# pculbertson/argus

Measured on NVIDIA B200. Metric: train image-pairs/sec, higher is better.
Workload: dtype bf16

## Files before the change

argus_b200/csrc/api.cu:

```cuda
#include "../../include/argus_b200.h"

#include "conv_ops.h"
#include "kernels.h"
#include "kernels_fp32.h"
#include "model.h"
#include "runtime.h"

#include <algorithm>
#include <cstring>
#include <vector>

using namespace argus;

static float* lib_scratch(int64_t elems) {
  static float* buf = nullptr;
  static int64_t cap = 0;
  if (elems > cap) {
    ARGUS_CUDA(cudaDeviceSynchronize());
    if (buf) ARGUS_CUDA(cudaFree(buf));
    ARGUS_CUDA(cudaMalloc(&buf, elems * sizeof(float)));
    cap = elems;
  }
  return buf;
}

static ConvShape make_shape(int N, int H, int W, int Cin, int Cout, int k, int stride, int kind) {
  ConvShape s;
  s.N = N; s.H = H; s.W = W; s.Cin = Cin; s.Cout = Cout; s.k = k; s.stride = stride; s.kind = kind;
  return s;
}

extern "C" {

const char* argus_last_error_string(void) { return get_last_error(); }
int argus_version(void) { return 100; }

int argus_profile_enable(int on) {
  ARGUS_API_BEGIN
  profile_enable(on != 0);
  ARGUS_API_END
}
int argus_profile_report(char* json, int cap) {
  ARGUS_API_BEGIN
  ARGUS_CHECK(json != nullptr && cap > 2, "bad report buffer");
  const std::string r = profile_report_json();
  ARGUS_CHECK(static_cast<int>(r.size()) < cap, "profile report buffer too small");
  std::memcpy(json, r.c_str(), r.size() + 1);
  ARGUS_API_END
}
int64_t argus_launch_count(void) { return launch_count(); }

int argus_require_device(void) {
  ARGUS_API_BEGIN
  require_sm100();
  ARGUS_API_END
}

int argus_conv2d_forward(const void* x, const void* w, void* y, int N, int H, int W, int Cin, int Cout, int k,
                         int stride, int kind, const float* scale, const float* shift, const void* residual, int relu,
                         float* stat_partial, int stat_slot_capacity, void* stream) {
  ARGUS_API_BEGIN
  require_sm100();
  ConvShape s = make_shape(N, H, W, Cin, Cout, k, stride, kind);
  ConvLaunch l = plan_conv_forward(s, static_cast<const __nv_bfloat16*>(x), static_cast<const __nv_bfloat16*>(w),
                                   static_cast<__nv_bfloat16*>(y));
  Epilogue e;
  e.scale = scale; e.shift = shift; e.residual = static_cast<const __nv_bfloat16*>(residual); e.relu = relu;
  e.stat_partial = stat_partial;
  ARGUS_CHECK(stat_partial == nullptr || stat_slot_capacity >= stat_slots(l), "statistics buffer has too few slots");
  launch_conv(l, e, static_cast<cudaStream_t>(stream));
  ARGUS_API_END
}

int argus_conv2d_stat_slots(int N, int H, int W, int Cin, int Cout, int k, int stride, int kind, int* slots) {
  ARGUS_API_BEGIN
  require_sm100();
  ARGUS_CHECK(slots != nullptr, "null argument");
  ConvShape s = make_shape(N, H, W, Cin, Cout, k, stride, kind);
  validate_shape(s);
  const int64_t m_tiles = (s.out_pixels() + kBlockM - 1) / kBlockM;
  const int64_t tiles = m_tiles * ((Cout + 63) / 64);
  *slots = 4 * static_cast<int>(std::min<int64_t>(tiles, num_sms()));
  ARGUS_API_END
}

int argus_conv2d_dgrad(const void* dy, const void* w, void* dx, int N, int H, int W, int Cin, int Cout, int k,
                       int stride, const void* residual, void* stream) {
  ARGUS_API_BEGIN
  require_sm100();
  ConvShape s = make_shape(N, H, W, Cin, Cout, k, stride, 0);
  ARGUS_CHECK(residual == nullptr || stride == 1, "residual add is only supported for stride-1 dgrad");
  auto ls = plan_conv_dgrad(s, static_cast<const __nv_bfloat16*>(dy), static_cast<const __nv_bfloat16*>(w),
                            static_cast<__nv_bfloat16*>(dx));
  Epilogue e;
  e.residual = static_cast<const __nv_bfloat16*>(residual);
  for (auto& l : ls) launch_conv(l, e, static_cast<cudaStream_t>(stream));
  ARGUS_API_END
}

int argus_conv2d_dgrad_bits(const void* dy, const void* w, void* dx, int N, int H, int W, int Cin, int Cout, int k,
                            const void* residual, const void* residual_bits, void* stream) {
  ARGUS_API_BEGIN
  require_sm100();
  ConvShape s = make_shape(N, H, W, Cin, Cout, k, 1, 0);
  ARGUS_CHECK(residual != nullptr && residual_bits != nullptr, "null argument");
  auto ls = plan_conv_dgrad(s, static_cast<const __nv_bfloat16*>(dy), static_cast<const __nv_bfloat16*>(w),
                            static_cast<__nv_bfloat16*>(dx));
  Epilogue e;
  e.residual = static_cast<const __nv_bfloat16*>(residual);
  e.residual_bits = static_cast<const uint8_t*>(residual_bits);
  for (auto& l : ls) launch_conv(l, e, static_cast<cudaStream_t>(stream));
  ARGUS_API_END
}

int argus_conv2d_dgrad_ex(const void* dy, const void* w, void* dx, int N, int H, int W, int Cin, int Cout, int stride,
                          const void* concat_a, int concat_channels, const float* bias, const void* residual,
                          const void* out_bits, float* stat_partial, int stat_slot_capacity, void* stream) {
  ARGUS_API_BEGIN
  require_sm100();
  ConvShape s = make_shape(N, H, W, Cin, Cout, 1, stride, 0);
  ARGUS_CHECK(residual == nullptr || stride == 1, "residual add is only supported for stride-1 dgrad");
  ConvLaunch l;
  if (concat_a != nullptr) {
    l = plan_dgrad_concat(s, static_cast<const __nv_bfloat16*>(dy), static_cast<const __nv_bfloat16*>(concat_a),
                          concat_channels, static_cast<const __nv_bfloat16*>(w), static_cast<__nv_bfloat16*>(dx));
  } else {
    auto ls = plan_conv_dgrad(s, static_cast<const __nv_bfloat16*>(dy), static_cast<const __nv_bfloat16*>(w),
                              static_cast<__nv_bfloat16*>(dx));
    ARGUS_CHECK(ls.size() == 1, "unexpected dgrad decomposition");
    l = ls[0];
  }
  Epilogue e;
  e.shift = bias;
  e.residual = static_cast<const __nv_bfloat16*>(residual);
  e.out_bits = static_cast<const uint8_t*>(out_bits);
  e.stat_partial = stat_partial;
  ARGUS_CHECK(stat_partial == nullptr || stat_slot_capacity >= stat_slots(l), "statistics buffer has too few slots");
  launch_conv(l, e, static_cast<cudaStream_t>(stream));
  ARGUS_API_END
}

int argus_conv2d_forward_full(const void* x, const void* w, void* y, int N, int H, int W, int Cin, int Cout, int k,
                              int stride, int kind, const float* scale, const float* shift, const void* residual,
                              const float* res_scale, const float* res_shift, int relu, void* relu_bits_out,
                              float* stat_partial, int stat_slot_capacity, int early_trigger, void* stream) {
  ARGUS_API_BEGIN
  require_sm100();
  ConvShape s = make_shape(N, H, W, Cin, Cout, k, stride, kind);
  ConvLaunch l = plan_conv_forward(s, static_cast<const bf16*>(x), static_cast<const bf16*>(w), static_cast<bf16*>(y));
  Epilogue e;
  e.scale = scale; e.shift = shift; e.residual = static_cast<const bf16*>(residual);
  e.res_scale = res_scale; e.res_shift = res_shift;
  e.relu = relu; e.relu_bits_out = static_cast<uint8_t*>(relu_bits_out);
  e.stat_partial = stat_partial;
  e.early_trigger = early_trigger;
  ARGUS_CHECK(relu_bits_out == nullptr || relu != 0, "the ReLU bit mask needs the ReLU");
  ARGUS_CHECK(res_scale == nullptr || residual != nullptr, "residual scale / shift need a residual");
  ARGUS_CHECK(stat_partial == nullptr || stat_slot_capacity >= stat_slots(l), "statistics buffer has too few slots");
  launch_conv(l, e, static_cast<cudaStream_t>(stream));
  ARGUS_API_END
}

static ConvLaunch plan_bnred_dgrad(const ConvShape& s, const void* dy, const void* w, void* dx, const void* concat_a,
                                   int concat_channels) {
  ARGUS_CHECK(s.stride == 1, "the fused BN reduction exists for stride-1 dgrads");
  if (concat_a != nullptr)
    return plan_dgrad_concat(s, static_cast<const bf16*>(dy), static_cast<const bf16*>(concat_a), concat_channels,
                             static_cast<const bf16*>(w), static_cast<bf16*>(dx));
  auto ls = plan_conv_dgrad(s, static_cast<const bf16*>(dy), static_cast<const bf16*>(w), static_cast<bf16*>(dx));
  ARGUS_CHECK(ls.size() == 1, "unexpected dgrad decomposition");
  return ls[0];
}

int argus_conv2d_dgrad_bnred(const void* dy, const void* w, void* dx, int N, int H, int W, int Cin, int Cout, int k,
                             int stride, const void* concat_a, int concat_channels, const float* bias,
                             const void* bn_raw, const float* bn_scale, const float* bn_shift, float* stat_partial,
                             int stat_slot_capacity, void* stream) {
  ARGUS_API_BEGIN
  require_sm100();
  ARGUS_CHECK(bn_raw != nullptr && bn_scale != nullptr && bn_shift != nullptr && stat_partial != nullptr,
              "null argument");
  ConvShape s = make_shape(N, H, W, Cin, Cout, k, stride, 0);
  ConvLaunch l = plan_bnred_dgrad(s, dy, w, dx, concat_a, concat_channels);
  Epilogue e;
  e.shift = bias;
  e.bn_raw = static_cast<const bf16*>(bn_raw);
  e.bn_scale = bn_scale;
  e.bn_shift = bn_shift;
  e.stat_partial = stat_partial;
  ARGUS_CHECK(stat_slot_capacity >= stat_slots(l), "statistics buffer has too few slots");
  launch_conv(l, e, static_cast<cudaStream_t>(stream));
  ARGUS_API_END
}

int argus_conv2d_launch_info(int launch, int N, int H, int W, int Cin, int Cout, int k, int stride, int kind,
                             int concat_channels, int flags, int* out, int cap, int* n_launches) {
  ARGUS_API_BEGIN
  require_sm100();
  ARGUS_CHECK(out != nullptr && n_launches != nullptr, "null argument");
  ARGUS_CUDA(cudaFree(nullptr));
  static __align__(1024) char dummy[1024];
  bf16* d = reinterpret_cast<bf16*>(dummy);
  const float* f = reinterpret_cast<const float*>(dummy);
  uint8_t* b = reinterpret_cast<uint8_t*>(dummy);
  ConvShape s = make_shape(N, H, W, Cin, Cout, k, stride, kind);
  std::vector<ConvLaunch> ls;
  if (launch == 0) ls.push_back(plan_conv_forward(s, d, d, d));
  else if (launch == 1 && (flags & ARGUS_EPI_BN_RAW)) ls.push_back(plan_bnred_dgrad(s, d, d, d, nullptr, 0));
  else if (launch == 1) ls = plan_conv_dgrad(s, d, d, d);
  else if (launch == 2 && (flags & ARGUS_EPI_BN_RAW))
    ls.push_back(plan_bnred_dgrad(make_shape(N, H, W, Cin, Cout, 1, stride, 0), d, d, d, d, concat_channels));
  else if (launch == 2) ls.push_back(plan_dgrad_concat(make_shape(N, H, W, Cin, Cout, 1, stride, 0), d, d, concat_channels, d, d));
  else throw Error("unknown launch kind");
  Epilogue e;
  if (flags & ARGUS_EPI_SCALE) e.scale = f;
  if (flags & ARGUS_EPI_SHIFT) e.shift = f;
  if (flags & ARGUS_EPI_RESIDUAL) e.residual = d;
  if (flags & ARGUS_EPI_RES_AFFINE) { e.res_scale = f; e.res_shift = f; }
  if (flags & ARGUS_EPI_RELU) e.relu = 1;
  if (flags & ARGUS_EPI_RELU_BITS_OUT) e.relu_bits_out = b;
  if (flags & ARGUS_EPI_OUT_BITS) e.out_bits = b;
  if (flags & ARGUS_EPI_RESIDUAL_BITS) e.residual_bits = b;
  if (flags & ARGUS_EPI_STATS) e.stat_partial = const_cast<float*>(f);
  if (flags & ARGUS_EPI_BN_RAW) { e.bn_raw = d; e.bn_scale = f; e.bn_shift = f; }
  if (flags & ARGUS_EPI_EARLY_TRIGGER) e.early_trigger = 1;
  *n_launches = static_cast<int>(ls.size());
  ARGUS_CHECK(cap >= ARGUS_LAUNCH_INFO_INTS * *n_launches, "launch info buffer too small");
  for (size_t i = 0; i < ls.size(); ++i) {
    const ConvLaunchInfo li = conv_launch_info(ls[i], e);
    const int v[ARGUS_LAUNCH_INFO_INTS] = {li.inst.block_n, li.inst.b_mn, li.inst.opt, li.halo, li.b_resident,
                                           li.halo_stages, li.num_m_tiles, li.num_n_tiles, li.grid, li.stat_slots};
    std::memcpy(out + i * ARGUS_LAUNCH_INFO_INTS, v, sizeof(v));
  }
  ARGUS_API_END
}

int argus_conv_instances_record(int on) {
  ARGUS_API_BEGIN
  conv_instances_record(on != 0);
  ARGUS_API_END
}
int argus_conv_instances_get(int* keys, int cap, int* n) {
  ARGUS_API_BEGIN
  ARGUS_CHECK(n != nullptr && (keys != nullptr || cap == 0), "null argument");
  const auto rec = conv_instances_recorded();
  *n = static_cast<int>(rec.size());
  for (int i = 0; i < *n && 5 * (i + 1) <= cap; ++i) std::memcpy(keys + 5 * i, rec[i].data(), 5 * sizeof(int));
  ARGUS_API_END
}

int argus_conv_instances_all(int* keys, int cap, int* n) {
  ARGUS_API_BEGIN
  ARGUS_CHECK(n != nullptr && (keys != nullptr || cap == 0), "null argument");
  const auto all = conv_instances_all();
  *n = static_cast<int>(all.size());
  for (int i = 0; i < *n && 3 * (i + 1) <= cap; ++i) std::memcpy(keys + 3 * i, all[i].data(), 3 * sizeof(int));
  ARGUS_API_END
}

int argus_conv2d_gram(const void* x, float* g, int N, int H, int W, int Cin, int Cout, int stride, void* stream) {
  ARGUS_API_BEGIN
  require_sm100();
  ConvShape s = make_shape(N, H, W, Cin, Cout, 1, stride, 0);
  validate_shape(s);
  WgradLaunch l = plan_gram(s, static_cast<const bf16*>(x), g);
  launch_wgrad(l, lib_scratch(wgrad_scratch_elems(l)), static_cast<cudaStream_t>(stream));
  ARGUS_API_END
}

int argus_colsum_pixels(const void* x, int N, int H, int W, int C, int stride, float* scratch, float* out, void* stream) {
  ARGUS_API_BEGIN
  require_sm100();
  ARGUS_CHECK(x != nullptr && scratch != nullptr && out != nullptr, "null argument");
  ARGUS_CHECK(N > 0 && H > 0 && W > 0 && (stride == 1 || stride == 2) && H % stride == 0 && W % stride == 0,
              "colsum: bad shape");
  colsum_pixels_bf16(static_cast<const bf16*>(x), N, H, W, C, stride, scratch, out, static_cast<cudaStream_t>(stream));
  ARGUS_API_END
}

int argus_bn_stats_from_gram(const void* W, const float* G, const float* s, double rows, const float* gamma,
                             const float* beta, float* running_mean, float* running_var, float momentum, float eps,
                             float* scale, float* shift, float* save_mean, float* save_invstd, float* scratch, int O,
                             int C, void* stream) {
  ARGUS_API_BEGIN
  require_sm100();
  ARGUS_CHECK((running_mean == nullptr) == (running_var == nullptr), "running mean and variance come together");
  bn_stats_from_gram(static_cast<const bf16*>(W), G, s, rows, gamma, beta, running_mean, running_var, momentum, eps,
                     scale, shift, save_mean, save_invstd, scratch, O, C, static_cast<cudaStream_t>(stream));
  ARGUS_API_END
}

int argus_conv2d_wgrad_gram(const void* dy, const void* x, float* dw, int N, int H, int W, int Cin, int Cout, int stride,
                            void* stream) {
  ARGUS_API_BEGIN
  require_sm100();
  ConvShape s = make_shape(N, H, W, Cin, Cout, 1, stride, 0);
  WgradLaunch l = plan_conv_wgrad_gram(s, static_cast<const __nv_bfloat16*>(dy), static_cast<const __nv_bfloat16*>(x), dw);
  launch_wgrad(l, lib_scratch(wgrad_scratch_elems(l)), static_cast<cudaStream_t>(stream));
  ARGUS_API_END
}

int argus_conv_bn_backward_algebraic(const void* g, const void* act, const void* w_bf16, const float* g_colsum,
                                     const float* scale, const float* mean, const float* invstd, float* dgamma,
                                     float* dbeta, float* dw, void* dact, int N, int H, int W, int C, int O, int stride,
                                     void* stream) {
  ARGUS_API_BEGIN
  require_sm100();
  cudaStream_t st = static_cast<cudaStream_t>(stream);
  ConvShape s = make_shape(N, H, W, C, O, 1, stride, 0);
  const int64_t rows = s.out_pixels();
  const size_t OC = static_cast<size_t>(O) * C, CC = static_cast<size_t>(C) * C;
  const int64_t colsum_scratch = 4LL * num_sms() * C;
  const int64_t mpart = bn_alg_matrix_scratch_elems(C);
  const int64_t total = static_cast<int64_t>(OC + CC) + C + 2 * O + C + colsum_scratch + mpart + (static_cast<int64_t>(O + C) * C + 1) / 2;
  static float* buf = nullptr;
  static int64_t cap = 0;
  if (total > cap) {
    ARGUS_CUDA(cudaDeviceSynchronize());
    if (buf) ARGUS_CUDA(cudaFree(buf));
    ARGUS_CUDA(cudaMalloc(&buf, total * sizeof(float)));
    cap = total;
  }
  float* Hb = buf;
  float* Gb = Hb + OC;
  float* sb = Gb + CC;
  float* k1k0 = sb + C;
  float* bias = k1k0 + 2 * O;
  float* cs = bias + C;
  float* mp = cs + colsum_scratch;
  bf16* bstack = reinterpret_cast<bf16*>(mp + mpart);
  const bf16* G16 = static_cast<const bf16*>(g);
  const bf16* A16 = static_cast<const bf16*>(act);
  const bf16* W16 = static_cast<const bf16*>(w_bf16);
  WgradLaunch hg = plan_conv_wgrad_gram(s, G16, A16, Hb);
  ConvLaunch concat = plan_dgrad_concat(s, G16, A16, C, bstack, static_cast<bf16*>(dact));
  ARGUS_CUDA(cudaMemsetAsync(Hb, 0, (OC + CC) * sizeof(float), st)); pdl_break(st, kPdlAfterMemop);
  launch_wgrad(hg, lib_scratch(wgrad_scratch_elems(hg)), st);
  colsum_pixels_bf16(A16, N, H, W, C, stride, cs, sb, st);
  bn_alg_backward_small(W16, Hb, Gb, sb, g_colsum, 1, O, scale, mean, invstd, static_cast<double>(rows), dgamma, dbeta, dw,
                        k1k0, bstack, bias, mp, O, C, st);
  if (stride == 2)
    ARGUS_CUDA(cudaMemsetAsync(dact, 0, static_cast<size_t>(N) * H * W * C * sizeof(bf16), st)); pdl_break(st, kPdlAfterMemop);
  Epilogue e;
  e.shift = bias;
  launch_conv(concat, e, st);
  ARGUS_API_END
}

int argus_conv2d_wgrad(const void* dy, const void* x, float* dw, int N, int H, int W, int Cin, int Cout, int k,
                       int stride, int kind, void* stream) {
  ARGUS_API_BEGIN
  require_sm100();
  ConvShape s = make_shape(N, H, W, Cin, Cout, k, stride, kind);
  WgradLaunch l = plan_conv_wgrad(s, static_cast<const __nv_bfloat16*>(dy), static_cast<const __nv_bfloat16*>(x), dw);
  launch_wgrad(l, lib_scratch(wgrad_scratch_elems(l)), static_cast<cudaStream_t>(stream));
  ARGUS_API_END
}

int argus_stem_dgrad(const void* dy, const void* w, float* dx, int N, int H, int W, void* stream) {
  ARGUS_API_BEGIN
  require_sm100();
  stem_dgrad(static_cast<const __nv_bfloat16*>(dy), static_cast<const __nv_bfloat16*>(w), dx, N, H, W,
             static_cast<cudaStream_t>(stream));
  ARGUS_API_END
}

int argus_bn_finalize(const float* partial, int slots, double count, const float* gamma, const float* beta,
                      float* running_mean, float* running_var, float momentum, float eps, float* scale, float* shift,
                      float* save_mean, float* save_invstd, int C, void* stream) {
  ARGUS_API_BEGIN
  require_sm100();
  bn_finalize(partial, slots, count, gamma, beta, running_mean, running_var, momentum, eps, scale, shift, save_mean,
              save_invstd, C, static_cast<cudaStream_t>(stream));
  ARGUS_API_END
}
int argus_bn_apply(const void* x, const float* scale, const float* shift, const void* res, const float* rscale,
                   const float* rshift, int relu, void* y, int64_t rows, int C, void* stream) {
  ARGUS_API_BEGIN
  require_sm100();
  bn_apply(static_cast<const bf16*>(x), scale, shift, static_cast<const bf16*>(res), rscale, rshift, relu,
           static_cast<bf16*>(y), nullptr, nullptr, rows, C, static_cast<cudaStream_t>(stream));
  ARGUS_API_END
}
int argus_bn_apply_bits(const void* x, const float* scale, const float* shift, const void* res, const float* rscale,
                        const float* rshift, int relu, void* y, void* relu_bits, int64_t rows, int C, void* stream) {
  ARGUS_API_BEGIN
  require_sm100();
  bn_apply(static_cast<const bf16*>(x), scale, shift, static_cast<const bf16*>(res), rscale, rshift, relu,
           static_cast<bf16*>(y), static_cast<uint8_t*>(relu_bits), nullptr, rows, C, static_cast<cudaStream_t>(stream));
  ARGUS_API_END
}
int argus_bn_backward(void* dy, const void* x, const void* out, const float* scale, const float* shift,
                      const float* mean, const float* invstd, float* dgamma, float* dbeta, void* dx, int64_t rows,
                      int C, int mask_mode, void* stream) {
  ARGUS_API_BEGIN
  require_sm100();
  cudaStream_t s = static_cast<cudaStream_t>(stream);
  bn_check_aligned(dy, x, out, dx);
  bn_bwd_reduce(static_cast<const bf16*>(dy), static_cast<const bf16*>(x), static_cast<const bf16*>(out), scale, shift,
                mean, invstd, dgamma, dbeta, rows, C, mask_mode, lib_scratch(bn_bwd_scratch_elems()), s);
  bn_bwd_apply(static_cast<bf16*>(dy), static_cast<const bf16*>(x), static_cast<const bf16*>(out), scale, shift, mean,
               invstd, dgamma, dbeta, static_cast<bf16*>(dx), rows, C, mask_mode, s);
  ARGUS_API_END
}
int argus_maxpool_forward(const void* x, const float* scale, const float* shift, void* y, void* idx, int N, int H,
                          int W, int C, void* stream) {
  ARGUS_API_BEGIN
  require_sm100();
  ARGUS_CHECK(H % 2 == 0 && W % 2 == 0 && C % 8 == 0, "maxpool: even H, W and C % 8 == 0 required");
  maxpool_fwd(static_cast<const bf16*>(x), scale, shift, static_cast<bf16*>(y), static_cast<uint8_t*>(idx), N, H, W, C,
              static_cast<cudaStream_t>(stream));
  ARGUS_API_END
}
int argus_maxpool_backward(const void* dy, const void* idx, void* dx, int N, int H, int W, int C, void* stream) {
  ARGUS_API_BEGIN
  require_sm100();
  maxpool_bwd(static_cast<const bf16*>(dy), static_cast<const uint8_t*>(idx), static_cast<bf16*>(dx), N, H, W, C,
              static_cast<cudaStream_t>(stream));
  ARGUS_API_END
}
int argus_stem_pool_bn_backward(const void* dpool, const void* idx, const void* raw, const float* scale,
                                const float* shift, const float* mean, const float* invstd, float* dgamma,
                                float* dbeta, void* dx, int N, int H, int W, int C, void* stream) {
  ARGUS_API_BEGIN
  require_sm100();
  stem_pool_bn_backward(static_cast<const bf16*>(dpool), static_cast<const uint8_t*>(idx), static_cast<const bf16*>(raw),
                        scale, shift, mean, invstd, dgamma, dbeta, static_cast<bf16*>(dx), N, H, W, C,
                        lib_scratch(bn_bwd_scratch_elems()), static_cast<cudaStream_t>(stream));
  ARGUS_API_END
}
int argus_avgpool_forward(const void* x, void* y, int N, int HW, int C, void* stream) {
  ARGUS_API_BEGIN
  require_sm100();
  avgpool_fwd(static_cast<const bf16*>(x), static_cast<bf16*>(y), N, HW, C, static_cast<cudaStream_t>(stream));
  ARGUS_API_END
}
int argus_avgpool_backward(const void* dy, void* dx, int N, int HW, int C, void* stream) {
  ARGUS_API_BEGIN
  require_sm100();
  avgpool_bwd(static_cast<const bf16*>(dy), static_cast<bf16*>(dx), nullptr, N, HW, C, static_cast<cudaStream_t>(stream));
  ARGUS_API_END
}

int argus_augment_sample_params(float* params, int n_images, int n_cams, int H, int W, uint64_t seed, uint64_t step,
                                const argus_aug_config* cfg, void* stream) {
  ARGUS_API_BEGIN
  require_sm100();
  ARGUS_CHECK(cfg != nullptr && params != nullptr && n_cams >= 1, "bad augmentation arguments");
  AugConfig c;
  c.color_jiggle = cfg->color_jiggle; c.planckian_jitter = cfg->planckian_jitter; c.blur = cfg->blur;
  c.motion_blur = cfg->motion_blur; c.plasma_shadow = cfg->plasma_shadow;
  c.brightness_lo = cfg->brightness_lo; c.brightness_span = cfg->brightness_span;
  c.contrast_lo = cfg->contrast_lo; c.contrast_span = cfg->contrast_span;
  c.saturation_lo = cfg->saturation_lo; c.saturation_span = cfg->saturation_span;
  c.hue_lo = cfg->hue_lo; c.hue_span = cfg->hue_span;
  c.random_erasing = cfg->random_erasing; c.salt_and_pepper = cfg->salt_and_pepper;
  augment_sample_params(params, n_images, n_cams, H, W, seed, step, c, static_cast<cudaStream_t>(stream));
  ARGUS_API_END
}
int argus_augment(const void* in, int in_u8, void* out, int out_s2d, const float* params, const void* arc_mask,
                  void* plasma_ws, int n_images, int H, int W, int apply, void* stream) {
  ARGUS_API_BEGIN
  require_sm100();
  ARGUS_CHECK(!apply || params != nullptr, "augmentation needs a parameter table");
  augment_images(in, in_u8 != 0, out, out_s2d != 0, params, static_cast<const uint32_t*>(arc_mask),
                 static_cast<uint32_t*>(plasma_ws), n_images, H, W, apply != 0, static_cast<cudaStream_t>(stream));
  ARGUS_API_END
}

int argus_spaghetti_sample_params(float* arcs, int n_images, int n_arcs, int H, int W, uint64_t seed, uint64_t step,
                                  void* stream) {
  ARGUS_API_BEGIN
  require_sm100();
  ARGUS_CHECK(arcs != nullptr, "null arc table");
  spaghetti_sample_params(arcs, n_images, n_arcs, H, W, seed, step, static_cast<cudaStream_t>(stream));
  ARGUS_API_END
}
int argus_spaghetti_mask(const float* arcs, void* mask, int n_images, int n_arcs, int H, int W, void* stream) {
  ARGUS_API_BEGIN
  require_sm100();
  ARGUS_CHECK(mask != nullptr && (arcs != nullptr || n_arcs == 0), "null argument");
  spaghetti_mask(arcs, static_cast<uint32_t*>(mask), n_images, n_arcs, H, W, static_cast<cudaStream_t>(stream));
  ARGUS_API_END
}
int argus_spaghetti_draw(const void* in, void* out, const float* arcs, void* mask_ws, int n_images, int n_arcs, int H,
                         int W, void* stream) {
  ARGUS_API_BEGIN
  require_sm100();
  ARGUS_CHECK(in != nullptr && out != nullptr && mask_ws != nullptr && (arcs != nullptr || n_arcs == 0), "null argument");
  spaghetti_draw(static_cast<const uint8_t*>(in), static_cast<uint8_t*>(out), arcs, static_cast<uint32_t*>(mask_ws),
                 n_images, n_arcs, H, W, static_cast<cudaStream_t>(stream));
  ARGUS_API_END
}

int argus_pose_loss(const float* pred, const float* target, float* loss, float* loss_mean, float* grad, int B,
                    float grad_scale, void* stream) {
  ARGUS_API_BEGIN
  require_sm100();
  ARGUS_CHECK(B >= 0, "negative batch");
  pose_loss_fwd_bwd(pred, target, loss, loss_mean, grad, B, grad_scale, static_cast<cudaStream_t>(stream));
  ARGUS_API_END
}

int argus_pose_exp(const float* pred, float* pose, int B, int wxyz, void* stream) {
  ARGUS_API_BEGIN
  require_sm100();
  pose_exp(pred, pose, B, wxyz, static_cast<cudaStream_t>(stream));
  ARGUS_API_END
}

int argus_clip_adam_step(float* params, const float* grads, float* exp_avg, float* exp_avg_sq, int64_t n,
                         float* scratch, float gscale, float max_norm, float lr, float beta1, float beta2, float eps,
                         int step, float* norm_out, void* stream) {
  ARGUS_API_BEGIN
  require_sm100();
  ARGUS_CHECK(step >= 1, "Adam step counter starts at 1");
  cudaStream_t s = static_cast<cudaStream_t>(stream);
  const int np = grad_sqnorm_partials(grads, n, scratch, s);
  clip_adam_step(params, grads, exp_avg, exp_avg_sq, n, scratch, np, gscale, max_norm, lr, beta1, beta2, eps, step,
                 norm_out, false, s);
  ARGUS_API_END
}
int argus_clip_adam_step_amp(float* params, const float* grads, float* exp_avg, float* exp_avg_sq, int64_t n,
                             float* scratch, float gscale, float max_norm, float lr, float beta1, float beta2, float eps,
                             int step, float* norm_out, void* stream) {
  ARGUS_API_BEGIN
  require_sm100();
  ARGUS_CHECK(step >= 1, "Adam step counter starts at 1");
  ARGUS_CHECK(norm_out != nullptr, "the caller needs the gradient norm to learn whether the step was skipped");
  cudaStream_t s = static_cast<cudaStream_t>(stream);
  const int np = grad_sqnorm_partials(grads, n, scratch, s);
  clip_adam_step(params, grads, exp_avg, exp_avg_sq, n, scratch, np, gscale, max_norm, lr, beta1, beta2, eps, step,
                 norm_out, true, s);
  ARGUS_API_END
}

static ConvShapeF32 make_shape_f32(int N, int H, int W, int Cin, int Cout, int k, int stride) {
  ARGUS_CHECK(N > 0 && H > 0 && W > 0 && Cin > 0 && Cout > 0, "empty convolution");
  ARGUS_CHECK((k == 1 || k == 3 || k == 7) && (stride == 1 || stride == 2), "fp32 conv: k in {1,3,7}, stride in {1,2}");
  ConvShapeF32 s;
  s.N = N; s.H = H; s.W = W; s.Cin = Cin; s.Cout = Cout; s.k = k; s.stride = stride;
  return s;
}
int argus_fp32_conv2d_forward(const float* x, const float* w, const float* bias, float* y, int N, int H, int W, int Cin,
                              int Cout, int k, int stride, void* stream) {
  ARGUS_API_BEGIN
  require_sm100();
  conv_f32_forward(make_shape_f32(N, H, W, Cin, Cout, k, stride), x, w, bias, y, static_cast<cudaStream_t>(stream));
  ARGUS_API_END
}
int argus_fp32_conv2d_dgrad(const float* dy, const float* w, float* dx, int N, int H, int W, int Cin, int Cout, int k,
                            int stride, void* stream) {
  ARGUS_API_BEGIN
  require_sm100();
  conv_f32_dgrad(make_shape_f32(N, H, W, Cin, Cout, k, stride), dy, w, dx, static_cast<cudaStream_t>(stream));
  ARGUS_API_END
}
int argus_fp32_conv2d_wgrad(const float* dy, const float* x, float* dw, int N, int H, int W, int Cin, int Cout, int k,
                            int stride, void* stream) {
  ARGUS_API_BEGIN
  require_sm100();
  const ConvShapeF32 s = make_shape_f32(N, H, W, Cin, Cout, k, stride);
  conv_f32_wgrad(s, dy, x, dw, lib_scratch(conv_f32_wgrad_scratch_elems(s, nullptr)), static_cast<cudaStream_t>(stream));
  ARGUS_API_END
}
static double* lib_scratch_f64(int64_t elems) { return reinterpret_cast<double*>(lib_scratch(2 * elems)); }
int argus_fp32_bn_train(const float* x, int64_t rows, int C, const float* gamma, const float* beta, float* running_mean,
                        float* running_var, float momentum, float eps, float* scale, float* shift, float* save_mean,
                        float* save_invstd, void* stream) {
  ARGUS_API_BEGIN
  require_sm100();
  bn_f32_train_stats(x, rows, C, gamma, beta, running_mean, running_var, momentum, eps, scale, shift, save_mean,
                     save_invstd, lib_scratch_f64(static_cast<int64_t>(kBnF32MaxBlocks) * 2 * C),
                     static_cast<cudaStream_t>(stream));
  ARGUS_API_END
}
int argus_fp32_bn_apply(const float* x, const float* scale, const float* shift, const float* res, const float* rscale,
                        const float* rshift, int relu, float* y, int64_t rows, int C, void* stream) {
  ARGUS_API_BEGIN
  require_sm100();
  bn_f32_apply(x, scale, shift, res, rscale, rshift, relu, y, rows, C, static_cast<cudaStream_t>(stream));
  ARGUS_API_END
}
int argus_fp32_bn_backward(const float* dy, const float* x, const float* out, const float* scale, const float* mean,
                           const float* invstd, float* dgamma, float* dbeta, float* dx, float* g_out, int64_t rows,
                           int C, void* stream) {
  ARGUS_API_BEGIN
  require_sm100();
  double* part = lib_scratch_f64(static_cast<int64_t>(kBnF32MaxBlocks) * 2 * C + C);
  float* sums = reinterpret_cast<float*>(part + static_cast<int64_t>(kBnF32MaxBlocks) * 2 * C);
  bn_f32_backward(dy, x, out, scale, mean, invstd, dgamma, dbeta, dx, g_out, rows, C, part, sums,
                  static_cast<cudaStream_t>(stream));
  ARGUS_API_END
}
int argus_fp32_maxpool_forward(const float* x, float* y, void* idx, int N, int H, int W, int C, void* stream) {
  ARGUS_API_BEGIN
  require_sm100();
  maxpool_f32_fwd(x, y, static_cast<uint8_t*>(idx), N, H, W, C, static_cast<cudaStream_t>(stream));
  ARGUS_API_END
}
int argus_fp32_maxpool_backward(const float* dy, const void* idx, float* dx, int N, int H, int W, int C, void* stream) {
  ARGUS_API_BEGIN
  require_sm100();
  maxpool_f32_bwd(dy, static_cast<const uint8_t*>(idx), dx, N, H, W, C, static_cast<cudaStream_t>(stream));
  ARGUS_API_END
}

struct argus_model {
  Model impl;
  argus_model(int n_cams, int dim) : impl(n_cams, dim) {}
};

int argus_model_create(argus_model** out, int n_cams, int resnet_output_dim) {
  ARGUS_API_BEGIN
  ARGUS_CHECK(out != nullptr, "null out pointer");
  *out = new argus_model(n_cams, resnet_output_dim);
  ARGUS_API_END
}
int argus_model_destroy(argus_model* m) {
  ARGUS_API_BEGIN
  delete m;
  ARGUS_API_END
}
int argus_model_counts(argus_model* m, int* n_params, int* n_buffers, int64_t* param_elems, int64_t* buffer_elems) {
  ARGUS_API_BEGIN
  ARGUS_CHECK(m != nullptr, "null model");
  if (n_params) *n_params = static_cast<int>(m->impl.params().size());
  if (n_buffers) *n_buffers = static_cast<int>(m->impl.buffers().size());
  if (param_elems) *param_elems = m->impl.num_param_elems();
  if (buffer_elems) *buffer_elems = m->impl.num_buffer_elems();
  ARGUS_API_END
}
int argus_model_tensor_info(argus_model* m, int is_buffer, int index, char* name, int name_cap, int64_t* offset,
                            int64_t* numel, int* ndim, int64_t* shape) {
  ARGUS_API_BEGIN
  ARGUS_CHECK(m != nullptr, "null model");
  const auto& v = is_buffer ? m->impl.buffers() : m->impl.params();
  ARGUS_CHECK(index >= 0 && index < static_cast<int>(v.size()), "tensor index out of range");
  const TensorInfo& t = v[index];
  if (name && name_cap > 0) {
    std::strncpy(name, t.name.c_str(), name_cap - 1);
    name[name_cap - 1] = 0;
  }
  if (offset) *offset = t.offset;
  if (numel) *numel = t.numel;
  if (ndim) *ndim = t.ndim;
  if (shape) for (int i = 0; i < 4; ++i) shape[i] = t.shape[i];
  ARGUS_API_END
}
int argus_model_bind(argus_model* m, float* params, float* grads, float* buffers) {
  ARGUS_API_BEGIN
  ARGUS_CHECK(m != nullptr, "null model");
  m->impl.bind(params, grads, buffers);
  ARGUS_API_END
}
int argus_model_reserve(argus_model* m, int max_batch, int H, int W, int training) {
  ARGUS_API_BEGIN
  ARGUS_CHECK(m != nullptr, "null model");
  m->impl.reserve(max_batch, H, W, training != 0);
  ARGUS_API_END
}
int argus_model_sync_weights(argus_model* m, void* stream) {
  ARGUS_API_BEGIN
  ARGUS_CHECK(m != nullptr, "null model");
  m->impl.sync_weights(static_cast<cudaStream_t>(stream));
  ARGUS_API_END
}
int argus_model_forward(argus_model* m, const void* x, int is_u8, int B, int H, int W, int training, float* out,
                        void* stream) {
  ARGUS_API_BEGIN
  ARGUS_CHECK(m != nullptr, "null model");
  m->impl.forward(x, is_u8 != 0, B, H, W, training != 0, out, static_cast<cudaStream_t>(stream));
  ARGUS_API_END
}
int argus_model_stage_input_u8(argus_model* m, const void* images, const float* aug_params, const void* arc_mask,
                               void* plasma_ws, int B, int H, int W, int training, int apply, void* stream) {
  ARGUS_API_BEGIN
  ARGUS_CHECK(m != nullptr, "null model");
  m->impl.stage_input_u8(static_cast<const uint8_t*>(images), aug_params, static_cast<const uint32_t*>(arc_mask),
                         static_cast<uint32_t*>(plasma_ws), B, H, W, training != 0, apply != 0,
                         static_cast<cudaStream_t>(stream));
  ARGUS_API_END
}
int argus_model_set_precision(argus_model* m, int mode) {
  ARGUS_API_BEGIN
  ARGUS_CHECK(m != nullptr, "null model");
  m->impl.set_precision(mode);
  ARGUS_API_END
}
int argus_model_set_wgrad_overlap(argus_model* m, int on) {
  ARGUS_API_BEGIN
  ARGUS_CHECK(m != nullptr, "null model");
  m->impl.set_wgrad_overlap(on != 0);
  ARGUS_API_END
}
int argus_model_zero_grads(argus_model* m, void* stream) {
  ARGUS_API_BEGIN
  ARGUS_CHECK(m != nullptr, "null model");
  m->impl.zero_grads(static_cast<cudaStream_t>(stream));
  ARGUS_API_END
}
int argus_model_backward(argus_model* m, const float* d_out, int stage_begin, int stage_end, void* stream) {
  ARGUS_API_BEGIN
  ARGUS_CHECK(m != nullptr, "null model");
  ARGUS_CHECK(0 <= stage_begin && stage_begin <= stage_end && stage_end <= 4, "bad stage range");
  m->impl.backward(d_out, stage_begin, stage_end, static_cast<cudaStream_t>(stream));
  ARGUS_API_END
}
int argus_model_input_grad(argus_model* m, float* dx, void* stream) {
  ARGUS_API_BEGIN
  ARGUS_CHECK(m != nullptr, "null model");
  ARGUS_CHECK(dx != nullptr, "null gradient buffer");
  m->impl.input_grad(dx, static_cast<cudaStream_t>(stream));
  ARGUS_API_END
}
int argus_model_stage_range(argus_model* m, int stage, int64_t* begin, int64_t* end) {
  ARGUS_API_BEGIN
  ARGUS_CHECK(m != nullptr, "null model");
  m->impl.stage_param_range(stage, begin, end);
  ARGUS_API_END
}
int argus_model_copy_activation(argus_model* m, int index, void* dst, int64_t capacity_elems, int64_t* rows, int* C,
                                void* stream) {
  ARGUS_API_BEGIN
  ARGUS_CHECK(m != nullptr, "null model");
  m->impl.copy_activation(index, dst, capacity_elems, rows, C, static_cast<cudaStream_t>(stream));
  ARGUS_API_END
}
int argus_model_arena_bytes(argus_model* m, int64_t* bytes) {
  ARGUS_API_BEGIN
  ARGUS_CHECK(m != nullptr, "null model");
  *bytes = static_cast<int64_t>(m->impl.arena_bytes());
  ARGUS_API_END
}

}
```

argus_b200/csrc/conv_gemm.cuh:

```cuda
#pragma once
#include "ptx.cuh"

namespace argus {

constexpr int kBlockM = 128;
constexpr int kBlockK = 64;
constexpr int kNumThreads = 320;
constexpr int kWgradThreads = 192;
constexpr int kMaxTaps = 16;

struct Tap {
  int8_t map;
  int8_t dh;
  int8_t dw;
  int8_t pad_;
  int32_t b_off;
};

struct ConvGemmParams {
  CUtensorMap a_map[4];
  CUtensorMap b_map;
  CUtensorMap out_map;
  CUtensorMap res_map;
  Tap taps[kMaxTaps];
  int num_taps;
  int kblocks_per_tap;
  int num_m_tiles;
  int num_n_tiles;
  int log2_wo;
  int log2_howo;
  int m_total;
  int n_total;
  const float* scale;
  const float* shift;
  int has_res;
  int b_resident;
  int res_stages;
  int halo;
  int halo_rows;
  int halo_row_bytes;
  int halo_stages;
  int32_t halo_boff[3][3];
  CUtensorMap halo_map;
  const uint8_t* res_bits;
  const float* res_scale;
  const float* res_shift;
  uint8_t* relu_bits_out;
  const uint8_t* out_bits;
  int k2_blocks;
  int relu;
  const __nv_bfloat16* bn_raw;
  const float* bn_scale;
  const float* bn_shift;
  int early_trigger;
  float* stat_partial;
};

template <int BLOCK_N, int OPT, int EPI = 2>
constexpr int conv_staging_buffers() { return (EPI == 4 || (BLOCK_N == 64 && !(OPT & 2))) ? 1 : 2; }

template <int BLOCK_N, int EPI = 2, int NBUF = 2>
struct ConvGemmSmem {
  static constexpr int kABytes = kBlockM * kBlockK * 2;
  static constexpr int kBBytes = BLOCK_N * kBlockK * 2;
  static constexpr int kStageBytes = kABytes + kBBytes;
  static constexpr int kStagingBytes = kBlockM * 128;
  static constexpr int kGroupCols = (EPI == 4) ? BLOCK_N / 2 : BLOCK_N;
  static constexpr int kStatsBytes = EPI * 4 * 2 * kGroupCols * 4;
  static constexpr int kPipeBytes = (232448 - 1024 - NBUF * EPI * kStagingBytes - kStatsBytes - 512) / 1024 * 1024;
  static constexpr int kStagesRaw = kPipeBytes / kStageBytes;
  static constexpr int kStages = kStagesRaw > 6 ? 6 : kStagesRaw;
  static constexpr int kOffStaging = kPipeBytes;
  static constexpr int kOffStats = kOffStaging + NBUF * EPI * kStagingBytes;
  static constexpr int kOffBars = kOffStats + kStatsBytes;
  static constexpr int kMaxStages = 8;
  static constexpr int kNumBars = 2 * kMaxStages + EPI + 2 + 2 * EPI + 1;
  static constexpr int kOffTmemPtr = kOffBars + kNumBars * 8;
  static constexpr int kTotal = kOffTmemPtr + 16;
};

constexpr int kOptAffine = 1;
constexpr int kOptRes = 2;
constexpr int kOptOutBits = 4;
constexpr int kOptRelu = 8;
constexpr int kOptResExtra = 16;
constexpr int kOptBnRed = 32;
constexpr int kOptAll = 31;
template <int BLOCK_N, int B_MN, int EPI, int OPT = kOptAll>
__global__ void __launch_bounds__(64 + 128 * EPI, 1)
conv_gemm_kernel(const __grid_constant__ ConvGemmParams p) {
  pdl_begin(p.early_trigger);
  constexpr int NBUF = conv_staging_buffers<BLOCK_N, OPT, EPI>();
  static_assert(NBUF == 2 || !(OPT & kOptRes), "the residual prefetch needs two staging buffers");
  constexpr bool SPLIT = (EPI == 4);
  constexpr int kTileGroups = SPLIT ? 2 : EPI;
  static_assert(!SPLIT || (BLOCK_N == 256 && !(OPT & kOptRes)), "split-tile mode: 256-wide tiles without residual");
  using L = ConvGemmSmem<BLOCK_N, EPI, NBUF>;
  constexpr int kStages = L::kStages;
  constexpr int kTmemCols = (2 * BLOCK_N) < 32 ? 32 : (2 * BLOCK_N);
  static_assert(BLOCK_N == 64 || BLOCK_N == 128 || BLOCK_N == 256, "BLOCK_N");

  extern __shared__ __align__(1024) uint8_t smem[];
  const uint32_t smem_base = smem_u32(smem);
  const int warp = threadIdx.x >> 5;
  const int lane = threadIdx.x & 31;

  constexpr int kMaxStages = L::kMaxStages;
  const uint32_t bar_base = smem_base + L::kOffBars;
  auto full_bar = [&](int s) { return bar_base + 8u * s; };
  auto empty_bar = [&](int s) { return bar_base + 8u * (kMaxStages + s); };
  auto tfull_bar = [&](int g) { return bar_base + 8u * (2 * kMaxStages + g); };
  auto tempty_bar = [&](int s) { return bar_base + 8u * (2 * kMaxStages + EPI + s); };
  auto res_bar = [&](int g, int b) { return bar_base + 8u * (2 * kMaxStages + EPI + 2 + 2 * g + b); };
  const uint32_t bres_bar = bar_base + 8u * (2 * kMaxStages + EPI + 2 + 2 * EPI);
  volatile uint32_t* tmem_ptr_smem = reinterpret_cast<volatile uint32_t*>(smem + L::kOffTmemPtr);
  float* s_stats_all = reinterpret_cast<float*>(smem + L::kOffStats);
  const bool resident = (p.b_resident != 0);
  const bool halo = (p.halo != 0);
  const uint32_t halo_a_bytes = static_cast<uint32_t>(p.halo_rows + 2) * p.halo_row_bytes;
  const int nstages = halo ? p.halo_stages : (resident ? p.res_stages : kStages);
  const uint32_t stage_bytes = halo ? halo_a_bytes + (resident ? 0u : 3u * L::kBBytes)
                                    : (resident ? L::kABytes : L::kStageBytes);
  const uint32_t bres_base = smem_base + static_cast<uint32_t>(nstages) * stage_bytes;

  if (threadIdx.x == 0) {
    if (smem_base & 1023u) __trap();
    for (int s = 0; s < kMaxStages; ++s) {
      mbar_init(full_bar(s), 1);
      mbar_init(empty_bar(s), 1);
    }
    mbar_init(bres_bar, 1);
    for (int s = 0; s < 2; ++s) mbar_init(tempty_bar(s), SPLIT ? 8 : 4);
    for (int g = 0; g < EPI; ++g) {
      mbar_init(tfull_bar(g), 1);
      mbar_init(res_bar(g, 0), 1);
      mbar_init(res_bar(g, 1), 1);
    }
    fence_mbar_init();
  }
  if (warp == 0 && lane == 0) {
    for (int i = 0; i < 4; ++i) tma_prefetch_desc(&p.a_map[i]);
    if (p.halo) tma_prefetch_desc(&p.halo_map);
    tma_prefetch_desc(&p.b_map);
    tma_prefetch_desc(&p.out_map);
    if (p.has_res) tma_prefetch_desc(&p.res_map);
  }
  if (warp == 1) {
    tmem_alloc(smem_u32(const_cast<uint32_t*>(tmem_ptr_smem)), kTmemCols);
    tmem_relinquish();
  }
  for (int i = threadIdx.x; i < EPI * 8 * L::kGroupCols; i += blockDim.x) s_stats_all[i] = 0.f;
  tc_fence_before();
  __syncthreads();
  tc_fence_after();
  const uint32_t tmem_base = *tmem_ptr_smem;
  pdl_wait_deferred(p.early_trigger);

  const int num_tiles = p.num_m_tiles * p.num_n_tiles;
  const int num_kblocks = p.num_taps * p.kblocks_per_tap + p.k2_blocks;

  if (warp == 0) {
    if (lane == 0) {
      auto load_b = [&](uint32_t bar, uint32_t sb, const Tap& tap, int kb, int n0) {
        if (B_MN == 0) {
          tma_load_2d(&p.b_map, bar, sb, tap.b_off + kb * kBlockK, n0);
        } else {
#pragma unroll
          for (int j = 0; j < BLOCK_N / 64; ++j)
            tma_load_2d(&p.b_map, bar, sb + j * 8192, tap.b_off + n0 + j * 64, kb * kBlockK);
        }
      };
      if (resident && blockIdx.x < num_tiles) {
        const int n0 = (blockIdx.x % p.num_n_tiles) * BLOCK_N;
        mbar_arrive_expect_tx(bres_bar, static_cast<uint32_t>(num_kblocks) * L::kBBytes);
        if (halo) {
          for (int kb = 0; kb < p.kblocks_per_tap; ++kb)
            for (int dwi = 0; dwi < 3; ++dwi)
              for (int dhi = 0; dhi < 3; ++dhi) {
                Tap tap{};
                tap.b_off = p.halo_boff[dwi][dhi];
                load_b(bres_bar, bres_base + static_cast<uint32_t>((kb * 3 + dwi) * 3 + dhi) * L::kBBytes, tap, kb, n0);
              }
        } else {
          for (int t = 0; t < p.num_taps; ++t)
            for (int kb = 0; kb < p.kblocks_per_tap; ++kb)
              load_b(bres_bar, bres_base + static_cast<uint32_t>(t * p.kblocks_per_tap + kb) * L::kBBytes, p.taps[t], kb, n0);
        }
      }
      int stage = 0;
      uint32_t phase = 0;
      for (int tile = blockIdx.x; tile < num_tiles; tile += gridDim.x) {
        const int m_tile = tile / p.num_n_tiles;
        const int n_tile = tile - m_tile * p.num_n_tiles;
        const int m0 = m_tile * kBlockM;
        const int img0 = m0 >> p.log2_howo;
        const int rem = m0 & ((1 << p.log2_howo) - 1);
        const int h0 = rem >> p.log2_wo;
        const int w0 = rem & ((1 << p.log2_wo) - 1);
        const int n0 = n_tile * BLOCK_N;
        if (halo) {
          for (int kb = 0; kb < p.kblocks_per_tap; ++kb)
            for (int dwi = 0; dwi < 3; ++dwi) {
              mbar_wait(empty_bar(stage), phase ^ 1);
              const uint32_t sa = smem_base + stage * stage_bytes;
              mbar_arrive_expect_tx(full_bar(stage), stage_bytes);
              tma_load_4d(&p.halo_map, full_bar(stage), sa, kb * kBlockK, w0 + dwi - 1, h0 - 1, img0);
              if (!resident) {
#pragma unroll
                for (int dhi = 0; dhi < 3; ++dhi) {
                  Tap tap{};
                  tap.b_off = p.halo_boff[dwi][dhi];
                  load_b(full_bar(stage), sa + halo_a_bytes + dhi * L::kBBytes, tap, kb, n0);
                }
              }
              if (++stage == nstages) { stage = 0; phase ^= 1; }
            }
          continue;
        }
        for (int t = 0; t < p.num_taps; ++t) {
          const Tap tap = p.taps[t];
          for (int kb = 0; kb < p.kblocks_per_tap; ++kb) {
            mbar_wait(empty_bar(stage), phase ^ 1);
            const uint32_t sa = smem_base + stage * stage_bytes;
            mbar_arrive_expect_tx(full_bar(stage), stage_bytes);
            tma_load_4d(&p.a_map[tap.map], full_bar(stage), sa, kb * kBlockK, w0 + tap.dw, h0 + tap.dh, img0);
            if (!resident) load_b(full_bar(stage), sa + L::kABytes, tap, kb, n0);
            if (++stage == nstages) { stage = 0; phase ^= 1; }
          }
        }
        for (int kb = 0; kb < p.k2_blocks; ++kb) {
          mbar_wait(empty_bar(stage), phase ^ 1);
          const uint32_t sa = smem_base + stage * stage_bytes;
          mbar_arrive_expect_tx(full_bar(stage), stage_bytes);
          tma_load_4d(&p.a_map[1], full_bar(stage), sa, kb * kBlockK, w0, h0, img0);
          Tap tap{};
          load_b(full_bar(stage), sa + L::kABytes, tap, p.num_taps * p.kblocks_per_tap + kb, n0);
          if (++stage == nstages) { stage = 0; phase ^= 1; }
        }
      }
    }
  } else if (warp == 1) {
    if (lane == 0) {
      constexpr uint32_t idesc = make_idesc_bf16(kBlockM, BLOCK_N, 0, B_MN);
      int stage = 0;
      uint32_t phase = 0;
      int acc = 0;
      uint32_t acc_phase = 0;
      int tgrp = 0;
      if (resident && blockIdx.x < num_tiles) mbar_wait(bres_bar, 0);
      for (int tile = blockIdx.x; tile < num_tiles; tile += gridDim.x) {
        mbar_wait(tempty_bar(acc), acc_phase ^ 1);
        tc_fence_after();
        const uint32_t tmem_d = tmem_base + acc * BLOCK_N;
        if (halo) {
          const int nst = 3 * p.kblocks_per_tap;
          for (int st = 0; st < nst; ++st) {
            mbar_wait(full_bar(stage), phase);
            tc_fence_after();
            const uint32_t sa = smem_base + stage * stage_bytes;
#pragma unroll
            for (int dhi = 0; dhi < 3; ++dhi) {
              const uint32_t a0 = sa + static_cast<uint32_t>(dhi) * p.halo_row_bytes;
              const uint32_t sb = resident ? bres_base + static_cast<uint32_t>(st * 3 + dhi) * L::kBBytes
                                           : sa + halo_a_bytes + dhi * L::kBBytes;
#pragma unroll
              for (int k = 0; k < kBlockK / 16; ++k) {
                const uint64_t da = make_smem_desc_sw128(a0 + k * 32, 0, 1024);
                const uint64_t db = (B_MN == 0) ? make_smem_desc_sw128(sb + k * 32, 0, 1024)
                                                : make_smem_desc_sw128(sb + k * 2048, 8192, 1024);
                umma_bf16(tmem_d, da, db, idesc, (st | dhi | k) != 0);
              }
            }
            umma_commit(empty_bar(stage));
            if (st == nst - 1) umma_commit(tfull_bar(tgrp));
            if (++stage == nstages) { stage = 0; phase ^= 1; }
          }
          if (++acc == 2) { acc = 0; acc_phase ^= 1; }
          if (++tgrp == kTileGroups) tgrp = 0;
          continue;
        }
        for (int kb = 0; kb < num_kblocks; ++kb) {
          mbar_wait(full_bar(stage), phase);
          tc_fence_after();
          const uint32_t sa = smem_base + stage * stage_bytes;
          const uint32_t sb = resident ? bres_base + static_cast<uint32_t>(kb) * L::kBBytes : sa + L::kABytes;
#pragma unroll
          for (int k = 0; k < kBlockK / 16; ++k) {
            const uint64_t da = make_smem_desc_sw128(sa + k * 32, 0, 1024);
            const uint64_t db = (B_MN == 0) ? make_smem_desc_sw128(sb + k * 32, 0, 1024)
                                            : make_smem_desc_sw128(sb + k * 2048, 8192, 1024);
            umma_bf16(tmem_d, da, db, idesc, (kb | k) != 0);
          }
          umma_commit(empty_bar(stage));
          if (kb == num_kblocks - 1) umma_commit(tfull_bar(tgrp));
          if (++stage == nstages) { stage = 0; phase ^= 1; }
        }
        if (++acc == 2) { acc = 0; acc_phase ^= 1; }
        if (++tgrp == kTileGroups) tgrp = 0;
      }
    }
  } else {
    const int ew = warp - 2;
    const int grp = ew >> 2;
    const int tg = SPLIT ? (grp >> 1) : grp;
    constexpr int GW = L::kGroupCols;
    const int col_base = SPLIT ? (grp & 1) * GW : 0;
    const int wq = warp & 3;
    const int r = wq * 32 + lane;
    const int et = (ew & 3) * 32 + lane;
    const bool store_leader = (et == 0);
    const uint32_t bar_id = 1 + grp;
    float* s_stats = s_stats_all + grp * 8 * GW;
    float* s_mine = s_stats + (ew & 3) * 2 * GW;
    uint8_t* stg_base = smem + L::kOffStaging + grp * NBUF * L::kStagingBytes;
    uint32_t res_phase[2] = {0, 0};
    int buf = 0;
    int cur_n = -1;
    const bool do_stats = (p.stat_partial != nullptr);
    const bool has_res = (OPT & kOptRes) ? (p.has_res != 0) : false;
    const float* const ep_scale = (OPT & kOptAffine) ? p.scale : nullptr;
    const float* const ep_shift = (OPT & kOptAffine) ? p.shift : nullptr;
    const float* const ep_res_scale = (OPT & kOptResExtra) ? p.res_scale : nullptr;
    const float* const ep_res_shift = (OPT & kOptResExtra) ? p.res_shift : nullptr;
    const uint8_t* const ep_res_bits = (OPT & kOptResExtra) ? p.res_bits : nullptr;
    const uint8_t* const ep_out_bits = (OPT & kOptOutBits) ? p.out_bits : nullptr;
    uint8_t* const ep_relu_bits_out = (OPT & kOptRelu) ? p.relu_bits_out : nullptr;
    const bool ep_relu = (OPT & kOptRelu) ? (p.relu != 0) : false;
    constexpr bool BNRED = (OPT & kOptBnRed) != 0;
    static_assert(!BNRED || ((OPT & kOptRes) && !(OPT & (kOptResExtra | kOptRelu | kOptOutBits))), "kOptBnRed rides the residual path");
    float* my_partial = do_stats ? p.stat_partial + static_cast<size_t>(EPI * blockIdx.x + grp) * 2 * p.n_total : nullptr;
    constexpr int kChunks = GW / 64;
    constexpr bool FAST_TAIL = (OPT & kOptAffine) && !(OPT & ~(kOptAffine | kOptRes | kOptRelu)) && EPI == 2;
    float* s_aff = s_stats;
    int cur_aff_n = -1;

    auto flush_stats = [&](int n_tile) {
      named_bar_sync(bar_id, 128);
      for (int c = et; c < 2 * GW; c += 128) {
        const int which = c / GW, col = c - which * GW;
        const int gc = n_tile * BLOCK_N + col_base + col;
        float acc_s = 0.f;
#pragma unroll
        for (int w = 0; w < 4; ++w) {
          acc_s += s_stats[w * 2 * GW + c];
          s_stats[w * 2 * GW + c] = 0.f;
        }
        if (gc < p.n_total) my_partial[which * p.n_total + gc] += acc_s;
      }
      named_bar_sync(bar_id, 128);
    };
    auto issue_residual = [&](int tile, int ch, int b) {
      const int m_tile = tile / p.num_n_tiles;
      const int n_tile = tile - m_tile * p.num_n_tiles;
      const int m0 = m_tile * kBlockM;
      const int img0 = m0 >> p.log2_howo;
      const int rem = m0 & ((1 << p.log2_howo) - 1);
      mbar_arrive_expect_tx(res_bar(grp, b), L::kStagingBytes);
      tma_load_4d(&p.res_map, res_bar(grp, b), smem_u32(stg_base + b * L::kStagingBytes), n_tile * BLOCK_N + ch * 64,
                  rem & ((1 << p.log2_wo) - 1), rem >> p.log2_wo, img0);
    };
    const int first_tile = blockIdx.x + tg * gridDim.x;
    if (has_res && store_leader && first_tile < num_tiles) issue_residual(first_tile, 0, 0);

    int t_local = tg;
    uint32_t full_phase = 0;
    for (int tile = first_tile; tile < num_tiles; tile += kTileGroups * gridDim.x, t_local += kTileGroups, full_phase ^= 1) {
      const int acc = t_local & 1;
      const int m_tile = tile / p.num_n_tiles;
      const int n_tile = tile - m_tile * p.num_n_tiles;
      const int m0 = m_tile * kBlockM;
      const int img0 = m0 >> p.log2_howo;
      const int rem = m0 & ((1 << p.log2_howo) - 1);
      const int h0 = rem >> p.log2_wo;
      const int w0 = rem & ((1 << p.log2_wo) - 1);
      const int n0 = n_tile * BLOCK_N + col_base;
      if (do_stats && n_tile != cur_n) {
        if (cur_n >= 0) flush_stats(cur_n);
        cur_n = n_tile;
      }
      if (FAST_TAIL && n_tile != cur_aff_n) {
        named_bar_sync(bar_id, 128);
        for (int c = et; c < GW; c += 128) {
          const int gc = n_tile * BLOCK_N + col_base + c;
          s_aff[c] = gc < p.n_total ? __ldg(ep_scale + gc) : 0.f;
          s_aff[GW + c] = gc < p.n_total ? __ldg(ep_shift + gc) : 0.f;
        }
        named_bar_sync(bar_id, 128);
        cur_aff_n = n_tile;
      }

      mbar_wait(tfull_bar(tg), full_phase);
      tc_fence_after();

#pragma unroll 1
      for (int ch = 0; ch < kChunks; ++ch) {
        uint8_t* stg = stg_base + buf * L::kStagingBytes;
        uint32_t v[2][32];
#pragma unroll
        for (int h = 0; h < 2; ++h) {
          const uint32_t taddr = tmem_base + (static_cast<uint32_t>(wq * 32) << 16) + acc * BLOCK_N + col_base + ch * 64 + h * 32;
          tmem_ld_32x32(taddr, v[h]);
        }
        if (has_res && do_stats) named_bar_sync(bar_id, 128);
        if (store_leader) {
          if (has_res) {
            tma_store_wait_read<0>();
            const bool last_ch = (ch == kChunks - 1);
            const int ntile = last_ch ? tile + kTileGroups * gridDim.x : tile;
            if (ntile < num_tiles) issue_residual(ntile, last_ch ? 0 : ch + 1, buf ^ 1);
          } else {
            if (NBUF == 2) tma_store_wait_read<1>();
            else tma_store_wait_read<0>();
          }
        }
        if (!has_res) named_bar_sync(bar_id, 128);
        uint32_t rawc[BNRED ? 32 : 1];
        if (BNRED) {
          const uint32_t* rp = reinterpret_cast<const uint32_t*>(p.bn_raw + static_cast<size_t>(m0 + wq * 32) * p.n_total +
                                                                 n0 + ch * 64) + lane;
          const int nrow = p.m_total - (m0 + wq * 32);
#pragma unroll
          for (int rr = 0; rr < 32; ++rr)
            rawc[rr] = (rr < nrow) ? ldg_nc_u32(rp + static_cast<size_t>(rr) * (p.n_total >> 1)) : 0u;
        }
        uint2 obits = make_uint2(0xffffffffu, 0xffffffffu);
        if (ep_out_bits != nullptr && m0 + r < p.m_total)
          obits = __ldg(reinterpret_cast<const uint2*>(ep_out_bits + static_cast<size_t>(m0 + r) * (p.n_total >> 3) +
                                                       ((n0 + ch * 64) >> 3)));
        uint2 rbits = make_uint2(0xffffffffu, 0xffffffffu);
        if (ep_res_bits != nullptr && m0 + r < p.m_total)
          rbits = __ldg(reinterpret_cast<const uint2*>(ep_res_bits + static_cast<size_t>(m0 + r) * (p.n_total >> 3) +
                                                       ((n0 + ch * 64) >> 3)));
        tmem_ld_wait();
        if (ch == kChunks - 1) {
          tc_fence_before();
          __syncwarp();
          if (lane == 0) mbar_arrive(tempty_bar(acc));
        }
        if (has_res) {
          mbar_wait(res_bar(grp, buf), res_phase[buf]);
          res_phase[buf] ^= 1;
        }
#pragma unroll
        for (int h = 0; h < 2; ++h) {
          const int c0 = n0 + ch * 64 + h * 32;
          if constexpr (FAST_TAIL) {
            uint32_t ob = 0;
            const float4* sc4 = reinterpret_cast<const float4*>(s_aff + ch * 64 + h * 32);
            const float4* sh4 = reinterpret_cast<const float4*>(s_aff + GW + ch * 64 + h * 32);
#pragma unroll
            for (int q = 0; q < 4; ++q) {
              const int phys = (h * 4 + q) ^ (r & 7);
              uint4* slot = reinterpret_cast<uint4*>(stg + r * 128 + phys * 16);
              uint4 rv = make_uint4(0u, 0u, 0u, 0u);
              if constexpr ((OPT & kOptRes) != 0) rv = *slot;
              const float4 s0 = sc4[2 * q], s1 = sc4[2 * q + 1], t0 = sh4[2 * q], t1 = sh4[2 * q + 1];
              uint64_t y0 = f32x2_pack(t0.x, t0.y), y1 = f32x2_pack(t0.z, t0.w), y2 = f32x2_pack(t1.x, t1.y), y3 = f32x2_pack(t1.z, t1.w);
              f32x2_fma(y0, f32x2_pack(__uint_as_float(v[h][q * 8 + 0]), __uint_as_float(v[h][q * 8 + 1])), f32x2_pack(s0.x, s0.y));
              f32x2_fma(y1, f32x2_pack(__uint_as_float(v[h][q * 8 + 2]), __uint_as_float(v[h][q * 8 + 3])), f32x2_pack(s0.z, s0.w));
              f32x2_fma(y2, f32x2_pack(__uint_as_float(v[h][q * 8 + 4]), __uint_as_float(v[h][q * 8 + 5])), f32x2_pack(s1.x, s1.y));
              f32x2_fma(y3, f32x2_pack(__uint_as_float(v[h][q * 8 + 6]), __uint_as_float(v[h][q * 8 + 7])), f32x2_pack(s1.z, s1.w));
              if constexpr ((OPT & kOptRes) != 0) {
                f32x2_add(y0, f32x2_from_bf16x2(rv.x));
                f32x2_add(y1, f32x2_from_bf16x2(rv.y));
                f32x2_add(y2, f32x2_from_bf16x2(rv.z));
                f32x2_add(y3, f32x2_from_bf16x2(rv.w));
              }
              const float2 a = f32x2_unpack(y0), b = f32x2_unpack(y1), c = f32x2_unpack(y2), d = f32x2_unpack(y3);
              const float y8[8] = {a.x, a.y, b.x, b.y, c.x, c.y, d.x, d.y};
              if constexpr ((OPT & kOptRelu) != 0) {
#pragma unroll
                for (int j = 0; j < 8; ++j) ob |= (y8[j] > 0.f ? 1u : 0u) << (q * 8 + j);
              }
              const float floor_ = ep_relu ? 0.f : -INFINITY;
              uint4 o;
              o.x = pack_bf16x2(fmaxf(y8[0], floor_), fmaxf(y8[1], floor_));
              o.y = pack_bf16x2(fmaxf(y8[2], floor_), fmaxf(y8[3], floor_));
              o.z = pack_bf16x2(fmaxf(y8[4], floor_), fmaxf(y8[5], floor_));
              o.w = pack_bf16x2(fmaxf(y8[6], floor_), fmaxf(y8[7], floor_));
              *slot = o;
            }
            if constexpr ((OPT & kOptRelu) != 0) {
              if (ep_relu_bits_out != nullptr && m0 + r < p.m_total)
                *reinterpret_cast<uint32_t*>(ep_relu_bits_out + static_cast<size_t>(m0 + r) * (p.n_total >> 3) + (c0 >> 3)) = ob;
            }
          } else {
          float f[32];
#pragma unroll
          for (int i = 0; i < 32; ++i) f[i] = __uint_as_float(v[h][i]);
          if (ep_scale != nullptr) {
#pragma unroll
            for (int i = 0; i < 32; i += 4) {
              const float4 sc = __ldg(reinterpret_cast<const float4*>(ep_scale + c0 + i));
              f[i] *= sc.x; f[i + 1] *= sc.y; f[i + 2] *= sc.z; f[i + 3] *= sc.w;
            }
          }
          if (ep_shift != nullptr) {
#pragma unroll
            for (int i = 0; i < 32; i += 4) {
              const float4 sh = __ldg(reinterpret_cast<const float4*>(ep_shift + c0 + i));
              f[i] += sh.x; f[i + 1] += sh.y; f[i + 2] += sh.z; f[i + 3] += sh.w;
            }
          }
          if (BNRED) {
            const bool row_ok = (m0 + r < p.m_total);
#pragma unroll
            for (int q = 0; q < 4; ++q) {
              const int phys = (h * 4 + q) ^ (r & 7);
              const uint4 rv = *reinterpret_cast<const uint4*>(stg + r * 128 + phys * 16);
              const float2 a = unpack_bf16x2(rv.x), b = unpack_bf16x2(rv.y), c = unpack_bf16x2(rv.z), d = unpack_bf16x2(rv.w);
              const float rr8[8] = {a.x, a.y, b.x, b.y, c.x, c.y, d.x, d.y};
              const float4 s0 = __ldg(reinterpret_cast<const float4*>(p.bn_scale + c0 + q * 8));
              const float4 s1 = __ldg(reinterpret_cast<const float4*>(p.bn_scale + c0 + q * 8 + 4));
              const float4 t0 = __ldg(reinterpret_cast<const float4*>(p.bn_shift + c0 + q * 8));
              const float4 t1 = __ldg(reinterpret_cast<const float4*>(p.bn_shift + c0 + q * 8 + 4));
              const float sc8[8] = {s0.x, s0.y, s0.z, s0.w, s1.x, s1.y, s1.z, s1.w};
              const float sh8[8] = {t0.x, t0.y, t0.z, t0.w, t1.x, t1.y, t1.z, t1.w};
#pragma unroll
              for (int j = 0; j < 8; ++j)
                f[q * 8 + j] = (row_ok && fmaf(rr8[j], sc8[j], sh8[j]) > 0.f) ? f[q * 8 + j] : 0.f;
            }
          } else if (has_res) {
#pragma unroll
            for (int q = 0; q < 4; ++q) {
              const int phys = (h * 4 + q) ^ (r & 7);
              uint4 rv = *reinterpret_cast<const uint4*>(stg + r * 128 + phys * 16);
              if (ep_res_bits != nullptr) {
                const uint32_t mb = ((h == 0 ? rbits.x : rbits.y) >> (8 * q)) & 0xffu;
                rv.x &= ((mb & 1u) ? 0x0000ffffu : 0u) | ((mb & 2u) ? 0xffff0000u : 0u);
                rv.y &= ((mb & 4u) ? 0x0000ffffu : 0u) | ((mb & 8u) ? 0xffff0000u : 0u);
                rv.z &= ((mb & 16u) ? 0x0000ffffu : 0u) | ((mb & 32u) ? 0xffff0000u : 0u);
                rv.w &= ((mb & 64u) ? 0x0000ffffu : 0u) | ((mb & 128u) ? 0xffff0000u : 0u);
              }
              float2 a = unpack_bf16x2(rv.x), b = unpack_bf16x2(rv.y), c = unpack_bf16x2(rv.z), d = unpack_bf16x2(rv.w);
              float rr8[8] = {a.x, a.y, b.x, b.y, c.x, c.y, d.x, d.y};
              if (ep_res_scale != nullptr) {
                const float4 s0 = __ldg(reinterpret_cast<const float4*>(ep_res_scale + c0 + q * 8));
                const float4 s1 = __ldg(reinterpret_cast<const float4*>(ep_res_scale + c0 + q * 8 + 4));
                const float4 t0 = __ldg(reinterpret_cast<const float4*>(ep_res_shift + c0 + q * 8));
                const float4 t1 = __ldg(reinterpret_cast<const float4*>(ep_res_shift + c0 + q * 8 + 4));
                rr8[0] = fmaf(rr8[0], s0.x, t0.x); rr8[1] = fmaf(rr8[1], s0.y, t0.y);
                rr8[2] = fmaf(rr8[2], s0.z, t0.z); rr8[3] = fmaf(rr8[3], s0.w, t0.w);
                rr8[4] = fmaf(rr8[4], s1.x, t1.x); rr8[5] = fmaf(rr8[5], s1.y, t1.y);
                rr8[6] = fmaf(rr8[6], s1.z, t1.z); rr8[7] = fmaf(rr8[7], s1.w, t1.w);
              }
#pragma unroll
              for (int j = 0; j < 8; ++j) f[q * 8 + j] += rr8[j];
            }
          }
          if (ep_relu_bits_out != nullptr) {
            uint32_t ob = 0;
#pragma unroll
            for (int i = 0; i < 32; ++i) ob |= (f[i] > 0.f ? 1u : 0u) << i;
            if (m0 + r < p.m_total)
              *reinterpret_cast<uint32_t*>(ep_relu_bits_out + static_cast<size_t>(m0 + r) * (p.n_total >> 3) +
                                           ((n0 + ch * 64 + h * 32) >> 3)) = ob;
          }
          if (ep_relu) {
#pragma unroll
            for (int i = 0; i < 32; ++i) f[i] = fmaxf(f[i], 0.f);
          }
          if (ep_out_bits != nullptr) {
            const uint32_t ob = (h == 0 ? obits.x : obits.y);
#pragma unroll
            for (int i = 0; i < 32; ++i) f[i] = ((ob >> i) & 1u) ? f[i] : 0.f;
          }
#pragma unroll
          for (int q = 0; q < 4; ++q) {
            uint4 o;
            o.x = pack_bf16x2(f[q * 8 + 0], f[q * 8 + 1]);
            o.y = pack_bf16x2(f[q * 8 + 2], f[q * 8 + 3]);
            o.z = pack_bf16x2(f[q * 8 + 4], f[q * 8 + 5]);
            o.w = pack_bf16x2(f[q * 8 + 6], f[q * 8 + 7]);
            const int phys = (h * 4 + q) ^ (r & 7);
            *reinterpret_cast<uint4*>(stg + r * 128 + phys * 16) = o;
          }
          }
        }
        fence_proxy_async_smem();
        named_bar_sync(bar_id, 128);
        if (store_leader) {
          tma_store_4d(&p.out_map, smem_u32(stg), n0 + ch * 64, w0, h0, img0);
          tma_store_commit();
        }
        if (do_stats) {
          uint64_t sa = 0ull, sb = 0ull, qa = 0ull, qb = 0ull;
          const uint32_t jl = static_cast<uint32_t>(lane) >> 2;
          const uint32_t sbase = smem_u32(stg) + static_cast<uint32_t>(wq) * 4096u + ((static_cast<uint32_t>(lane) & 3u) << 2);
#pragma unroll
          for (int rr = 0; rr < 32; rr += 2) {
            const uint64_t x0 = f32x2_from_bf16x2(lds_u32(sbase + rr * 128 + ((jl ^ (rr & 7)) << 4)));
            const uint64_t x1 = f32x2_from_bf16x2(lds_u32(sbase + (rr + 1) * 128 + ((jl ^ ((rr + 1) & 7)) << 4)));
            f32x2_add(sa, x0);
            f32x2_add(sb, x1);
            if (BNRED) {
              f32x2_fma(qa, x0, f32x2_from_bf16x2(rawc[rr]));
              f32x2_fma(qb, x1, f32x2_from_bf16x2(rawc[rr + 1]));
            } else {
              f32x2_fma_sq(qa, x0);
              f32x2_fma_sq(qb, x1);
            }
          }
          f32x2_add(sa, sb);
          f32x2_add(qa, qb);
          const float2 s2 = f32x2_unpack(sa), q2 = f32x2_unpack(qa);
          const int c = ch * 64 + lane * 2;
          s_mine[c] += s2.x;
          s_mine[c + 1] += s2.y;
          s_mine[GW + c] += q2.x;
          s_mine[GW + c + 1] += q2.y;
        }
        if (NBUF == 2) buf ^= 1;
      }
    }
    if (do_stats && cur_n >= 0) flush_stats(cur_n);
    if (store_leader) tma_store_wait_all<0>();
  }

  tc_fence_before();
  __syncthreads();
  if (warp == 1) {
    tc_fence_after();
    tmem_dealloc(tmem_base, kTmemCols);
  }
}

struct WgradParams {
  CUtensorMap dy_map;
  int co_split;
  int stacked;
  CUtensorMap a_map[4];
  Tap taps[kMaxTaps];
  int num_taps;
  int num_co_tiles;
  int num_ci_tiles;
  int num_ksplits;
  int kblocks_total;
  int log2_wo, log2_howo;
  int cout, cin;
  int dw_row_stride;
  float* dw;
  float* partial;
  long long partial_stride;
};

template <int BLOCK_N>
struct WgradSmem {
  static constexpr int kABytes = 2 * 8192;
  static constexpr int kBBytes = (BLOCK_N / 64) * 8192;
  static constexpr int kStageBytes = kABytes + kBBytes;
  static constexpr int kStagesRaw = 196608 / kStageBytes;
  static constexpr int kStages = kStagesRaw > 8 ? 8 : kStagesRaw;
  static constexpr int kOffBars = kStages * kStageBytes;
  static constexpr int kNumBars = 2 * kStages + 4;
  static constexpr int kOffTmemPtr = kOffBars + kNumBars * 8;
  static constexpr int kTotal = kOffTmemPtr + 16;
};

template <int BLOCK_N>
__global__ void __launch_bounds__(kWgradThreads, 1)
wgrad_kernel(const __grid_constant__ WgradParams p) {
  pdl_prologue();
  using L = WgradSmem<BLOCK_N>;
  constexpr int kStages = L::kStages;
  constexpr int kTmemCols = 2 * BLOCK_N;

  extern __shared__ __align__(1024) uint8_t smem[];
  const uint32_t smem_base = smem_u32(smem);
  const int warp = threadIdx.x >> 5;
  const int lane = threadIdx.x & 31;
  const uint32_t bar_base = smem_base + L::kOffBars;
  auto full_bar = [&](int s) { return bar_base + 8u * s; };
  auto empty_bar = [&](int s) { return bar_base + 8u * (kStages + s); };
  auto tfull_bar = [&](int s) { return bar_base + 8u * (2 * kStages + s); };
  auto tempty_bar = [&](int s) { return bar_base + 8u * (2 * kStages + 2 + s); };
  volatile uint32_t* tmem_ptr_smem = reinterpret_cast<volatile uint32_t*>(smem + L::kOffTmemPtr);

  if (threadIdx.x == 0) {
    if (smem_base & 1023u) __trap();
    for (int s = 0; s < kStages; ++s) {
      mbar_init(full_bar(s), 1);
      mbar_init(empty_bar(s), 1);
    }
    for (int s = 0; s < 2; ++s) {
      mbar_init(tfull_bar(s), 1);
      mbar_init(tempty_bar(s), 4);
    }
    fence_mbar_init();
  }
  if (warp == 0 && lane == 0) {
    tma_prefetch_desc(&p.dy_map);
    for (int i = 0; i < 4; ++i) tma_prefetch_desc(&p.a_map[i]);
  }
  if (warp == 1) {
    tmem_alloc(smem_u32(const_cast<uint32_t*>(tmem_ptr_smem)), kTmemCols);
    tmem_relinquish();
  }
  tc_fence_before();
  __syncthreads();
  tc_fence_after();
  const uint32_t tmem_base = *tmem_ptr_smem;

  const int items_per_tap = p.num_co_tiles * p.num_ci_tiles * p.num_ksplits;
  const int num_items = items_per_tap * p.num_taps;
  const int kb_per_split = (p.kblocks_total + p.num_ksplits - 1) / p.num_ksplits;

  auto decode = [&](int item, int& tap, int& co_t, int& ci_t, int& kb0, int& kb1) {
    int ks = item % p.num_ksplits;
    int rest = item / p.num_ksplits;
    tap = rest % p.num_taps;
    rest /= p.num_taps;
    ci_t = rest % p.num_ci_tiles;
    co_t = rest / p.num_ci_tiles;
    kb0 = ks * kb_per_split;
    kb1 = min(kb0 + kb_per_split, p.kblocks_total);
  };

  if (warp == 0) {
    if (lane == 0) {
      int stage = 0;
      uint32_t phase = 0;
      for (int item = blockIdx.x; item < num_items; item += gridDim.x) {
        int t, co_t, ci_t, kb0, kb1;
        decode(item, t, co_t, ci_t, kb0, kb1);
        const Tap tap = p.taps[t];
        for (int kb = kb0; kb < kb1; ++kb) {
          const int p0 = kb * 64;
          const int img0 = p0 >> p.log2_howo;
          const int rem = p0 & ((1 << p.log2_howo) - 1);
          const int h0 = rem >> p.log2_wo;
          const int w0 = rem & ((1 << p.log2_wo) - 1);
          mbar_wait(empty_bar(stage), phase ^ 1);
          const uint32_t sa = smem_base + stage * L::kStageBytes;
          const uint32_t sb = sa + L::kABytes;
          mbar_arrive_expect_tx(full_bar(stage), L::kStageBytes);
          if (p.stacked && co_t * 128 >= p.co_split) {
            const int c0 = co_t * 128 - p.co_split;
            tma_load_4d(&p.a_map[tap.map], full_bar(stage), sa, c0, w0 + tap.dw, h0 + tap.dh, img0);
            tma_load_4d(&p.a_map[tap.map], full_bar(stage), sa + 8192, c0 + 64, w0 + tap.dw, h0 + tap.dh, img0);
          } else {
            tma_load_2d(&p.dy_map, full_bar(stage), sa, co_t * 128, p0);
            tma_load_2d(&p.dy_map, full_bar(stage), sa + 8192, co_t * 128 + 64, p0);
          }
#pragma unroll
          for (int j = 0; j < BLOCK_N / 64; ++j)
            tma_load_4d(&p.a_map[tap.map], full_bar(stage), sb + j * 8192, ci_t * BLOCK_N + j * 64, w0 + tap.dw,
                        h0 + tap.dh, img0);
          if (++stage == kStages) { stage = 0; phase ^= 1; }
        }
      }
    }
  } else if (warp == 1) {
    if (lane == 0) {
      constexpr uint32_t idesc = make_idesc_bf16(128, BLOCK_N, 1, 1);
      int stage = 0;
      uint32_t phase = 0;
      int acc = 0;
      uint32_t acc_phase = 0;
      for (int item = blockIdx.x; item < num_items; item += gridDim.x) {
        int t, co_t, ci_t, kb0, kb1;
        decode(item, t, co_t, ci_t, kb0, kb1);
        mbar_wait(tempty_bar(acc), acc_phase ^ 1);
        tc_fence_after();
        const uint32_t tmem_d = tmem_base + acc * BLOCK_N;
        for (int kb = kb0; kb < kb1; ++kb) {
          mbar_wait(full_bar(stage), phase);
          tc_fence_after();
          const uint32_t sa = smem_base + stage * L::kStageBytes;
          const uint32_t sb = sa + L::kABytes;
#pragma unroll
          for (int k = 0; k < 4; ++k) {
            const uint64_t da = make_smem_desc_sw128(sa + k * 2048, 8192, 1024);
            const uint64_t db = make_smem_desc_sw128(sb + k * 2048, 8192, 1024);
            umma_bf16(tmem_d, da, db, idesc, (kb > kb0) || (k != 0));
          }
          umma_commit(empty_bar(stage));
          if (kb == kb1 - 1) umma_commit(tfull_bar(acc));
          if (++stage == kStages) { stage = 0; phase ^= 1; }
        }
        if (kb1 <= kb0) umma_commit(tfull_bar(acc));
        if (++acc == 2) { acc = 0; acc_phase ^= 1; }
      }
    }
  } else {
    const int wq = warp & 3;
    const int r = wq * 32 + lane;
    int acc = 0;
    uint32_t acc_phase = 0;
    for (int item = blockIdx.x; item < num_items; item += gridDim.x) {
      int t, co_t, ci_t, kb0, kb1;
      decode(item, t, co_t, ci_t, kb0, kb1);
      const Tap tap = p.taps[t];
      mbar_wait(tfull_bar(acc), acc_phase);
      tc_fence_after();
      const int co = co_t * 128 + r;
      const bool use_partial = (p.num_ksplits > 1);
      const int ks = item % p.num_ksplits;
      float* base = use_partial ? p.partial + static_cast<size_t>(ks) * p.partial_stride : p.dw;
      float* row = base + static_cast<size_t>(co) * p.dw_row_stride + tap.b_off + ci_t * BLOCK_N;
#pragma unroll 1
      for (int ch = 0; ch < BLOCK_N / 32; ++ch) {
        uint32_t v[32];
        const uint32_t taddr = tmem_base + (static_cast<uint32_t>(wq * 32) << 16) + acc * BLOCK_N + ch * 32;
        tmem_ld_32x32(taddr, v);
        tmem_ld_wait();
        if (kb1 > kb0 && co < p.cout) {
#pragma unroll
          for (int i = 0; i < 32; i += 4) {
            const int ci = ci_t * BLOCK_N + ch * 32 + i;
            if (ci + 3 < p.cin) {
              if (use_partial)
                *reinterpret_cast<uint4*>(row + ch * 32 + i) = make_uint4(v[i], v[i + 1], v[i + 2], v[i + 3]);
              else
                red_add_v4(row + ch * 32 + i, v[i], v[i + 1], v[i + 2], v[i + 3]);
            }
          }
        }
      }
      tc_fence_before();
      __syncwarp();
      if (lane == 0) mbar_arrive(tempty_bar(acc));
      if (++acc == 2) { acc = 0; acc_phase ^= 1; }
    }
  }

  tc_fence_before();
  __syncthreads();
  if (warp == 1) {
    tc_fence_after();
    tmem_dealloc(tmem_base, kTmemCols);
  }
}

struct XposeBox {
  int8_t map, dh, dw, valid;
  int16_t c_off;
  int16_t out_off;
};
struct WgradXposeParams {
  CUtensorMap dy_map;
  CUtensorMap a_map[4];
  XposeBox boxes[10];
  int num_splits;
  int kblocks_total;
  int log2_wo, log2_howo;
  int dw_row_stride;
  float* partial;
};

template <int NBOX>
struct WgradXposeSmem {
  static constexpr int kStageBytes = 8192 + NBOX * 8192;
  static constexpr int kStagesRaw = 196608 / kStageBytes;
  static constexpr int kStages = kStagesRaw > 6 ? 6 : kStagesRaw;
  static constexpr int kOffBars = kStages * kStageBytes;
  static constexpr int kNumBars = 2 * kStages + 1;
  static constexpr int kOffTmemPtr = kOffBars + kNumBars * 8;
  static constexpr int kTotal = kOffTmemPtr + 16;
};

template <int NBOX>
__global__ void __launch_bounds__(kWgradThreads, 1)
wgrad_xpose_kernel(const __grid_constant__ WgradXposeParams p) {
  pdl_prologue();
  using L = WgradXposeSmem<NBOX>;
  constexpr int kStages = L::kStages;
  constexpr int kPairs = NBOX / 2;
  constexpr int kTmemCols = kPairs * 64 <= 64 ? 64 : (kPairs * 64 <= 128 ? 128 : (kPairs * 64 <= 256 ? 256 : 512));

  extern __shared__ __align__(1024) uint8_t smem[];
  const uint32_t smem_base = smem_u32(smem);
  const int warp = threadIdx.x >> 5;
  const int lane = threadIdx.x & 31;
  const uint32_t bar_base = smem_base + L::kOffBars;
  auto full_bar = [&](int s) { return bar_base + 8u * s; };
  auto empty_bar = [&](int s) { return bar_base + 8u * (kStages + s); };
  const uint32_t done_bar = bar_base + 8u * (2 * kStages);
  volatile uint32_t* tmem_ptr_smem = reinterpret_cast<volatile uint32_t*>(smem + L::kOffTmemPtr);

  int n_valid = 0;
  for (int b = 0; b < NBOX; ++b) n_valid += p.boxes[b].valid ? 1 : 0;
  for (int s = 0; s < kStages; ++s)
    for (int b = 0; b < NBOX; ++b)
      if (!p.boxes[b].valid) {
        uint4* z = reinterpret_cast<uint4*>(smem + s * L::kStageBytes + 8192 + b * 8192);
        for (int i = threadIdx.x; i < 512; i += kWgradThreads) z[i] = make_uint4(0u, 0u, 0u, 0u);
      }
  fence_proxy_async_smem();

  if (threadIdx.x == 0) {
    if (smem_base & 1023u) __trap();
    for (int s = 0; s < kStages; ++s) {
      mbar_init(full_bar(s), 1);
      mbar_init(empty_bar(s), 1);
    }
    mbar_init(done_bar, 1);
    fence_mbar_init();
  }
  if (warp == 0 && lane == 0) {
    tma_prefetch_desc(&p.dy_map);
    for (int i = 0; i < 4; ++i) tma_prefetch_desc(&p.a_map[i]);
  }
  if (warp == 1) {
    tmem_alloc(smem_u32(const_cast<uint32_t*>(tmem_ptr_smem)), kTmemCols);
    tmem_relinquish();
  }
  tc_fence_before();
  __syncthreads();
  tc_fence_after();
  const uint32_t tmem_base = *tmem_ptr_smem;

  const int per = (p.kblocks_total + p.num_splits - 1) / p.num_splits;
  const int kb0 = blockIdx.x * per;
  const int kb1 = min(kb0 + per, p.kblocks_total);

  if (warp == 0) {
    if (lane == 0) {
      int stage = 0;
      uint32_t phase = 0;
      for (int kb = kb0; kb < kb1; ++kb) {
        const int p0 = kb * 64;
        const int img0 = p0 >> p.log2_howo;
        const int rem = p0 & ((1 << p.log2_howo) - 1);
        const int h0 = rem >> p.log2_wo;
        const int w0 = rem & ((1 << p.log2_wo) - 1);
        mbar_wait(empty_bar(stage), phase ^ 1);
        const uint32_t sb = smem_base + stage * L::kStageBytes;
        mbar_arrive_expect_tx(full_bar(stage), 8192u * (1 + n_valid));
        tma_load_2d(&p.dy_map, full_bar(stage), sb, 0, p0);
#pragma unroll
        for (int b = 0; b < NBOX; ++b) {
          const XposeBox bx = p.boxes[b];
          if (bx.valid)
            tma_load_4d(&p.a_map[bx.map], full_bar(stage), sb + 8192 + b * 8192, bx.c_off, w0 + bx.dw, h0 + bx.dh, img0);
        }
        if (++stage == kStages) { stage = 0; phase ^= 1; }
      }
    }
  } else if (warp == 1) {
    if (lane == 0) {
      constexpr uint32_t idesc = make_idesc_bf16(128, 64, 1, 1);
      int stage = 0;
      uint32_t phase = 0;
      for (int kb = kb0; kb < kb1; ++kb) {
        mbar_wait(full_bar(stage), phase);
        tc_fence_after();
        const uint32_t sb = smem_base + stage * L::kStageBytes;
#pragma unroll
        for (int j = 0; j < kPairs; ++j) {
#pragma unroll
          for (int k = 0; k < 4; ++k) {
            const uint64_t da = make_smem_desc_sw128(sb + 8192 + j * 16384 + k * 2048, 8192, 1024);
            const uint64_t db = make_smem_desc_sw128(sb + k * 2048, 8192, 1024);
            umma_bf16(tmem_base + j * 64, da, db, idesc, (kb > kb0) || (k != 0));
          }
        }
        umma_commit(empty_bar(stage));
        if (++stage == kStages) { stage = 0; phase ^= 1; }
      }
      umma_commit(done_bar);
    }
  } else {
    const int wq = warp & 3;
    const int r = wq * 32 + lane;
    mbar_wait(done_bar, 0);
    tc_fence_after();
    float* base = p.partial + static_cast<size_t>(blockIdx.x) * 64 * p.dw_row_stride;
#pragma unroll 1
    for (int j = 0; j < kPairs; ++j) {
      const XposeBox bx = p.boxes[2 * j + (r >> 6)];
      float* col0 = base + bx.out_off + (r & 63);
#pragma unroll 1
      for (int h = 0; h < 2; ++h) {
        uint32_t v[32];
        tmem_ld_32x32(tmem_base + (static_cast<uint32_t>(wq * 32) << 16) + j * 64 + h * 32, v);
        tmem_ld_wait();
        if (bx.valid) {
          if (kb1 > kb0) {
#pragma unroll
            for (int i = 0; i < 32; ++i) col0[static_cast<size_t>(h * 32 + i) * p.dw_row_stride] = __uint_as_float(v[i]);
          } else {
#pragma unroll
            for (int i = 0; i < 32; ++i) col0[static_cast<size_t>(h * 32 + i) * p.dw_row_stride] = 0.f;
          }
        }
      }
    }
  }

  tc_fence_before();
  __syncthreads();
  if (warp == 1) {
    tc_fence_after();
    tmem_dealloc(tmem_base, kTmemCols);
  }
}

}
```

argus_b200/csrc/conv_ops.cu:

```cuda
#include "conv_ops.h"

#include <algorithm>
#include <array>
#include <atomic>
#include <cstdio>
#include <cstdlib>
#include <cstring>
#include <map>
#include <mutex>
#include <set>

namespace argus {

static thread_local std::string g_last_error;
void set_last_error(const std::string& msg) { g_last_error = msg; }
const char* get_last_error() { return g_last_error.c_str(); }

typedef CUresult (*EncodeTiledFn)(CUtensorMap*, CUtensorMapDataType, cuuint32_t, void*, const cuuint64_t*,
                                  const cuuint64_t*, const cuuint32_t*, const cuuint32_t*, CUtensorMapInterleave,
                                  CUtensorMapSwizzle, CUtensorMapL2promotion, CUtensorMapFloatOOBfill);

static EncodeTiledFn get_encode_fn() {
  static EncodeTiledFn fn = nullptr;
  static std::once_flag once;
  std::call_once(once, [] {
    void* sym = nullptr;
    cudaDriverEntryPointQueryResult qres;
    cudaError_t e = cudaGetDriverEntryPoint("cuTensorMapEncodeTiled", &sym, cudaEnableDefault, &qres);
    if (e == cudaSuccess && qres == cudaDriverEntryPointSuccess) fn = reinterpret_cast<EncodeTiledFn>(sym);
  });
  ARGUS_CHECK(fn != nullptr, "cuTensorMapEncodeTiled not available from the CUDA driver");
  return fn;
}

CUtensorMap make_tmap_bf16(const void* base, int rank, const uint64_t* dims, const uint64_t* strides_bytes,
                           const uint32_t* box) {
  CUtensorMap m;
  std::memset(&m, 0, sizeof(m));
  cuuint64_t gdim[5];
  cuuint64_t gstr[4];
  cuuint32_t bdim[5];
  cuuint32_t estr[5];
  for (int i = 0; i < rank; ++i) {
    gdim[i] = dims[i];
    bdim[i] = box[i];
    estr[i] = 1;
  }
  for (int i = 0; i + 1 < rank; ++i) gstr[i] = strides_bytes[i];
  ARGUS_CHECK((reinterpret_cast<uintptr_t>(base) & 15) == 0, "TMA base address must be 16-byte aligned");
  ARGUS_CHECK(box[0] * 2 == 128, "SWIZZLE_128B boxes are 64 bf16 wide");
  CUresult r = get_encode_fn()(&m, CU_TENSOR_MAP_DATA_TYPE_BFLOAT16, rank, const_cast<void*>(base), gdim, gstr, bdim,
                               estr, CU_TENSOR_MAP_INTERLEAVE_NONE, CU_TENSOR_MAP_SWIZZLE_128B,
                               CU_TENSOR_MAP_L2_PROMOTION_L2_256B, CU_TENSOR_MAP_FLOAT_OOB_FILL_NONE);
  if (r != CUDA_SUCCESS) {
    std::string msg = "cuTensorMapEncodeTiled failed (" + std::to_string(static_cast<int>(r)) + ") rank=" +
                      std::to_string(rank) + " dims=";
    for (int i = 0; i < rank; ++i) msg += std::to_string(dims[i]) + ",";
    msg += " strides=";
    for (int i = 0; i + 1 < rank; ++i) msg += std::to_string(strides_bytes[i]) + ",";
    msg += " box=";
    for (int i = 0; i < rank; ++i) msg += std::to_string(box[i]) + ",";
    throw Error(msg);
  }
  return m;
}

namespace {
struct ProfRecord {
  std::string family;
  cudaEvent_t start, stop;
  double flops, bytes;
};
std::atomic<int64_t> g_launches{0};
bool g_profiling = false;
std::vector<ProfRecord> g_records;
std::vector<cudaEvent_t> g_event_pool;
cudaEvent_t new_event() {
  if (!g_event_pool.empty()) {
    cudaEvent_t e = g_event_pool.back();
    g_event_pool.pop_back();
    return e;
  }
  cudaEvent_t e;
  ARGUS_CUDA(cudaEventCreate(&e));
  return e;
}
}

void profile_enable(bool on) {
  if (on) {
    for (auto& r : g_records) { g_event_pool.push_back(r.start); g_event_pool.push_back(r.stop); }
    g_records.clear();
  }
  g_profiling = on;
}
bool profile_enabled() { return g_profiling; }
int64_t launch_count() { return g_launches.load(); }

ProfileScope::ProfileScope(const char* family, cudaStream_t s, double flops, double bytes) : stream(s) {
  g_launches.fetch_add(1);
  if (!g_profiling) return;
  ProfRecord r{family, new_event(), new_event(), flops, bytes};
  cudaEventRecord(r.start, s);
  pdl_break(s, kPdlAfterRecord);
  slot = static_cast<int>(g_records.size());
  g_records.push_back(r);
}
ProfileScope::ProfileScope(const std::string& family, cudaStream_t s, double flops, double bytes) : stream(s) {
  g_launches.fetch_add(1);
  if (!g_profiling) return;
  ProfRecord r{family, new_event(), new_event(), flops, bytes};
  cudaEventRecord(r.start, s);
  pdl_break(s, kPdlAfterRecord);
  slot = static_cast<int>(g_records.size());
  g_records.push_back(r);
}
bool profile_detailed() {
  static int v = -1;
  if (v < 0) {
    const char* e = getenv("ARGUS_PROFILE_DETAIL");
    v = (e && e[0] == '1') ? 1 : 0;
  }
  return v == 1;
}
ProfileScope::~ProfileScope() {
  if (slot >= 0) { cudaEventRecord(g_records[slot].stop, stream); pdl_break(stream, kPdlAfterRecord); }
}

std::string profile_report_json() {
  struct Agg { int launches = 0; double ms = 0, flops = 0, bytes = 0; };
  std::map<std::string, Agg> agg;
  std::vector<std::string> order;
  for (auto& r : g_records) {
    cudaEventSynchronize(r.stop);
    float ms = 0.f;
    cudaEventElapsedTime(&ms, r.start, r.stop);
    if (!agg.count(r.family)) order.push_back(r.family);
    Agg& a = agg[r.family];
    a.launches += 1; a.ms += ms; a.flops += r.flops; a.bytes += r.bytes;
  }
  std::string out = "{";
  bool first = true;
  for (auto& name : order) {
    const Agg& a = agg[name];
    char buf[384];
    snprintf(buf, sizeof(buf), "%s\"%s\": {\"launches\": %d, \"ms\": %.6f, \"flops\": %.6e, \"bytes\": %.6e}",
             first ? "" : ", ", name.c_str(), a.launches, a.ms, a.flops, a.bytes);
    out += buf;
    first = false;
  }
  out += "}";
  return out;
}

bool pdl_enabled() {
  static const bool on = [] { const char* e = getenv("ARGUS_PDL"); return !(e && e[0] == '0'); }();
  return on;
}
namespace {
std::mutex g_pdl_mu;
std::vector<std::pair<cudaStream_t, bool>> g_pdl_ok;
}
void pdl_break(cudaStream_t stream, int) {
  std::lock_guard<std::mutex> lk(g_pdl_mu);
  for (auto& e : g_pdl_ok)
    if (e.first == stream) e.second = false;
}
void pdl_break_all() {
  std::lock_guard<std::mutex> lk(g_pdl_mu);
  for (auto& e : g_pdl_ok) e.second = false;
}
bool pdl_chain_ok(cudaStream_t stream) {
  std::lock_guard<std::mutex> lk(g_pdl_mu);
  for (auto& e : g_pdl_ok)
    if (e.first == stream) return e.second;
  return false;
}
void pdl_mark_kernel(cudaStream_t stream) {
  std::lock_guard<std::mutex> lk(g_pdl_mu);
  for (auto& e : g_pdl_ok)
    if (e.first == stream) { e.second = true; return; }
  g_pdl_ok.emplace_back(stream, true);
}
int num_sms() {
  static int n = 0;
  if (n == 0) {
    int dev = 0;
    ARGUS_CUDA(cudaGetDevice(&dev));
    ARGUS_CUDA(cudaDeviceGetAttribute(&n, cudaDevAttrMultiProcessorCount, dev));
  }
  return n;
}

void require_sm100() {
  int dev = 0, major = 0;
  ARGUS_CUDA(cudaGetDevice(&dev));
  ARGUS_CUDA(cudaDeviceGetAttribute(&major, cudaDevAttrComputeCapabilityMajor, dev));
  ARGUS_CHECK(major == 10, "argus_b200 kernels are built for sm_100a only; no fallback path exists");
}

void validate_shape(const ConvShape& s) {
  ARGUS_CHECK(s.N > 0 && s.H > 0 && s.W > 0, "empty convolution input");
  ARGUS_CHECK(is_pow2(s.H) && is_pow2(s.W), "spatial sizes must be powers of two (tiles are linear pixel runs)");
  if (s.kind == 1) {
    ARGUS_CHECK(s.Cout == 64 && s.stride == 2 && s.H >= 2 && s.W >= 2, "stem convolution is 3->64, stride 2");
    return;
  }
  ARGUS_CHECK(s.k == 1 || s.k == 3, "kernel size must be 1 or 3");
  ARGUS_CHECK(s.stride == 1 || s.stride == 2, "stride must be 1 or 2");
  ARGUS_CHECK(s.Cin % 64 == 0 && s.Cout % 64 == 0, "channel counts must be multiples of 64");
  ARGUS_CHECK(s.H % s.stride == 0 && s.W % s.stride == 0, "spatial size must be divisible by the stride");
}

static int pick_block_n(int n, int64_t m_tiles = (1 << 30)) {
  const int cands[3] = {256, 128, 64};
  for (int bn : cands)
    if (n >= bn && n % bn == 0 && m_tiles * (n / bn) >= num_sms()) return bn;
  return 64;
}

static void pixel_box(int Wo, int Ho, int pixels, uint32_t& bw, uint32_t& bh, uint32_t& bn) {
  bw = std::min(Wo, pixels);
  bh = std::min(Ho, pixels / static_cast<int>(bw));
  bn = pixels / (bw * bh);
}

static void make_input_maps(const ConvShape& s, const __nv_bfloat16* x, int pixels, CUtensorMap* maps) {
  uint32_t bw, bh, bn;
  pixel_box(s.Wo(), s.Ho(), pixels, bw, bh, bn);
  const uint32_t box[4] = {64, bw, bh, bn};
  if (s.kind == 1) {
    const uint64_t Hs = s.H / 2, Ws = s.W / 2, Wp = Ws + 4;
    const uint64_t dims[4] = {64, Ws, Hs, static_cast<uint64_t>(s.N)};
    const uint64_t str[3] = {32, Wp * 32, Hs * Wp * 32};
    maps[0] = make_tmap_bf16(x, 4, dims, str, box);
    for (int i = 1; i < 4; ++i) maps[i] = maps[0];
    return;
  }
  const uint64_t C = s.Cin, H = s.H, W = s.W;
  if (s.stride == 1) {
    const uint64_t dims[4] = {C, W, H, static_cast<uint64_t>(s.N)};
    const uint64_t str[3] = {C * 2, W * C * 2, H * W * C * 2};
    maps[0] = make_tmap_bf16(x, 4, dims, str, box);
    for (int i = 1; i < 4; ++i) maps[i] = maps[0];
  } else {
    for (int a = 0; a < 2; ++a)
      for (int b = 0; b < 2; ++b) {
        const uint64_t dims[4] = {C, W / 2, H / 2, static_cast<uint64_t>(s.N)};
        const uint64_t str[3] = {2 * C * 2, 2 * W * C * 2, H * W * C * 2};
        maps[a * 2 + b] = make_tmap_bf16(x + (a * W + b) * C, 4, dims, str, box);
      }
  }
}

static int fill_forward_taps(const ConvShape& s, Tap* taps) {
  int n = 0;
  if (s.kind == 1) {
    for (int pi = 0; pi < 4; ++pi) taps[n++] = Tap{0, static_cast<int8_t>(pi - 2), 0, 0, pi * 64};
    return n;
  }
  const int pad = s.k / 2;
  for (int kh = 0; kh < s.k; ++kh)
    for (int kw = 0; kw < s.k; ++kw) {
      Tap t{};
      t.b_off = (kh * s.k + kw) * s.Cin;
      const int eh = kh - pad, ew = kw - pad;
      if (s.stride == 1) {
        t.map = 0;
        t.dh = static_cast<int8_t>(eh);
        t.dw = static_cast<int8_t>(ew);
      } else {
        const int a = eh & 1, b = ew & 1;
        t.map = static_cast<int8_t>(a * 2 + b);
        t.dh = static_cast<int8_t>((eh - a) / 2);
        t.dw = static_cast<int8_t>((ew - b) / 2);
      }
      taps[n++] = t;
    }
  return n;
}

static void setup_halo(ConvGemmParams& p, const ConvShape& s, const __nv_bfloat16* src, int channels, bool dgrad,
                       int block_n) {
  p.halo = 0;
  if (s.kind != 0 || s.k != 3 || s.stride != 1 || block_n > 128) return;
  uint32_t bw, bh, bn;
  pixel_box(s.W, s.H, kBlockM, bw, bh, bn);
  if (bn != 1 || static_cast<int>(bw) != s.W || s.W < 8 || static_cast<int>(bw * bh) != kBlockM) return;
  const uint64_t C = channels, H = s.H, W = s.W;
  const uint64_t dims[4] = {C, W, H, static_cast<uint64_t>(s.N)};
  const uint64_t str[3] = {C * 2, W * C * 2, H * W * C * 2};
  const uint32_t box[4] = {64, bw, bh + 2, 1};
  p.halo_map = make_tmap_bf16(src, 4, dims, str, box);
  p.halo_rows = static_cast<int>(bh);
  p.halo_row_bytes = s.W * 128;
  for (int dwi = 0; dwi < 3; ++dwi)
    for (int dhi = 0; dhi < 3; ++dhi) {
      const int kh = dgrad ? 2 - dhi : dhi, kw = dgrad ? 2 - dwi : dwi;
      p.halo_boff[dwi][dhi] = (kh * 3 + kw) * s.Cin;
    }
  p.halo = 1;
}

ConvLaunch plan_conv_forward(const ConvShape& s, const __nv_bfloat16* x, const __nv_bfloat16* w, __nv_bfloat16* y) {
  validate_shape(s);
  ConvLaunch l;
  std::memset(&l.p, 0, sizeof(l.p));
  l.block_n = pick_block_n(s.Cout, (s.out_pixels() + kBlockM - 1) / kBlockM);
  l.b_mn = 0;
  ConvGemmParams& p = l.p;
  make_input_maps(s, x, kBlockM, p.a_map);
  {
    const uint64_t dims[2] = {static_cast<uint64_t>(s.Ktot()), static_cast<uint64_t>(s.Cout)};
    const uint64_t str[1] = {static_cast<uint64_t>(s.Ktot()) * 2};
    const uint32_t box[2] = {64, static_cast<uint32_t>(l.block_n)};
    p.b_map = make_tmap_bf16(w, 2, dims, str, box);
  }
  {
    uint32_t bw, bh, bn;
    pixel_box(s.Wo(), s.Ho(), kBlockM, bw, bh, bn);
    const uint64_t C = s.Cout, Ho = s.Ho(), Wo = s.Wo();
    const uint64_t dims[4] = {C, Wo, Ho, static_cast<uint64_t>(s.N)};
    const uint64_t str[3] = {C * 2, Wo * C * 2, Ho * Wo * C * 2};
    const uint32_t box[4] = {64, bw, bh, bn};
    p.out_map = make_tmap_bf16(y, 4, dims, str, box);
    l.out_geom.set(4, dims, str, box);
  }
  p.num_taps = fill_forward_taps(s, p.taps);
  p.kblocks_per_tap = (s.kind == 1) ? 1 : s.Cin / 64;
  p.m_total = static_cast<int>(s.out_pixels());
  p.n_total = s.Cout;
  p.num_m_tiles = (p.m_total + kBlockM - 1) / kBlockM;
  p.num_n_tiles = (s.Cout + l.block_n - 1) / l.block_n;
  p.log2_wo = ilog2(s.Wo());
  p.log2_howo = ilog2(s.Ho() * s.Wo());
  setup_halo(p, s, x, s.Cin, false, l.block_n);
  l.epi = choose_epilogue_groups(p, l.block_n);
  return l;
}

std::vector<ConvLaunch> plan_conv_dgrad(const ConvShape& s, const __nv_bfloat16* dy, const __nv_bfloat16* w,
                                        __nv_bfloat16* dx) {
  validate_shape(s);
  ARGUS_CHECK(s.kind == 0, "the stem has no input gradient");
  std::vector<ConvLaunch> out;
  const int pad = s.k / 2;
  const int Ho = s.Ho(), Wo = s.Wo();
  const int block_n = pick_block_n(s.Cin, (static_cast<int64_t>(s.N) * Ho * Wo + kBlockM - 1) / kBlockM);
  const int classes = (s.stride == 1) ? 1 : 4;
  for (int cls = 0; cls < classes; ++cls) {
    const int a = cls >> 1, b = cls & 1;
    ConvLaunch l;
    std::memset(&l.p, 0, sizeof(l.p));
    l.block_n = block_n;
    l.b_mn = 1;
    ConvGemmParams& p = l.p;
    int n = 0;
    for (int kh = 0; kh < s.k; ++kh)
      for (int kw = 0; kw < s.k; ++kw) {
        Tap t{};
        t.map = 0;
        t.b_off = (kh * s.k + kw) * s.Cin;
        if (s.stride == 1) {
          t.dh = static_cast<int8_t>(pad - kh);
          t.dw = static_cast<int8_t>(pad - kw);
        } else {
          const int eh = a + pad - kh, ew = b + pad - kw;
          if ((eh & 1) || (ew & 1)) continue;
          t.dh = static_cast<int8_t>(eh / 2);
          t.dw = static_cast<int8_t>(ew / 2);
        }
        p.taps[n++] = t;
      }
    if (n == 0) continue;
    p.num_taps = n;
    p.kblocks_per_tap = s.Cout / 64;
    uint32_t bw, bh, bn;
    pixel_box(Wo, Ho, kBlockM, bw, bh, bn);
    {
      const uint64_t C = s.Cout;
      const uint64_t dims[4] = {C, static_cast<uint64_t>(Wo), static_cast<uint64_t>(Ho), static_cast<uint64_t>(s.N)};
      const uint64_t str[3] = {C * 2, Wo * C * 2, static_cast<uint64_t>(Ho) * Wo * C * 2};
      const uint32_t box[4] = {64, bw, bh, bn};
      p.a_map[0] = make_tmap_bf16(dy, 4, dims, str, box);
      for (int i = 1; i < 4; ++i) p.a_map[i] = p.a_map[0];
    }
    {
      const uint64_t dims[2] = {static_cast<uint64_t>(s.Ktot()), static_cast<uint64_t>(s.Cout)};
      const uint64_t str[1] = {static_cast<uint64_t>(s.Ktot()) * 2};
      const uint32_t box[2] = {64, 64};
      p.b_map = make_tmap_bf16(w, 2, dims, str, box);
    }
    {
      const uint64_t C = s.Cin, H = s.H, W = s.W;
      const uint32_t box[4] = {64, bw, bh, bn};
      if (s.stride == 1) {
        const uint64_t dims[4] = {C, W, H, static_cast<uint64_t>(s.N)};
        const uint64_t str[3] = {C * 2, W * C * 2, H * W * C * 2};
        p.out_map = make_tmap_bf16(dx, 4, dims, str, box);
        l.out_geom.set(4, dims, str, box);
      } else {
        const uint64_t dims[4] = {C, W / 2, H / 2, static_cast<uint64_t>(s.N)};
        const uint64_t str[3] = {2 * C * 2, 2 * W * C * 2, H * W * C * 2};
        p.out_map = make_tmap_bf16(dx + (a * W + b) * C, 4, dims, str, box);
      }
    }
    p.m_total = s.N * Ho * Wo;
    p.n_total = s.Cin;
    p.num_m_tiles = (p.m_total + kBlockM - 1) / kBlockM;
    p.num_n_tiles = (s.Cin + block_n - 1) / block_n;
    p.log2_wo = ilog2(Wo);
    p.log2_howo = ilog2(Ho * Wo);
    setup_halo(p, s, dy, s.Cout, true, block_n);
    l.epi = choose_epilogue_groups(p, block_n);
    out.push_back(l);
  }
  return out;
}

ConvLaunch plan_dgrad_concat(const ConvShape& s, const __nv_bfloat16* dy, const __nv_bfloat16* a1, int C1,
                             const __nv_bfloat16* bstack, __nv_bfloat16* dx) {
  validate_shape(s);
  ARGUS_CHECK(s.kind == 0 && s.k == 1, "concatenated dgrad is defined for 1x1 convolutions");
  ARGUS_CHECK(C1 > 0 && C1 % 64 == 0, "second source must have a multiple of 64 channels");
  std::vector<ConvLaunch> ls = plan_conv_dgrad(s, dy, bstack, dx);
  ARGUS_CHECK(ls.size() == 1, "unexpected dgrad decomposition");
  ConvLaunch l = ls[0];
  ConvGemmParams& p = l.p;
  const int Ho = s.Ho(), Wo = s.Wo();
  uint32_t bw, bh, bn;
  pixel_box(Wo, Ho, kBlockM, bw, bh, bn);
  {
    const uint64_t C = C1, H = s.H, W = s.W, st = s.stride;
    const uint64_t dims[4] = {C, static_cast<uint64_t>(Wo), static_cast<uint64_t>(Ho), static_cast<uint64_t>(s.N)};
    const uint64_t str[3] = {st * C * 2, st * W * C * 2, H * W * C * 2};
    const uint32_t box[4] = {64, bw, bh, bn};
    p.a_map[1] = make_tmap_bf16(a1, 4, dims, str, box);
  }
  {
    const uint64_t dims[2] = {static_cast<uint64_t>(s.Cin), static_cast<uint64_t>(s.Cout + C1)};
    const uint64_t str[1] = {static_cast<uint64_t>(s.Cin) * 2};
    const uint32_t box[2] = {64, 64};
    p.b_map = make_tmap_bf16(bstack, 2, dims, str, box);
  }
  p.k2_blocks = C1 / 64;
  l.epi = choose_epilogue_groups(p, l.block_n);
  return l;
}

WgradLaunch plan_conv_wgrad(const ConvShape& s, const __nv_bfloat16* dy, const __nv_bfloat16* x, float* dw) {
  validate_shape(s);
  WgradLaunch l;
  std::memset(&l.p, 0, sizeof(l.p));
  WgradParams& p = l.p;
  const int cin_tile_extent = (s.kind == 1) ? 64 : s.Cin;
  l.block_n = pick_block_n(cin_tile_extent);
  const int64_t pixels = s.out_pixels();
  {
    const uint64_t dims[2] = {static_cast<uint64_t>(s.Cout), static_cast<uint64_t>(pixels)};
    const uint64_t str[1] = {static_cast<uint64_t>(s.Cout) * 2};
    const uint32_t box[2] = {64, 64};
    p.dy_map = make_tmap_bf16(dy, 2, dims, str, box);
  }
  make_input_maps(s, x, 64, p.a_map);
  p.num_taps = fill_forward_taps(s, p.taps);
  p.num_co_tiles = (s.Cout + 127) / 128;
  p.num_ci_tiles = (cin_tile_extent + l.block_n - 1) / l.block_n;
  p.kblocks_total = static_cast<int>((pixels + 63) / 64);
  const int base_items = p.num_co_tiles * p.num_ci_tiles * p.num_taps;
  int splits = std::max(1, num_sms() / base_items);
  splits = std::min(splits, std::max(1, p.kblocks_total / 4));
  while (splits > 1) {
    const int per = (p.kblocks_total + splits - 1) / splits;
    if (per * (splits - 1) < p.kblocks_total) break;
    --splits;
  }
  p.num_ksplits = splits;
  p.log2_wo = ilog2(s.Wo());
  p.log2_howo = ilog2(s.Ho() * s.Wo());
  p.cout = s.Cout;
  p.cin = cin_tile_extent;
  p.dw_row_stride = s.Ktot();
  p.dw = dw;

  const int n_boxes = (s.kind == 1) ? 4 : (s.k * s.k) * (s.Cin / 64);
  if (s.Cout == 64 && n_boxes <= 10 && (s.kind == 1 || (s.k == 3 && s.Cin == 64))) {
    WgradXposeParams& x = l.xp;
    std::memset(&x, 0, sizeof(x));
    x.dy_map = p.dy_map;
    for (int i = 0; i < 4; ++i) x.a_map[i] = p.a_map[i];
    int nb = 0;
    for (int t = 0; t < p.num_taps; ++t)
      for (int cb = 0; cb < cin_tile_extent / 64; ++cb) {
        XposeBox b{};
        b.map = p.taps[t].map; b.dh = p.taps[t].dh; b.dw = p.taps[t].dw; b.valid = 1;
        b.c_off = static_cast<int16_t>(cb * 64);
        b.out_off = static_cast<int16_t>(p.taps[t].b_off + cb * 64);
        x.boxes[nb++] = b;
      }
    const int padded = nb <= 2 ? 2 : (nb <= 4 ? 4 : 10);
    l.xpose_nbox = padded;
    x.kblocks_total = p.kblocks_total;
    x.num_splits = std::max(1, std::min(num_sms(), p.kblocks_total / 4));
    while (x.num_splits > 1) {
      const int per = (x.kblocks_total + x.num_splits - 1) / x.num_splits;
      if (per * (x.num_splits - 1) < x.kblocks_total) break;
      --x.num_splits;
    }
    x.log2_wo = p.log2_wo;
    x.log2_howo = p.log2_howo;
    x.dw_row_stride = p.dw_row_stride;
    p.num_ksplits = x.num_splits;
  }
  return l;
}

WgradLaunch plan_conv_wgrad_gram(const ConvShape& s, const __nv_bfloat16* dy, const __nv_bfloat16* x, float* dw) {
  ARGUS_CHECK(s.kind == 0 && s.k == 1, "stacked weight gradient + Gram is defined for 1x1 convolutions");
  ARGUS_CHECK(s.Cout % 128 == 0, "Cout must be a multiple of 128");
  ConvShape st = s;
  st.Cout = s.Cout + s.Cin;
  WgradLaunch l = plan_conv_wgrad(st, dy, x, dw);
  ARGUS_CHECK(l.xpose_nbox == 0, "unexpected kernel choice");
  const int64_t pixels = s.out_pixels();
  const uint64_t dims[2] = {static_cast<uint64_t>(s.Cout), static_cast<uint64_t>(pixels)};
  const uint64_t str[1] = {static_cast<uint64_t>(s.Cout) * 2};
  const uint32_t box[2] = {64, 64};
  l.p.dy_map = make_tmap_bf16(dy, 2, dims, str, box);
  l.p.co_split = s.Cout;
  l.p.stacked = 1;
  return l;
}

WgradLaunch plan_gram(const ConvShape& s, const __nv_bfloat16* x, float* g) {
  ARGUS_CHECK(s.kind == 0 && s.k == 1, "Gram matrix of the pixels a 1x1 convolution reads");
  ConvShape st = s;
  st.Cout = s.Cin;
  WgradLaunch l = plan_conv_wgrad(st, x, x, g);
  ARGUS_CHECK(l.xpose_nbox == 0, "unexpected kernel choice");
  l.p.co_split = 0;
  l.p.stacked = 1;
  l.family = "bn_algebra";
  return l;
}

template <int BN, int BMN, int EPI, int OPT>
static ConvGemmParams finish_params(const ConvGemmParams& p) {
  using L = ConvGemmSmem<BN, EPI, conv_staging_buffers<BN, OPT, EPI>()>;
  const int tiles = p.num_m_tiles * p.num_n_tiles;
  const int grid = std::min(tiles, num_sms());
  ConvGemmParams q = p;
  const int bres = p.num_taps * p.kblocks_per_tap * L::kBBytes;
  const bool fixed_n = (tiles <= grid) || (grid % p.num_n_tiles == 0);
  if (q.halo) {
    const int halo_a = (q.halo_rows + 2) * q.halo_row_bytes;
    const int stage = halo_a + 3 * L::kBBytes;
    q.halo_stages = std::min(L::kMaxStages, L::kPipeBytes / stage);
    if (q.halo_stages < 2) q.halo = 0;
    if (q.halo && fixed_n && q.k2_blocks == 0 && bres + 2 * halo_a <= L::kPipeBytes) {
      q.b_resident = 1;
      q.halo_stages = std::min(L::kMaxStages, (L::kPipeBytes - bres) / halo_a);
    }
  }
  return q;
}

template <int BN, int BMN, int EPI, int OPT>
static void launch_conv_t(const ConvGemmParams& q, cudaStream_t stream) {
  using L = ConvGemmSmem<BN, EPI, conv_staging_buffers<BN, OPT, EPI>()>;
  static bool configured = false;
  if (!configured) {
    ARGUS_CUDA(cudaFuncSetAttribute(conv_gemm_kernel<BN, BMN, EPI, OPT>, cudaFuncAttributeMaxDynamicSharedMemorySize, L::kTotal));
    configured = true;
  }
  const int grid = std::min(q.num_m_tiles * q.num_n_tiles, num_sms());
  launch_kernel(conv_gemm_kernel<BN, BMN, EPI, OPT>, grid, 64 + 128 * EPI, L::kTotal, stream, q);
  ARGUS_CUDA(cudaGetLastError());
}

int choose_epilogue_groups(const ConvGemmParams&, int) { return 2; }

namespace {
struct ConvInstanceEntry {
  int block_n, b_mn, opt;
  ConvGemmParams (*finish)(const ConvGemmParams&);
  void (*launch)(const ConvGemmParams&, cudaStream_t);
};
template <int BN, int BMN, int OPT>
constexpr ConvInstanceEntry conv_entry() {
  return {BN, BMN, OPT, &finish_params<BN, BMN, 2, OPT>, &launch_conv_t<BN, BMN, 2, OPT>};
}
constexpr int kTail = kOptAffine | kOptRes | kOptRelu;
const ConvInstanceEntry kConvInstances[] = {
    conv_entry<64, 1, kOptRes | kOptBnRed>(), conv_entry<128, 1, kOptRes | kOptBnRed>(),
    conv_entry<256, 1, kOptRes | kOptBnRed>(), conv_entry<64, 1, kOptAffine | kOptRes | kOptBnRed>(),
    conv_entry<128, 1, kOptAffine | kOptRes | kOptBnRed>(), conv_entry<256, 1, kOptAffine | kOptRes | kOptBnRed>(),
    conv_entry<64, 0, kTail>(), conv_entry<128, 0, kTail>(), conv_entry<256, 0, kTail>(),
    conv_entry<64, 0, kOptAffine | kOptRelu>(), conv_entry<128, 0, kOptAffine | kOptRelu>(),
    conv_entry<256, 0, kOptAffine | kOptRelu>(), conv_entry<64, 0, kOptAffine>(), conv_entry<128, 0, kOptAffine>(),
    conv_entry<256, 0, kOptAffine>(),
    conv_entry<64, 0, 0>(), conv_entry<128, 0, 0>(), conv_entry<256, 0, 0>(), conv_entry<64, 1, 0>(),
    conv_entry<128, 1, 0>(), conv_entry<256, 1, 0>(),
    conv_entry<64, 1, kOptRes | kOptOutBits>(), conv_entry<128, 1, kOptRes | kOptOutBits>(),
    conv_entry<256, 1, kOptRes | kOptOutBits>(), conv_entry<64, 1, kOptAffine | kOptOutBits>(),
    conv_entry<128, 1, kOptAffine | kOptOutBits>(), conv_entry<256, 1, kOptAffine | kOptOutBits>(),
    conv_entry<64, 0, kOptAll>(), conv_entry<128, 0, kOptAll>(), conv_entry<256, 0, kOptAll>(),
    conv_entry<64, 1, kOptAll>(), conv_entry<128, 1, kOptAll>(), conv_entry<256, 1, kOptAll>(),
};
const ConvInstanceEntry& find_instance(const ConvInstance& c) {
  for (const auto& e : kConvInstances)
    if (e.block_n == c.block_n && e.b_mn == c.b_mn && e.opt == c.opt) return e;
  throw Error("unsupported conv tile configuration");
}

std::mutex g_record_mu;
std::atomic<bool> g_recording{false};
std::set<std::array<int, 5>> g_recorded;
}

ConvGemmParams epilogue_params(const ConvLaunch& l, const Epilogue& e) {
  ConvGemmParams p = l.p;
  p.scale = e.scale;
  p.shift = e.shift;
  p.has_res = 0;
  if (e.residual != nullptr) {
    ARGUS_CHECK(l.out_geom.rank == 4, "this launch cannot take a residual (strided output)");
    p.res_map = make_tmap_bf16(e.residual, 4, l.out_geom.dims, l.out_geom.strides, l.out_geom.box);
    p.has_res = 1;
    p.res_bits = e.residual_bits;
  }
  p.bn_raw = nullptr;
  p.bn_scale = e.bn_scale;
  p.bn_shift = e.bn_shift;
  if (e.bn_raw != nullptr) {
    ARGUS_CHECK(l.b_mn == 1 && l.out_geom.rank == 4, "the fused BN reduction exists for dense-output dgrad launches");
    ARGUS_CHECK(e.residual == nullptr && e.out_bits == nullptr && e.relu == 0 && e.relu_bits_out == nullptr &&
                    e.scale == nullptr && e.bn_scale != nullptr && e.bn_shift != nullptr && e.stat_partial != nullptr,
                "fused BN reduction: unsupported epilogue combination");
    p.res_map = make_tmap_bf16(e.bn_raw, 4, l.out_geom.dims, l.out_geom.strides, l.out_geom.box);
    p.has_res = 1;
    p.bn_raw = e.bn_raw;
  }
  p.early_trigger = (e.early_trigger && pdl_enabled()) ? 1 : 0;
  p.relu = e.relu;
  p.out_bits = e.out_bits;
  p.res_scale = e.res_scale;
  p.res_shift = e.res_shift;
  p.relu_bits_out = e.relu_bits_out;
  ARGUS_CHECK((e.res_scale == nullptr) == (e.res_shift == nullptr), "residual scale and shift come together");
  p.stat_partial = e.stat_partial;
  return p;
}

ConvInstance select_conv_instance(const ConvLaunch& l, const ConvGemmParams& p) {
  ARGUS_CHECK(l.epi == 2, "two epilogue groups");
  int need = 0;
  if (p.scale || p.shift) need |= kOptAffine;
  if (p.has_res) need |= kOptRes;
  if (p.res_bits || p.res_scale) need |= kOptRes | kOptResExtra;
  if (p.out_bits) need |= kOptOutBits;
  if (p.relu || p.relu_bits_out) need |= kOptRelu;
  if (p.bn_raw != nullptr) return {l.block_n, 1, kOptRes | kOptBnRed | (p.shift != nullptr ? kOptAffine : 0)};
  const bool folded_bn = p.scale && p.shift && !p.stat_partial && !p.res_bits && !p.res_scale && !p.out_bits;
  if (l.b_mn == 0 && folded_bn && (need & kOptAffine) && !(need & ~kTail) && (p.relu || !p.relu_bits_out)) {
    const int t = need & kTail;
    if (t == kTail || t == (kOptAffine | kOptRelu) || t == kOptAffine) return {l.block_n, 0, t};
  }
  if (need == 0) return {l.block_n, l.b_mn, 0};
  if (l.b_mn == 1 && (need & ~(kOptRes | kOptOutBits)) == 0) return {l.block_n, 1, kOptRes | kOptOutBits};
  if (l.b_mn == 1 && (need & ~(kOptAffine | kOptOutBits)) == 0) return {l.block_n, 1, kOptAffine | kOptOutBits};
  return {l.block_n, l.b_mn, kOptAll};
}

ConvLaunchInfo conv_launch_info(const ConvLaunch& l, const Epilogue& e) {
  const ConvGemmParams p = epilogue_params(l, e);
  ConvLaunchInfo info;
  info.inst = select_conv_instance(l, p);
  const ConvGemmParams q = find_instance(info.inst).finish(p);
  info.halo = q.halo;
  info.b_resident = q.b_resident;
  info.halo_stages = q.halo ? q.halo_stages : 0;
  info.num_m_tiles = q.num_m_tiles;
  info.num_n_tiles = q.num_n_tiles;
  info.grid = std::min(q.num_m_tiles * q.num_n_tiles, num_sms());
  info.stat_slots = stat_slots(l);
  return info;
}

void conv_instances_record(bool on) {
  std::lock_guard<std::mutex> lk(g_record_mu);
  if (on) g_recorded.clear();
  g_recording = on;
}
std::vector<std::array<int, 3>> conv_instances_all() {
  std::vector<std::array<int, 3>> v;
  for (const auto& e : kConvInstances) v.push_back({e.block_n, e.b_mn, e.opt});
  return v;
}
std::vector<std::array<int, 5>> conv_instances_recorded() {
  std::lock_guard<std::mutex> lk(g_record_mu);
  return std::vector<std::array<int, 5>>(g_recorded.begin(), g_recorded.end());
}

void launch_conv(const ConvLaunch& l, const Epilogue& e, cudaStream_t stream) {
  const ConvGemmParams p = epilogue_params(l, e);
  const double flops = 2.0 * p.m_total * static_cast<double>(p.n_total) * (p.num_taps * p.kblocks_per_tap + p.k2_blocks) * kBlockK;
  std::string fam = l.b_mn ? "conv_dgrad" : "conv_fwd";
  if (g_profiling && profile_detailed())
    fam += ":M" + std::to_string(p.m_total) + "_N" + std::to_string(p.n_total) + "_K" +
           std::to_string((p.num_taps * p.kblocks_per_tap + p.k2_blocks) * kBlockK) + "_t" + std::to_string(p.num_taps);
  double bytes = 0.0;
  {
    int maps = 0;
    for (int t = 0; t < p.num_taps; ++t) maps |= 1 << p.taps[t].map;
    const int nmaps = __builtin_popcount(static_cast<unsigned>(maps));
    const double kc = static_cast<double>(p.kblocks_per_tap) * kBlockK;
    bytes += 2.0 * p.m_total * kc * nmaps + 2.0 * p.m_total * p.k2_blocks * kBlockK;
    bytes += 2.0 * p.m_total * p.n_total * (p.has_res ? 2 : 1);
    bytes += (p.out_bits ? 0.125 : 0.0) * p.m_total * p.n_total + (p.relu_bits_out ? 0.125 : 0.0) * p.m_total * p.n_total;
    bytes += 2.0 * p.n_total * (p.num_taps * kc + p.k2_blocks * kBlockK);
  }
  ProfileScope prof(fam, stream, flops, bytes);
  const ConvInstance inst = select_conv_instance(l, p);
  const ConvInstanceEntry& entry = find_instance(inst);
  const ConvGemmParams q = entry.finish(p);
  if (g_recording) {
    std::lock_guard<std::mutex> lk(g_record_mu);
    g_recorded.insert({inst.block_n, inst.b_mn, inst.opt, q.halo, q.b_resident});
  }
  entry.launch(q, stream);
}

int stat_slots(const ConvLaunch& l) {
  const int tiles = l.p.num_m_tiles * l.p.num_n_tiles;
  return l.epi * std::min(tiles, num_sms());
}

int64_t wgrad_scratch_elems(const WgradLaunch& l) {
  if (l.xpose_nbox > 0) return static_cast<int64_t>(l.xp.num_splits) * 64 * l.p.dw_row_stride;
  if (l.p.num_ksplits <= 1) return 0;
  return static_cast<int64_t>(l.p.num_ksplits) * l.p.cout * l.p.dw_row_stride;
}

__global__ void __launch_bounds__(256)
wgrad_reduce_kernel(const float4* __restrict__ partial, float4* __restrict__ dw, int64_t n4, int splits) {
  pdl_prologue();
  __shared__ float4 red[4][64];
  const int e = threadIdx.x & 63, g = threadIdx.x >> 6;
  auto add = [](float4& a, const float4& v) { a.x += v.x; a.y += v.y; a.z += v.z; a.w += v.w; };
  for (int64_t base = static_cast<int64_t>(blockIdx.x) * 64; base < n4; base += static_cast<int64_t>(gridDim.x) * 64) {
    const int64_t i = base + e;
    float4 acc = make_float4(0.f, 0.f, 0.f, 0.f);
    if (i < n4) {
      int k = g;
      for (; k + 28 < splits; k += 32) {
        float4 v[8];
#pragma unroll
        for (int u = 0; u < 8; ++u) v[u] = partial[static_cast<int64_t>(k + 4 * u) * n4 + i];
#pragma unroll
        for (int u = 0; u < 8; ++u) add(acc, v[u]);
      }
      for (; k < splits; k += 4) add(acc, partial[static_cast<int64_t>(k) * n4 + i]);
    }
    red[g][e] = acc;
    __syncthreads();
    if (g == 0 && i < n4) {
      float4 t = red[0][e];
      add(t, red[1][e]); add(t, red[2][e]); add(t, red[3][e]);
      float4 d = dw[i];
      add(d, t);
      dw[i] = d;
    }
    __syncthreads();
  }
}

template <int NBOX>
static void launch_wgrad_xpose_t(const WgradXposeParams& p, cudaStream_t stream) {
  using L = WgradXposeSmem<NBOX>;
  static bool configured = false;
  if (!configured) {
    ARGUS_CUDA(cudaFuncSetAttribute(wgrad_xpose_kernel<NBOX>, cudaFuncAttributeMaxDynamicSharedMemorySize, L::kTotal));
    configured = true;
  }
  launch_kernel(wgrad_xpose_kernel<NBOX>, p.num_splits, kWgradThreads, L::kTotal, stream, p);
  ARGUS_CUDA(cudaGetLastError());
}

template <int BN>
static void launch_wgrad_t(const WgradParams& p, cudaStream_t stream) {
  using L = WgradSmem<BN>;
  static bool configured = false;
  if (!configured) {
    ARGUS_CUDA(cudaFuncSetAttribute(wgrad_kernel<BN>, cudaFuncAttributeMaxDynamicSharedMemorySize, L::kTotal));
    configured = true;
  }
  const int items = p.num_co_tiles * p.num_ci_tiles * p.num_ksplits * p.num_taps;
  const int grid = std::min(items, num_sms());
  launch_kernel(wgrad_kernel<BN>, grid, kWgradThreads, L::kTotal, stream, p);
  ARGUS_CUDA(cudaGetLastError());
}

void launch_wgrad(const WgradLaunch& l0, float* scratch, cudaStream_t stream) {
  WgradLaunch l = l0;
  const int64_t need = wgrad_scratch_elems(l);
  ARGUS_CHECK(need == 0 || scratch != nullptr, "split-K weight gradient needs a scratch buffer");
  l.p.partial = scratch;
  l.p.partial_stride = static_cast<long long>(l.p.cout) * l.p.dw_row_stride;
  const double flops = 2.0 * l.p.kblocks_total * 64.0 * l.p.cout * static_cast<double>(l.p.cin) * l.p.num_taps;
  std::string fam = l0.family;
  if (g_profiling && profile_detailed())
    fam += std::string(l.xpose_nbox > 0 ? "x" : "") + ":P" + std::to_string(l.p.kblocks_total * 64) + "_Co" + std::to_string(l.p.cout) + "_Ci" +
           std::to_string(l.p.cin) + "_t" + std::to_string(l.p.num_taps) + "_s" + std::to_string(l.p.num_ksplits);
  const double wbytes = 2.0 * l.p.kblocks_total * 64.0 * (static_cast<double>(l.p.cout) + l.p.cin) +
                        4.0 * l.p.cout * static_cast<double>(l.p.dw_row_stride);
  ProfileScope prof(fam, stream, flops, wbytes);
  if (l.xpose_nbox > 0) {
    ARGUS_CHECK(scratch != nullptr, "transposed weight gradient needs a scratch buffer");
    l.xp.partial = scratch;
    switch (l.xpose_nbox) {
      case 2: launch_wgrad_xpose_t<2>(l.xp, stream); break;
      case 4: launch_wgrad_xpose_t<4>(l.xp, stream); break;
      case 10: launch_wgrad_xpose_t<10>(l.xp, stream); break;
      default: throw Error("unsupported transposed wgrad configuration");
    }
  } else {
    switch (l.block_n) {
      case 64: launch_wgrad_t<64>(l.p, stream); break;
      case 128: launch_wgrad_t<128>(l.p, stream); break;
      case 256: launch_wgrad_t<256>(l.p, stream); break;
      default: throw Error("unsupported wgrad tile configuration");
    }
  }
  if (need > 0) {
    const int64_t n4 = l.p.partial_stride / 4;
    const int grid = static_cast<int>(std::min<int64_t>((n4 + 63) / 64, 4LL * num_sms()));
    launch_kernel(wgrad_reduce_kernel, grid, 256, 0, stream, reinterpret_cast<const float4*>(scratch),
                                                  reinterpret_cast<float4*>(l.p.dw), n4, l.p.num_ksplits);
    ARGUS_CUDA(cudaGetLastError());
  }
}

}
```

argus_b200/csrc/conv_ops.h:

```cpp
#pragma once
#include <array>
#include <vector>

#include "conv_gemm.cuh"
#include "runtime.h"

namespace argus {

struct ConvShape {
  int N = 0, H = 0, W = 0;
  int Cin = 0, Cout = 0;
  int k = 1, stride = 1;
  int kind = 0;
  int Ho() const { return H / stride; }
  int Wo() const { return W / stride; }
  int Ktot() const { return kind == 1 ? 256 : k * k * Cin; }
  int64_t out_pixels() const { return static_cast<int64_t>(N) * Ho() * Wo(); }
};

struct Epilogue {
  const float* scale = nullptr;
  const float* shift = nullptr;
  const __nv_bfloat16* residual = nullptr;
  const uint8_t* residual_bits = nullptr;
  const uint8_t* out_bits = nullptr;
  const float* res_scale = nullptr;
  const float* res_shift = nullptr;
  uint8_t* relu_bits_out = nullptr;
  int relu = 0;
  float* stat_partial = nullptr;
  const __nv_bfloat16* bn_raw = nullptr;
  const float* bn_scale = nullptr;
  const float* bn_shift = nullptr;
  int early_trigger = 0;
};

struct TmapGeom {
  int rank = 0;
  uint64_t dims[4] = {0, 0, 0, 0};
  uint64_t strides[3] = {0, 0, 0};
  uint32_t box[4] = {0, 0, 0, 0};
  void set(int r, const uint64_t* d, const uint64_t* s, const uint32_t* b) {
    rank = r;
    for (int i = 0; i < r; ++i) { dims[i] = d[i]; box[i] = b[i]; }
    for (int i = 0; i + 1 < r; ++i) strides[i] = s[i];
  }
};

struct ConvLaunch {
  ConvGemmParams p;
  int block_n = 64;
  int b_mn = 0;
  int epi = 2;
  TmapGeom out_geom;
};

struct WgradLaunch {
  const char* family = "conv_wgrad";
  WgradParams p;
  int block_n = 64;
  int xpose_nbox = 0;
  WgradXposeParams xp;
};

void validate_shape(const ConvShape& s);

ConvLaunch plan_conv_forward(const ConvShape& s, const __nv_bfloat16* x, const __nv_bfloat16* w, __nv_bfloat16* y);
std::vector<ConvLaunch> plan_conv_dgrad(const ConvShape& s, const __nv_bfloat16* dy, const __nv_bfloat16* w,
                                        __nv_bfloat16* dx);
ConvLaunch plan_dgrad_concat(const ConvShape& s, const __nv_bfloat16* dy, const __nv_bfloat16* a1, int C1,
                             const __nv_bfloat16* bstack, __nv_bfloat16* dx);
WgradLaunch plan_conv_wgrad(const ConvShape& s, const __nv_bfloat16* dy, const __nv_bfloat16* x, float* dw);

WgradLaunch plan_conv_wgrad_gram(const ConvShape& s, const __nv_bfloat16* dy, const __nv_bfloat16* x, float* dw);

WgradLaunch plan_gram(const ConvShape& s, const __nv_bfloat16* x, float* g);

void stem_dgrad(const __nv_bfloat16* dy, const __nv_bfloat16* w, float* dx, int N, int H, int W, cudaStream_t stream);

void launch_conv(const ConvLaunch& l, const Epilogue& e, cudaStream_t stream);

struct ConvInstance {
  int block_n = 0, b_mn = 0, opt = 0;
};
ConvGemmParams epilogue_params(const ConvLaunch& l, const Epilogue& e);
ConvInstance select_conv_instance(const ConvLaunch& l, const ConvGemmParams& p);
struct ConvLaunchInfo {
  ConvInstance inst;
  int halo = 0, b_resident = 0, halo_stages = 0;
  int num_m_tiles = 0, num_n_tiles = 0, grid = 0, stat_slots = 0;
};
ConvLaunchInfo conv_launch_info(const ConvLaunch& l, const Epilogue& e);
void conv_instances_record(bool on);
std::vector<std::array<int, 5>> conv_instances_recorded();
std::vector<std::array<int, 3>> conv_instances_all();
int choose_epilogue_groups(const ConvGemmParams& p, int block_n);
int stat_slots(const ConvLaunch& l);
int64_t wgrad_scratch_elems(const WgradLaunch& l);
void launch_wgrad(const WgradLaunch& l, float* scratch, cudaStream_t stream);

}
```

argus_b200/csrc/ptx.cuh:

```cuda
#pragma once
#include <cuda.h>
#include <cuda_runtime.h>
#include <cuda_bf16.h>
#include <stdint.h>

namespace argus {

__device__ __forceinline__ uint32_t smem_u32(const void* p) {
  return static_cast<uint32_t>(__cvta_generic_to_shared(p));
}

__device__ __forceinline__ uint32_t elect_one() {
  uint32_t pred = 0;
  asm volatile(
      "{\n\t"
      ".reg .pred P;\n\t"
      "elect.sync _|P, 0xffffffff;\n\t"
      "selp.u32 %0, 1, 0, P;\n\t"
      "}\n"
      : "=r"(pred));
  return pred;
}

__device__ __forceinline__ void pdl_prologue() {
  asm volatile("griddepcontrol.wait;" ::: "memory");
}
__device__ __forceinline__ void pdl_begin(int trigger) {
  if (trigger) asm volatile("griddepcontrol.launch_dependents;" ::: "memory");
  else asm volatile("griddepcontrol.wait;" ::: "memory");
}
__device__ __forceinline__ void pdl_wait_deferred(int trigger) {
  if (trigger) asm volatile("griddepcontrol.wait;" ::: "memory");
}

__device__ __forceinline__ void mbar_init(uint32_t bar, uint32_t count) {
  asm volatile("mbarrier.init.shared::cta.b64 [%0], %1;" ::"r"(bar), "r"(count) : "memory");
}
__device__ __forceinline__ void fence_mbar_init() {
  asm volatile("fence.mbarrier_init.release.cluster;" ::: "memory");
}
__device__ __forceinline__ void mbar_arrive(uint32_t bar) {
  asm volatile("mbarrier.arrive.shared::cta.b64 _, [%0];" ::"r"(bar) : "memory");
}
__device__ __forceinline__ void mbar_arrive_expect_tx(uint32_t bar, uint32_t bytes) {
  asm volatile("mbarrier.arrive.expect_tx.shared::cta.b64 _, [%0], %1;" ::"r"(bar), "r"(bytes) : "memory");
}
__device__ __forceinline__ uint32_t mbar_try_wait(uint32_t bar, uint32_t parity) {
  uint32_t done;
  asm volatile(
      "{\n\t"
      ".reg .pred P;\n\t"
      "mbarrier.try_wait.parity.shared::cta.b64 P, [%1], %2;\n\t"
      "selp.u32 %0, 1, 0, P;\n\t"
      "}\n"
      : "=r"(done)
      : "r"(bar), "r"(parity)
      : "memory");
  return done;
}
__device__ __forceinline__ unsigned long long globaltimer_ns() {
  unsigned long long t;
  asm volatile("mov.u64 %0, %globaltimer;" : "=l"(t));
  return t;
}
__device__ __forceinline__ void mbar_wait(uint32_t bar, uint32_t parity) {
  if (mbar_try_wait(bar, parity)) return;
  unsigned long long t0 = 0;
  uint32_t it = 0;
  while (!mbar_try_wait(bar, parity)) {
    if ((++it & 0x3ff) == 0) {
      unsigned long long now = globaltimer_ns();
      if (t0 == 0) t0 = now;
      else if (now - t0 > 4000000000ull) __trap();
    }
  }
}

__device__ __forceinline__ void fence_proxy_async_smem() {
  asm volatile("fence.proxy.async.shared::cta;" ::: "memory");
}
__device__ __forceinline__ void tc_fence_before() {
  asm volatile("tcgen05.fence::before_thread_sync;" ::: "memory");
}
__device__ __forceinline__ void tc_fence_after() {
  asm volatile("tcgen05.fence::after_thread_sync;" ::: "memory");
}
__device__ __forceinline__ void named_bar_sync(uint32_t id, uint32_t nthreads) {
  asm volatile("bar.sync %0, %1;" ::"r"(id), "r"(nthreads) : "memory");
}

__device__ __forceinline__ void tma_prefetch_desc(const void* desc) {
  asm volatile("prefetch.tensormap [%0];" ::"l"(reinterpret_cast<uint64_t>(desc)) : "memory");
}
__device__ __forceinline__ void tma_load_2d(const void* desc, uint32_t bar, uint32_t dst, int c0, int c1) {
  asm volatile(
      "cp.async.bulk.tensor.2d.shared::cluster.global.mbarrier::complete_tx::bytes [%0], [%1, {%3, %4}], [%2];"
      ::"r"(dst), "l"(reinterpret_cast<uint64_t>(desc)), "r"(bar), "r"(c0), "r"(c1)
      : "memory");
}
__device__ __forceinline__ void tma_load_4d(const void* desc, uint32_t bar, uint32_t dst, int c0, int c1, int c2,
                                            int c3) {
  asm volatile(
      "cp.async.bulk.tensor.4d.shared::cluster.global.mbarrier::complete_tx::bytes [%0], [%1, {%3, %4, %5, %6}], "
      "[%2];" ::"r"(dst),
      "l"(reinterpret_cast<uint64_t>(desc)), "r"(bar), "r"(c0), "r"(c1), "r"(c2), "r"(c3)
      : "memory");
}
__device__ __forceinline__ void bulk_load_1d(uint32_t dst, const void* src, uint32_t bytes, uint32_t bar) {
  asm volatile("cp.async.bulk.shared::cluster.global.mbarrier::complete_tx::bytes [%0], [%1], %2, [%3];" ::"r"(dst),
               "l"(reinterpret_cast<uint64_t>(src)), "r"(bytes), "r"(bar)
               : "memory");
}
__device__ __forceinline__ void tma_store_4d(const void* desc, uint32_t src, int c0, int c1, int c2, int c3) {
  asm volatile("cp.async.bulk.tensor.4d.global.shared::cta.bulk_group [%0, {%2, %3, %4, %5}], [%1];" ::"l"(
                   reinterpret_cast<uint64_t>(desc)),
               "r"(src), "r"(c0), "r"(c1), "r"(c2), "r"(c3)
               : "memory");
}
__device__ __forceinline__ void tma_store_commit() { asm volatile("cp.async.bulk.commit_group;" ::: "memory"); }
template <int N>
__device__ __forceinline__ void tma_store_wait_read() {
  asm volatile("cp.async.bulk.wait_group.read %0;" ::"n"(N) : "memory");
}
template <int N>
__device__ __forceinline__ void tma_store_wait_all() {
  asm volatile("cp.async.bulk.wait_group %0;" ::"n"(N) : "memory");
}

__device__ __forceinline__ void tmem_alloc(uint32_t dst_smem, uint32_t ncols) {
  asm volatile("tcgen05.alloc.cta_group::1.sync.aligned.shared::cta.b32 [%0], %1;" ::"r"(dst_smem), "r"(ncols)
               : "memory");
}
__device__ __forceinline__ void tmem_relinquish() {
  asm volatile("tcgen05.relinquish_alloc_permit.cta_group::1.sync.aligned;" ::: "memory");
}
__device__ __forceinline__ void tmem_dealloc(uint32_t addr, uint32_t ncols) {
  asm volatile("tcgen05.dealloc.cta_group::1.sync.aligned.b32 %0, %1;" ::"r"(addr), "r"(ncols) : "memory");
}

__device__ __forceinline__ void umma_bf16(uint32_t tmem_d, uint64_t desc_a, uint64_t desc_b, uint32_t idesc,
                                          uint32_t accumulate) {
  asm volatile(
      "{\n\t"
      ".reg .pred p;\n\t"
      "setp.ne.b32 p, %4, 0;\n\t"
      "tcgen05.mma.cta_group::1.kind::f16 [%0], %1, %2, %3, p;\n\t"
      "}\n" ::"r"(tmem_d),
      "l"(desc_a), "l"(desc_b), "r"(idesc), "r"(accumulate)
      : "memory");
}
__device__ __forceinline__ void umma_commit(uint32_t bar) {
  asm volatile("tcgen05.commit.cta_group::1.mbarrier::arrive::one.shared::cluster.b64 [%0];" ::"r"(bar) : "memory");
}

__device__ __forceinline__ void tmem_ld_32x32(uint32_t taddr, uint32_t (&v)[32]) {
  asm volatile(
      "tcgen05.ld.sync.aligned.32x32b.x32.b32 "
      "{%0, %1, %2, %3, %4, %5, %6, %7, %8, %9, %10, %11, %12, %13, %14, %15, "
      "%16, %17, %18, %19, %20, %21, %22, %23, %24, %25, %26, %27, %28, %29, %30, %31}, [%32];"
      : "=r"(v[0]), "=r"(v[1]), "=r"(v[2]), "=r"(v[3]), "=r"(v[4]), "=r"(v[5]), "=r"(v[6]), "=r"(v[7]), "=r"(v[8]),
        "=r"(v[9]), "=r"(v[10]), "=r"(v[11]), "=r"(v[12]), "=r"(v[13]), "=r"(v[14]), "=r"(v[15]), "=r"(v[16]),
        "=r"(v[17]), "=r"(v[18]), "=r"(v[19]), "=r"(v[20]), "=r"(v[21]), "=r"(v[22]), "=r"(v[23]), "=r"(v[24]),
        "=r"(v[25]), "=r"(v[26]), "=r"(v[27]), "=r"(v[28]), "=r"(v[29]), "=r"(v[30]), "=r"(v[31])
      : "r"(taddr)
      : "memory");
}
__device__ __forceinline__ void tmem_ld_32x16(uint32_t taddr, uint32_t (&v)[16]) {
  asm volatile(
      "tcgen05.ld.sync.aligned.32x32b.x16.b32 "
      "{%0, %1, %2, %3, %4, %5, %6, %7, %8, %9, %10, %11, %12, %13, %14, %15}, [%16];"
      : "=r"(v[0]), "=r"(v[1]), "=r"(v[2]), "=r"(v[3]), "=r"(v[4]), "=r"(v[5]), "=r"(v[6]), "=r"(v[7]), "=r"(v[8]),
        "=r"(v[9]), "=r"(v[10]), "=r"(v[11]), "=r"(v[12]), "=r"(v[13]), "=r"(v[14]), "=r"(v[15])
      : "r"(taddr)
      : "memory");
}
__device__ __forceinline__ void tmem_ld_wait() { asm volatile("tcgen05.wait::ld.sync.aligned;" ::: "memory"); }

__device__ __forceinline__ uint64_t make_smem_desc_sw128(uint32_t saddr, uint32_t lbo_bytes, uint32_t sbo_bytes) {
  uint64_t d = 0;
  d |= static_cast<uint64_t>((saddr & 0x3FFFF) >> 4);
  d |= static_cast<uint64_t>((lbo_bytes >> 4) & 0x3FFF) << 16;
  d |= static_cast<uint64_t>((sbo_bytes >> 4) & 0x3FFF) << 32;
  d |= static_cast<uint64_t>(1) << 46;
  d |= static_cast<uint64_t>(2) << 61;
  return d;
}
__host__ __device__ constexpr uint32_t make_idesc_bf16(int M, int N, int a_mn_major, int b_mn_major) {
  return (1u << 4) | (1u << 7) | (1u << 10) | (static_cast<uint32_t>(a_mn_major) << 15) |
         (static_cast<uint32_t>(b_mn_major) << 16) | (static_cast<uint32_t>(N >> 3) << 17) |
         (static_cast<uint32_t>(M >> 4) << 24);
}

__device__ __forceinline__ uint32_t pack_bf16x2(float lo, float hi) {
  __nv_bfloat162 h = __floats2bfloat162_rn(lo, hi);
  return *reinterpret_cast<uint32_t*>(&h);
}
__device__ __forceinline__ float2 unpack_bf16x2(uint32_t v) {
  __nv_bfloat162 h = *reinterpret_cast<__nv_bfloat162*>(&v);
  return __bfloat1622float2(h);
}
__device__ __forceinline__ void red_add_v4(float* addr, uint32_t a, uint32_t b, uint32_t c, uint32_t d) {
  asm volatile("red.global.add.v4.f32 [%0], {%1, %2, %3, %4};" ::"l"(addr), "f"(__uint_as_float(a)),
               "f"(__uint_as_float(b)), "f"(__uint_as_float(c)), "f"(__uint_as_float(d))
               : "memory");
}
__device__ __forceinline__ uint64_t f32x2_from_bf16x2(uint32_t w) {
  uint64_t r;
  asm("mov.b64 %0, {%1, %2};" : "=l"(r) : "r"(w << 16), "r"(w & 0xffff0000u));
  return r;
}
__device__ __forceinline__ uint64_t f32x2_pack(float lo, float hi) {
  uint64_t r;
  asm("mov.b64 %0, {%1, %2};" : "=l"(r) : "f"(lo), "f"(hi));
  return r;
}
__device__ __forceinline__ void f32x2_add(uint64_t& acc, uint64_t x) {
  asm("add.rn.f32x2 %0, %0, %1;" : "+l"(acc) : "l"(x));
}
__device__ __forceinline__ void f32x2_fma_sq(uint64_t& acc, uint64_t x) {
  asm("fma.rn.f32x2 %0, %1, %1, %0;" : "+l"(acc) : "l"(x));
}
__device__ __forceinline__ void f32x2_fma(uint64_t& acc, uint64_t a, uint64_t b) {
  asm("fma.rn.f32x2 %0, %1, %2, %0;" : "+l"(acc) : "l"(a), "l"(b));
}
__device__ __forceinline__ float2 f32x2_unpack(uint64_t v) {
  float2 r;
  asm("mov.b64 {%0, %1}, %2;" : "=f"(r.x), "=f"(r.y) : "l"(v));
  return r;
}
__device__ __forceinline__ uint32_t ldg_nc_u32(const uint32_t* p) {
  uint32_t v;
  asm volatile("ld.global.nc.u32 %0, [%1];" : "=r"(v) : "l"(p));
  return v;
}
__device__ __forceinline__ uint32_t lds_u32(uint32_t saddr) {
  uint32_t v;
  asm volatile("ld.shared.u32 %0, [%1];" : "=r"(v) : "r"(saddr));
  return v;
}
__device__ __forceinline__ float warp_sum(float v) {
#pragma unroll
  for (int o = 16; o > 0; o >>= 1) v += __shfl_xor_sync(0xffffffffu, v, o);
  return v;
}

}
```

argus_b200/csrc/runtime.h:

```cpp
#pragma once
#include <cuda.h>
#include <cuda_runtime.h>
#include <cuda_bf16.h>
#include <stdint.h>
#include <stdexcept>
#include <string>
#include <vector>

namespace argus {

void set_last_error(const std::string& msg);
const char* get_last_error();

struct Error : std::runtime_error {
  using std::runtime_error::runtime_error;
};

#define ARGUS_CHECK(cond, msg)                                                                        \
  do {                                                                                                \
    if (!(cond)) throw ::argus::Error(std::string(__FILE__) + ":" + std::to_string(__LINE__) + ": " + \
                                      std::string(msg));                                              \
  } while (0)

#define ARGUS_CUDA(expr)                                                                                \
  do {                                                                                                  \
    cudaError_t _e = (expr);                                                                            \
    if (_e != cudaSuccess)                                                                              \
      throw ::argus::Error(std::string(__FILE__) + ":" + std::to_string(__LINE__) + ": " + #expr + ": " + \
                           cudaGetErrorString(_e));                                                     \
  } while (0)

#define ARGUS_API_BEGIN try { ::argus::pdl_break_all();
#define ARGUS_API_END                          \
  return 0;                                    \
  }                                            \
  catch (const std::exception& e) {            \
    ::argus::set_last_error(e.what());         \
    return 1;                                  \
  }                                            \
  catch (...) {                                \
    ::argus::set_last_error("unknown error");  \
    return 2;                                  \
  }

CUtensorMap make_tmap_bf16(const void* base, int rank, const uint64_t* dims, const uint64_t* strides_bytes,
                           const uint32_t* box);

int num_sms();
void require_sm100();

void profile_enable(bool on);
bool profile_enabled();
int64_t launch_count();
std::string profile_report_json();
bool profile_detailed();
struct ProfileScope {
  ProfileScope(const char* family, cudaStream_t stream, double flops, double bytes);
  ProfileScope(const std::string& family, cudaStream_t stream, double flops, double bytes);
  ~ProfileScope();
  int slot = -1;
  cudaStream_t stream = nullptr;
};

bool pdl_enabled();
enum PdlBreakKind { kPdlAfterWait = 1, kPdlAfterRecord = 2, kPdlAfterMemop = 4 };
void pdl_break(cudaStream_t stream, int kind);
void pdl_break_all();
bool pdl_chain_ok(cudaStream_t stream);
void pdl_mark_kernel(cudaStream_t stream);
#ifdef __CUDACC__
template <typename... KArgs, typename... Args>
inline void launch_kernel(void (*kernel)(KArgs...), dim3 grid, dim3 block, size_t smem, cudaStream_t stream,
                          Args&&... args) {
  cudaLaunchConfig_t cfg = {};
  cfg.gridDim = grid;
  cfg.blockDim = block;
  cfg.dynamicSmemBytes = smem;
  cfg.stream = stream;
  cudaLaunchAttribute attr[1];
  attr[0].id = cudaLaunchAttributeProgrammaticStreamSerialization;
  attr[0].val.programmaticStreamSerializationAllowed = 1;
  cfg.attrs = attr;
  cfg.numAttrs = (pdl_enabled() && pdl_chain_ok(stream)) ? 1 : 0;
  ARGUS_CUDA(cudaLaunchKernelEx(&cfg, kernel, static_cast<KArgs>(args)...));
  pdl_mark_kernel(stream);
}
#endif

inline int ilog2(int v) {
  int l = 0;
  while ((1 << l) < v) ++l;
  return l;
}
inline bool is_pow2(int v) { return v > 0 && (v & (v - 1)) == 0; }

}
```

include/argus_b200.h:

```cpp
#ifndef ARGUS_B200_H_
#define ARGUS_B200_H_

#include <stdint.h>

#ifdef __cplusplus
extern "C" {
#endif

const char* argus_last_error_string(void);
int argus_version(void);
int argus_require_device(void);
int64_t argus_launch_count(void);
int argus_profile_enable(int on);
int argus_profile_report(char* json, int cap);

int argus_conv2d_forward(const void* x, const void* w, void* y, int N, int H, int W, int Cin, int Cout, int k,
                         int stride, int kind, const float* scale, const float* shift, const void* residual, int relu,
                         float* stat_partial, int stat_slot_capacity, void* stream);
int argus_conv2d_stat_slots(int N, int H, int W, int Cin, int Cout, int k, int stride, int kind, int* slots);
int argus_conv2d_dgrad(const void* dy, const void* w, void* dx, int N, int H, int W, int Cin, int Cout, int k,
                       int stride, const void* residual, void* stream);
int argus_conv2d_dgrad_bits(const void* dy, const void* w, void* dx, int N, int H, int W, int Cin, int Cout, int k,
                            const void* residual, const void* residual_bits, void* stream);
int argus_conv2d_dgrad_ex(const void* dy, const void* w, void* dx, int N, int H, int W, int Cin, int Cout, int stride,
                          const void* concat_a, int concat_channels, const float* bias, const void* residual,
                          const void* out_bits, float* stat_partial, int stat_slot_capacity, void* stream);
int argus_conv2d_forward_full(const void* x, const void* w, void* y, int N, int H, int W, int Cin, int Cout, int k,
                              int stride, int kind, const float* scale, const float* shift, const void* residual,
                              const float* res_scale, const float* res_shift, int relu, void* relu_bits_out,
                              float* stat_partial, int stat_slot_capacity, int early_trigger, void* stream);
int argus_conv2d_dgrad_bnred(const void* dy, const void* w, void* dx, int N, int H, int W, int Cin, int Cout, int k,
                             int stride, const void* concat_a, int concat_channels, const float* bias,
                             const void* bn_raw, const float* bn_scale, const float* bn_shift, float* stat_partial,
                             int stat_slot_capacity, void* stream);
#define ARGUS_EPI_SCALE 1
#define ARGUS_EPI_SHIFT 2
#define ARGUS_EPI_RESIDUAL 4
#define ARGUS_EPI_RES_AFFINE 8
#define ARGUS_EPI_RELU 16
#define ARGUS_EPI_RELU_BITS_OUT 32
#define ARGUS_EPI_OUT_BITS 64
#define ARGUS_EPI_RESIDUAL_BITS 128
#define ARGUS_EPI_STATS 256
#define ARGUS_EPI_BN_RAW 512
#define ARGUS_EPI_EARLY_TRIGGER 1024
#define ARGUS_LAUNCH_INFO_INTS 10
int argus_conv2d_launch_info(int launch, int N, int H, int W, int Cin, int Cout, int k, int stride, int kind,
                             int concat_channels, int flags, int* out, int cap, int* n_launches);
int argus_conv_instances_record(int on);
int argus_conv_instances_get(int* keys, int cap, int* n);
int argus_conv_instances_all(int* keys, int cap, int* n);
int argus_conv2d_gram(const void* x, float* g, int N, int H, int W, int Cin, int Cout, int stride, void* stream);
int argus_colsum_pixels(const void* x, int N, int H, int W, int C, int stride, float* scratch, float* out, void* stream);
int argus_bn_stats_from_gram(const void* W, const float* G, const float* s, double rows, const float* gamma,
                             const float* beta, float* running_mean, float* running_var, float momentum, float eps,
                             float* scale, float* shift, float* save_mean, float* save_invstd, float* scratch, int O,
                             int C, void* stream);
int argus_conv2d_wgrad_gram(const void* dy, const void* x, float* dw, int N, int H, int W, int Cin, int Cout, int stride,
                            void* stream);
int argus_conv_bn_backward_algebraic(const void* g, const void* act, const void* w_bf16, const float* g_colsum,
                                     const float* scale, const float* mean, const float* invstd, float* dgamma,
                                     float* dbeta, float* dw, void* dact, int N, int H, int W, int C, int O, int stride,
                                     void* stream);
int argus_conv2d_wgrad(const void* dy, const void* x, float* dw, int N, int H, int W, int Cin, int Cout, int k,
                       int stride, int kind, void* stream);
int argus_stem_dgrad(const void* dy, const void* w, float* dx, int N, int H, int W, void* stream);

int argus_bn_finalize(const float* partial, int slots, double count, const float* gamma, const float* beta,
                      float* running_mean, float* running_var, float momentum, float eps, float* scale, float* shift,
                      float* save_mean, float* save_invstd, int C, void* stream);
int argus_bn_apply(const void* x, const float* scale, const float* shift, const void* res, const float* rscale,
                   const float* rshift, int relu, void* y, int64_t rows, int C, void* stream);
int argus_bn_apply_bits(const void* x, const float* scale, const float* shift, const void* res, const float* rscale,
                        const float* rshift, int relu, void* y, void* relu_bits, int64_t rows, int C, void* stream);
int argus_bn_backward(void* dy, const void* x, const void* out, const float* scale, const float* shift,
                      const float* mean, const float* invstd, float* dgamma, float* dbeta, void* dx, int64_t rows,
                      int C, int mask_mode, void* stream);
int argus_maxpool_forward(const void* x, const float* scale, const float* shift, void* y, void* idx, int N, int H,
                          int W, int C, void* stream);
int argus_maxpool_backward(const void* dy, const void* idx, void* dx, int N, int H, int W, int C, void* stream);
int argus_stem_pool_bn_backward(const void* dpool, const void* idx, const void* raw, const float* scale,
                                const float* shift, const float* mean, const float* invstd, float* dgamma,
                                float* dbeta, void* dx, int N, int H, int W, int C, void* stream);
int argus_avgpool_forward(const void* x, void* y, int N, int HW, int C, void* stream);
int argus_avgpool_backward(const void* dy, void* dx, int N, int HW, int C, void* stream);

int argus_fp32_conv2d_forward(const float* x, const float* w, const float* bias, float* y, int N, int H, int W, int Cin,
                              int Cout, int k, int stride, void* stream);
int argus_fp32_conv2d_dgrad(const float* dy, const float* w, float* dx, int N, int H, int W, int Cin, int Cout, int k,
                            int stride, void* stream);
int argus_fp32_conv2d_wgrad(const float* dy, const float* x, float* dw, int N, int H, int W, int Cin, int Cout, int k,
                            int stride, void* stream);
int argus_fp32_bn_train(const float* x, int64_t rows, int C, const float* gamma, const float* beta, float* running_mean,
                        float* running_var, float momentum, float eps, float* scale, float* shift, float* save_mean,
                        float* save_invstd, void* stream);
int argus_fp32_bn_apply(const float* x, const float* scale, const float* shift, const float* res, const float* rscale,
                        const float* rshift, int relu, float* y, int64_t rows, int C, void* stream);
int argus_fp32_bn_backward(const float* dy, const float* x, const float* out, const float* scale, const float* mean,
                           const float* invstd, float* dgamma, float* dbeta, float* dx, float* g_out, int64_t rows,
                           int C, void* stream);
int argus_fp32_maxpool_forward(const float* x, float* y, void* idx, int N, int H, int W, int C, void* stream);
int argus_fp32_maxpool_backward(const float* dy, const void* idx, float* dx, int N, int H, int W, int C, void* stream);

#define ARGUS_AUG_PARAMS 40
#define ARGUS_ARC_FIELDS 8
typedef struct argus_aug_config {
  int color_jiggle, planckian_jitter, blur, motion_blur, plasma_shadow;
  float brightness_lo, brightness_span, contrast_lo, contrast_span;
  float saturation_lo, saturation_span, hue_lo, hue_span;
  int random_erasing, salt_and_pepper;
} argus_aug_config;
int argus_augment_sample_params(float* params, int n_images, int n_cams, int H, int W, uint64_t seed, uint64_t step,
                                const argus_aug_config* cfg, void* stream);
int argus_augment(const void* in, int in_u8, void* out, int out_s2d, const float* params, const void* arc_mask,
                  void* plasma_ws, int n_images, int H, int W, int apply, void* stream);

int argus_spaghetti_sample_params(float* arcs, int n_images, int n_arcs, int H, int W, uint64_t seed, uint64_t step,
                                  void* stream);
int argus_spaghetti_mask(const float* arcs, void* mask, int n_images, int n_arcs, int H, int W, void* stream);
int argus_spaghetti_draw(const void* in, void* out, const float* arcs, void* mask_ws, int n_images, int n_arcs, int H,
                         int W, void* stream);

int argus_pose_loss(const float* pred, const float* target, float* loss, float* loss_mean, float* grad, int B,
                    float grad_scale, void* stream);
int argus_pose_exp(const float* pred, float* pose, int B, int wxyz, void* stream);

int argus_clip_adam_step(float* params, const float* grads, float* exp_avg, float* exp_avg_sq, int64_t n,
                         float* scratch, float gscale, float max_norm, float lr, float beta1, float beta2, float eps,
                         int step, float* norm_out, void* stream);
int argus_clip_adam_step_amp(float* params, const float* grads, float* exp_avg, float* exp_avg_sq, int64_t n,
                             float* scratch, float gscale, float max_norm, float lr, float beta1, float beta2, float eps,
                             int step, float* norm_out, void* stream);

typedef struct argus_model argus_model;
int argus_model_create(argus_model** out, int n_cams, int resnet_output_dim);
int argus_model_destroy(argus_model* m);
int argus_model_counts(argus_model* m, int* n_params, int* n_buffers, int64_t* param_elems, int64_t* buffer_elems);
int argus_model_tensor_info(argus_model* m, int is_buffer, int index, char* name, int name_cap, int64_t* offset,
                            int64_t* numel, int* ndim, int64_t* shape);
int argus_model_bind(argus_model* m, float* params, float* grads, float* buffers);
int argus_model_reserve(argus_model* m, int max_batch, int H, int W, int training);
int argus_model_sync_weights(argus_model* m, void* stream);
int argus_model_forward(argus_model* m, const void* x, int is_u8, int B, int H, int W, int training, float* out,
                        void* stream);
int argus_model_stage_input_u8(argus_model* m, const void* images, const float* aug_params, const void* arc_mask,
                               void* plasma_ws, int B, int H, int W, int training, int apply, void* stream);
int argus_model_set_precision(argus_model* m, int mode);
int argus_model_set_wgrad_overlap(argus_model* m, int on);
int argus_model_zero_grads(argus_model* m, void* stream);
int argus_model_backward(argus_model* m, const float* d_out, int stage_begin, int stage_end, void* stream);
int argus_model_input_grad(argus_model* m, float* dx, void* stream);
int argus_model_stage_range(argus_model* m, int stage, int64_t* begin, int64_t* end);
int argus_model_arena_bytes(argus_model* m, int64_t* bytes);
int argus_model_copy_activation(argus_model* m, int index, void* dst, int64_t capacity_elems, int64_t* rows, int* C,
                                void* stream);

typedef struct argus_loader argus_loader;
int argus_loader_create(argus_loader** out, const char* path, int batch, int rank, int world, uint64_t seed,
                        int shuffle, int drop_last);
int argus_loader_destroy(argus_loader* l);
int argus_loader_info(argus_loader* l, int64_t* n_samples, int* n_cams, int* H, int* W, int64_t* samples_per_rank,
                      int64_t* batches_per_epoch);
int argus_loader_bind(argus_loader* l, void* host_img0, void* host_img1, float* host_pose0, float* host_pose1,
                      void* dev_img0, void* dev_img1, float* dev_pose0, float* dev_pose1);
int argus_loader_set_lookahead(argus_loader* l, int on);
int argus_loader_start_epoch(argus_loader* l, int epoch);
int argus_loader_next(argus_loader* l, void* stream, int* count, int* buffer_index);

#ifdef __cplusplus
}
#endif
#endif
```

Measured before the change: 6781.

## Add 2-CTA paired tcgen05 MMA path for forward conv GEMMs

Adds a PAIR template variant of the conv GEMM kernel. It launches as 2-CTA clusters using cta_group::2 MMA with M=256: each CTA loads its own A tile and half of the B tile, and rank 0 issues the paired MMA into shared TMEM. This halves per-CTA weight traffic and smem for B, which allows more pipeline stages and bigger MMAs. The cost is cluster sync overhead and scheduling constraints. By default (mode 1) it turns on only for single-tap forward convs with block_n>=128, at least 8 k-blocks and balanced tile ownership. It also adds query APIs and an A/B profiling script.

New measurement: 6793, median of 6. Within noise of the previous version (+0.2%).

```diff
diff --git a/argus_b200/csrc/api.cu b/argus_b200/csrc/api.cu
--- a/argus_b200/csrc/api.cu
+++ b/argus_b200/csrc/api.cu
@@ -193,11 +193,8 @@
   ARGUS_API_END
 }
 
-int argus_conv2d_launch_info(int launch, int N, int H, int W, int Cin, int Cout, int k, int stride, int kind,
-                             int concat_channels, int flags, int* out, int cap, int* n_launches) {
-  ARGUS_API_BEGIN
-  require_sm100();
-  ARGUS_CHECK(out != nullptr && n_launches != nullptr, "null argument");
+static std::vector<ConvLaunch> plan_query(int launch, int N, int H, int W, int Cin, int Cout, int k, int stride,
+                                          int kind, int concat_channels, int flags, Epilogue& e) {
   ARGUS_CUDA(cudaFree(nullptr));
   static __align__(1024) char dummy[1024];
   bf16* d = reinterpret_cast<bf16*>(dummy);
@@ -212,7 +209,6 @@
     ls.push_back(plan_bnred_dgrad(make_shape(N, H, W, Cin, Cout, 1, stride, 0), d, d, d, d, concat_channels));
   else if (launch == 2) ls.push_back(plan_dgrad_concat(make_shape(N, H, W, Cin, Cout, 1, stride, 0), d, d, concat_channels, d, d));
   else throw Error("unknown launch kind");
-  Epilogue e;
   if (flags & ARGUS_EPI_SCALE) e.scale = f;
   if (flags & ARGUS_EPI_SHIFT) e.shift = f;
   if (flags & ARGUS_EPI_RESIDUAL) e.residual = d;
@@ -224,6 +220,16 @@
   if (flags & ARGUS_EPI_STATS) e.stat_partial = const_cast<float*>(f);
   if (flags & ARGUS_EPI_BN_RAW) { e.bn_raw = d; e.bn_scale = f; e.bn_shift = f; }
   if (flags & ARGUS_EPI_EARLY_TRIGGER) e.early_trigger = 1;
+  return ls;
+}
+
+int argus_conv2d_launch_info(int launch, int N, int H, int W, int Cin, int Cout, int k, int stride, int kind,
+                             int concat_channels, int flags, int* out, int cap, int* n_launches) {
+  ARGUS_API_BEGIN
+  require_sm100();
+  ARGUS_CHECK(out != nullptr && n_launches != nullptr, "null argument");
+  Epilogue e;
+  const std::vector<ConvLaunch> ls = plan_query(launch, N, H, W, Cin, Cout, k, stride, kind, concat_channels, flags, e);
   *n_launches = static_cast<int>(ls.size());
   ARGUS_CHECK(cap >= ARGUS_LAUNCH_INFO_INTS * *n_launches, "launch info buffer too small");
   for (size_t i = 0; i < ls.size(); ++i) {
@@ -232,6 +238,51 @@
                                            li.halo_stages, li.num_m_tiles, li.num_n_tiles, li.grid, li.stat_slots};
     std::memcpy(out + i * ARGUS_LAUNCH_INFO_INTS, v, sizeof(v));
   }
+  ARGUS_API_END
+}
+
+int argus_conv2d_pair_info(int launch, int N, int H, int W, int Cin, int Cout, int k, int stride, int kind,
+                           int concat_channels, int flags, int* out, int cap, int* n_launches, int* lid_map,
+                           int map_cap) {
+  ARGUS_API_BEGIN
+  require_sm100();
+  ARGUS_CHECK(out != nullptr && n_launches != nullptr, "null argument");
+  Epilogue e;
+  const std::vector<ConvLaunch> ls = plan_query(launch, N, H, W, Cin, Cout, k, stride, kind, concat_channels, flags, e);
+  *n_launches = static_cast<int>(ls.size());
+  ARGUS_CHECK(cap >= ARGUS_PAIR_INFO_INTS * *n_launches, "pair info buffer too small");
+  for (size_t i = 0; i < ls.size(); ++i) {
+    const ConvLaunchInfo li = conv_launch_info(ls[i], e);
+    const int v[ARGUS_PAIR_INFO_INTS] = {li.paired, li.pair_stages, li.max_pair_clusters, li.grid};
+    std::memcpy(out + i * ARGUS_PAIR_INFO_INTS, v, sizeof(v));
+    if (i == 0 && lid_map != nullptr && li.paired) {
+      ARGUS_CHECK(map_cap >= li.grid, "logical-id map buffer too small");
+      for (int c = 0; c < li.grid; ++c) lid_map[c] = pair_logical_cta(c >> 1, c & 1, li.num_n_tiles);
+    }
+  }
+  ARGUS_API_END
+}
+
+int argus_conv_pair_plan(int mode, int block_n, int b_mn, int halo, int b_resident, int k2_blocks, int has_stats,
+                         int num_m_tiles, int num_n_tiles, int num_taps, int num_kblocks, int grid, int max_clusters,
+                         int* paired, int* lid_map, int map_cap) {
+  ARGUS_API_BEGIN
+  ARGUS_CHECK(paired != nullptr && num_n_tiles > 0 && grid >= 0, "bad argument");
+  ConvPairQuery q;
+  q.mode = mode; q.block_n = block_n; q.b_mn = b_mn; q.halo = halo; q.b_resident = b_resident;
+  q.k2_blocks = k2_blocks; q.has_stats = has_stats; q.num_m_tiles = num_m_tiles; q.num_n_tiles = num_n_tiles;
+  q.num_taps = num_taps; q.num_kblocks = num_kblocks; q.grid = grid; q.max_clusters = max_clusters;
+  *paired = conv_pair_decide(q) ? 1 : 0;
+  if (lid_map != nullptr) {
+    ARGUS_CHECK(map_cap >= grid, "logical-id map buffer too small");
+    for (int c = 0; c < grid; ++c) lid_map[c] = pair_logical_cta(c >> 1, c & 1, num_n_tiles);
+  }
+  ARGUS_API_END
+}
+
+int argus_conv_set_pairing(int mode) {
+  ARGUS_API_BEGIN
+  conv_set_pair_mode(mode);
   ARGUS_API_END
 }
 
diff --git a/argus_b200/csrc/conv_gemm.cuh b/argus_b200/csrc/conv_gemm.cuh
--- a/argus_b200/csrc/conv_gemm.cuh
+++ b/argus_b200/csrc/conv_gemm.cuh
@@ -54,7 +54,14 @@
   const float* bn_shift;
   int early_trigger;
   float* stat_partial;
+  int paired;
+  int pair_stages;
+  CUtensorMap b_half_map;
 };
+
+__host__ __device__ inline int pair_logical_cta(int cluster, int rank, int num_n_tiles) {
+  return (cluster / num_n_tiles) * 2 * num_n_tiles + rank * num_n_tiles + cluster % num_n_tiles;
+}
 
 template <int BLOCK_N, int OPT, int EPI = 2>
 constexpr int conv_staging_buffers() { return (EPI == 4 || (BLOCK_N == 64 && !(OPT & 2))) ? 1 : 2; }
@@ -86,7 +93,7 @@
 constexpr int kOptResExtra = 16;
 constexpr int kOptBnRed = 32;
 constexpr int kOptAll = 31;
-template <int BLOCK_N, int B_MN, int EPI, int OPT = kOptAll>
+template <int BLOCK_N, int B_MN, int EPI, int OPT = kOptAll, bool PAIR = false>
 __global__ void __launch_bounds__(64 + 128 * EPI, 1)
 conv_gemm_kernel(const __grid_constant__ ConvGemmParams p) {
   pdl_begin(p.early_trigger);
@@ -117,10 +124,18 @@
   float* s_stats_all = reinterpret_cast<float*>(smem + L::kOffStats);
   const bool resident = (p.b_resident != 0);
   const bool halo = (p.halo != 0);
+  constexpr bool paired = PAIR;
+  const uint32_t rank = paired ? cluster_ctarank() : 0u;
+  auto cta_id = [&]() -> uint32_t {
+    return paired ? static_cast<uint32_t>(pair_logical_cta(static_cast<int>(cluster_id_x()), static_cast<int>(rank),
+                                                           p.num_n_tiles))
+                  : blockIdx.x;
+  };
+  const uint32_t half_b_bytes = L::kBBytes / 2;
   const uint32_t halo_a_bytes = static_cast<uint32_t>(p.halo_rows + 2) * p.halo_row_bytes;
-  const int nstages = halo ? p.halo_stages : (resident ? p.res_stages : kStages);
+  const int nstages = halo ? p.halo_stages : (resident ? p.res_stages : (paired ? p.pair_stages : kStages));
   const uint32_t stage_bytes = halo ? halo_a_bytes + (resident ? 0u : 3u * L::kBBytes)
-                                    : (resident ? L::kABytes : L::kStageBytes);
+                                    : (resident ? L::kABytes : (paired ? L::kABytes + half_b_bytes : L::kStageBytes));
   const uint32_t bres_base = smem_base + static_cast<uint32_t>(nstages) * stage_bytes;
 
   if (threadIdx.x == 0) {
@@ -130,7 +145,7 @@
       mbar_init(empty_bar(s), 1);
     }
     mbar_init(bres_bar, 1);
-    for (int s = 0; s < 2; ++s) mbar_init(tempty_bar(s), SPLIT ? 8 : 4);
+    for (int s = 0; s < 2; ++s) mbar_init(tempty_bar(s), (SPLIT ? 8 : 4) * (paired ? 2 : 1));
     for (int g = 0; g < EPI; ++g) {
       mbar_init(tfull_bar(g), 1);
       mbar_init(res_bar(g, 0), 1);
@@ -141,17 +156,23 @@
   if (warp == 0 && lane == 0) {
     for (int i = 0; i < 4; ++i) tma_prefetch_desc(&p.a_map[i]);
     if (p.halo) tma_prefetch_desc(&p.halo_map);
-    tma_prefetch_desc(&p.b_map);
+    tma_prefetch_desc(paired ? &p.b_half_map : &p.b_map);
     tma_prefetch_desc(&p.out_map);
     if (p.has_res) tma_prefetch_desc(&p.res_map);
   }
   if (warp == 1) {
-    tmem_alloc(smem_u32(const_cast<uint32_t*>(tmem_ptr_smem)), kTmemCols);
-    tmem_relinquish();
+    if (paired) {
+      tmem_alloc_pair(smem_u32(const_cast<uint32_t*>(tmem_ptr_smem)), kTmemCols);
+      tmem_relinquish_pair();
+    } else {
+      tmem_alloc(smem_u32(const_cast<uint32_t*>(tmem_ptr_smem)), kTmemCols);
+      tmem_relinquish();
+    }
   }
   for (int i = threadIdx.x; i < EPI * 8 * L::kGroupCols; i += blockDim.x) s_stats_all[i] = 0.f;
   tc_fence_before();
-  __syncthreads();
+  if (paired) cluster_sync();
+  else __syncthreads();
   tc_fence_after();
   const uint32_t tmem_base = *tmem_ptr_smem;
   pdl_wait_deferred(p.early_trigger);
@@ -161,6 +182,38 @@
 
   if (warp == 0) {
     if (lane == 0) {
+      if (paired) {
+        static_assert(!PAIR || B_MN == 0, "CTA pairs exist for K-major weights (forward launches)");
+        const int nb = static_cast<int>(rank) * (BLOCK_N / 2);
+        int stage = 0;
+        uint32_t phase = 0;
+        for (int tile = static_cast<int>(cta_id()); tile < num_tiles; tile += gridDim.x) {
+          const int m_tile = tile / p.num_n_tiles;
+          const int n_tile = tile - m_tile * p.num_n_tiles;
+          const int m0 = m_tile * kBlockM;
+          const int img0 = m0 >> p.log2_howo;
+          const int rem = m0 & ((1 << p.log2_howo) - 1);
+          const int h0 = rem >> p.log2_wo;
+          const int w0 = rem & ((1 << p.log2_wo) - 1);
+          const int n0 = n_tile * BLOCK_N + nb;
+          for (int kb = 0; kb < num_kblocks; ++kb) {
+            mbar_wait(empty_bar(stage), phase ^ 1);
+            const uint32_t sa = smem_base + stage * stage_bytes;
+            const uint32_t bar = mapa_shared(full_bar(stage), 0);
+            if (rank == 0) mbar_arrive_expect_tx(full_bar(stage), 2 * stage_bytes);
+            const int t = kb / p.kblocks_per_tap;
+            const Tap tap = p.taps[t];
+            const int kin = kb - t * p.kblocks_per_tap;
+            tma_load_4d_pair(&p.a_map[tap.map], bar, sa, kin * kBlockK, w0 + tap.dw, h0 + tap.dh, img0);
+            tma_load_2d_pair(&p.b_half_map, bar, sa + L::kABytes, tap.b_off + kin * kBlockK, n0);
+            if (++stage == nstages) { stage = 0; phase ^= 1; }
+          }
+        }
+        for (int s = 0; s < nstages; ++s) {
+          mbar_wait(empty_bar(stage), phase ^ 1);
+          if (++stage == nstages) { stage = 0; phase ^= 1; }
+        }
+      } else {
       auto load_b = [&](uint32_t bar, uint32_t sb, const Tap& tap, int kb, int n0) {
         if (B_MN == 0) {
           tma_load_2d(&p.b_map, bar, sb, tap.b_off + kb * kBlockK, n0);
@@ -238,9 +291,40 @@
           if (++stage == nstages) { stage = 0; phase ^= 1; }
         }
       }
+      }
     }
   } else if (warp == 1) {
-    if (lane == 0) {
+    if (lane == 0 && paired && rank == 0) {
+      constexpr uint32_t idesc = make_idesc_bf16(2 * kBlockM, BLOCK_N, 0, B_MN);
+      int stage = 0;
+      uint32_t phase = 0;
+      int acc = 0;
+      uint32_t acc_phase = 0;
+      int tgrp = 0;
+      for (int tile = static_cast<int>(cta_id()); tile < num_tiles; tile += gridDim.x) {
+        mbar_wait(tempty_bar(acc), acc_phase ^ 1);
+        tc_fence_after();
+        const uint32_t tmem_d = tmem_base + acc * BLOCK_N;
+        for (int kb = 0; kb < num_kblocks; ++kb) {
+          mbar_wait(full_bar(stage), phase);
+          tc_fence_after();
+          const uint32_t sa = smem_base + stage * stage_bytes;
+          const uint32_t sb = sa + L::kABytes;
+#pragma unroll
+          for (int k = 0; k < kBlockK / 16; ++k) {
+            const uint64_t da = make_smem_desc_sw128(sa + k * 32, 0, 1024);
+            const uint64_t db = (B_MN == 0) ? make_smem_desc_sw128(sb + k * 32, 0, 1024)
+                                            : make_smem_desc_sw128(sb + k * 2048, 8192, 1024);
+            umma_bf16_pair(tmem_d, da, db, idesc, (kb | k) != 0);
+          }
+          umma_commit_pair(empty_bar(stage));
+          if (kb == num_kblocks - 1) umma_commit_pair(tfull_bar(tgrp));
+          if (++stage == nstages) { stage = 0; phase ^= 1; }
+        }
+        if (++acc == 2) { acc = 0; acc_phase ^= 1; }
+        if (++tgrp == kTileGroups) tgrp = 0;
+      }
+    } else if (lane == 0 && !paired) {
       constexpr uint32_t idesc = make_idesc_bf16(kBlockM, BLOCK_N, 0, B_MN);
       int stage = 0;
       uint32_t phase = 0;
@@ -328,7 +412,7 @@
     const bool ep_relu = (OPT & kOptRelu) ? (p.relu != 0) : false;
     constexpr bool BNRED = (OPT & kOptBnRed) != 0;
     static_assert(!BNRED || ((OPT & kOptRes) && !(OPT & (kOptResExtra | kOptRelu | kOptOutBits))), "kOptBnRed rides the residual path");
-    float* my_partial = do_stats ? p.stat_partial + static_cast<size_t>(EPI * blockIdx.x + grp) * 2 * p.n_total : nullptr;
+    float* my_partial = do_stats ? p.stat_partial + static_cast<size_t>(EPI * cta_id() + grp) * 2 * p.n_total : nullptr;
     constexpr int kChunks = GW / 64;
     constexpr bool FAST_TAIL = (OPT & kOptAffine) && !(OPT & ~(kOptAffine | kOptRes | kOptRelu)) && EPI == 2;
     float* s_aff = s_stats;
@@ -359,7 +443,7 @@
       tma_load_4d(&p.res_map, res_bar(grp, b), smem_u32(stg_base + b * L::kStagingBytes), n_tile * BLOCK_N + ch * 64,
                   rem & ((1 << p.log2_wo) - 1), rem >> p.log2_wo, img0);
     };
-    const int first_tile = blockIdx.x + tg * gridDim.x;
+    const int first_tile = cta_id() + tg * gridDim.x;
     if (has_res && store_leader && first_tile < num_tiles) issue_residual(first_tile, 0, 0);
 
     int t_local = tg;
@@ -435,7 +519,10 @@
         if (ch == kChunks - 1) {
           tc_fence_before();
           __syncwarp();
-          if (lane == 0) mbar_arrive(tempty_bar(acc));
+          if (lane == 0) {
+            if (paired && cluster_ctarank() != 0) mbar_arrive_cluster(mapa_shared(tempty_bar(acc), 0));
+            else mbar_arrive(tempty_bar(acc));
+          }
         }
         if (has_res) {
           mbar_wait(res_bar(grp, buf), res_phase[buf]);
@@ -618,10 +705,12 @@
   }
 
   tc_fence_before();
-  __syncthreads();
+  if (paired) cluster_sync();
+  else __syncthreads();
   if (warp == 1) {
     tc_fence_after();
-    tmem_dealloc(tmem_base, kTmemCols);
+    if (paired) tmem_dealloc_pair(tmem_base, kTmemCols);
+    else tmem_dealloc(tmem_base, kTmemCols);
   }
 }
 
diff --git a/argus_b200/csrc/conv_ops.cu b/argus_b200/csrc/conv_ops.cu
--- a/argus_b200/csrc/conv_ops.cu
+++ b/argus_b200/csrc/conv_ops.cu
@@ -315,6 +315,10 @@
     const uint64_t str[1] = {static_cast<uint64_t>(s.Ktot()) * 2};
     const uint32_t box[2] = {64, static_cast<uint32_t>(l.block_n)};
     p.b_map = make_tmap_bf16(w, 2, dims, str, box);
+    if (l.block_n >= 128) {
+      const uint32_t half[2] = {64, static_cast<uint32_t>(l.block_n / 2)};
+      p.b_half_map = make_tmap_bf16(w, 2, dims, str, half);
+    }
   }
   {
     uint32_t bw, bh, bn;
@@ -544,6 +548,68 @@
   return l;
 }
 
+namespace {
+std::atomic<int> g_pair_mode{1};
+}
+void conv_set_pair_mode(int mode) {
+  ARGUS_CHECK(mode >= 0 && mode <= 2, "CTA-pair mode is 0, 1 or 2");
+  g_pair_mode = mode;
+}
+int conv_pair_mode() { return g_pair_mode.load(); }
+
+bool conv_pair_decide(const ConvPairQuery& q) {
+  if (q.mode == 0 || q.block_n < 128 || q.b_mn != 0 || q.halo || q.b_resident || q.k2_blocks) return false;
+  if (q.grid < 2 || q.grid % 2 != 0 || q.max_clusters < q.grid / 2) return false;
+  const int nt = q.num_n_tiles, tiles = q.num_m_tiles * nt;
+  if (nt < 1 || q.grid % (2 * nt) != 0) return false;
+  auto owned = [&](int c) { return c < tiles ? (tiles - c + q.grid - 1) / q.grid : 0; };
+  for (int c = 0; c < q.grid / 2; ++c)
+    if (owned(pair_logical_cta(c, 0, nt)) != owned(pair_logical_cta(c, 1, nt))) return false;
+  if (q.mode == 1) return q.num_taps == 1 && q.num_kblocks >= 8;
+  return true;
+}
+
+template <int BN, int BMN, int EPI, int OPT, bool PAIR>
+static void configure_conv_t() {
+  using L = ConvGemmSmem<BN, EPI, conv_staging_buffers<BN, OPT, EPI>()>;
+  static bool configured = false;
+  if (!configured) {
+    ARGUS_CUDA(cudaFuncSetAttribute(conv_gemm_kernel<BN, BMN, EPI, OPT, PAIR>, cudaFuncAttributeMaxDynamicSharedMemorySize, L::kTotal));
+    configured = true;
+  }
+}
+
+template <int BN, int BMN>
+constexpr bool has_pair_twin() { return BN >= 128 && BMN == 0; }
+
+template <int BN, int BMN, int EPI, int OPT>
+static int max_pair_clusters() {
+  using L = ConvGemmSmem<BN, EPI, conv_staging_buffers<BN, OPT, EPI>()>;
+  if constexpr (!has_pair_twin<BN, BMN>()) {
+    return 0;
+  } else {
+  static int n = -1;
+  if (n < 0) {
+    configure_conv_t<BN, BMN, EPI, OPT, true>();
+    cudaLaunchConfig_t cfg = {};
+    cfg.gridDim = dim3(num_sms() / 2 * 2);
+    cfg.blockDim = dim3(64 + 128 * EPI);
+    cfg.dynamicSmemBytes = L::kTotal;
+    cudaLaunchAttribute attr;
+    attr.id = cudaLaunchAttributeClusterDimension;
+    attr.val.clusterDim.x = 2;
+    attr.val.clusterDim.y = 1;
+    attr.val.clusterDim.z = 1;
+    cfg.attrs = &attr;
+    cfg.numAttrs = 1;
+    int c = 0;
+    ARGUS_CUDA(cudaOccupancyMaxActiveClusters(&c, conv_gemm_kernel<BN, BMN, EPI, OPT, true>, &cfg));
+    n = c;
+  }
+  return n;
+  }
+}
+
 template <int BN, int BMN, int EPI, int OPT>
 static ConvGemmParams finish_params(const ConvGemmParams& p) {
   using L = ConvGemmSmem<BN, EPI, conv_staging_buffers<BN, OPT, EPI>()>;
@@ -562,18 +628,41 @@
       q.halo_stages = std::min(L::kMaxStages, (L::kPipeBytes - bres) / halo_a);
     }
   }
+  q.paired = 0;
+  q.pair_stages = 0;
+  ConvPairQuery pq;
+  pq.mode = conv_pair_mode();
+  pq.block_n = BN; pq.b_mn = BMN; pq.halo = q.halo; pq.b_resident = q.b_resident; pq.k2_blocks = q.k2_blocks;
+  pq.has_stats = q.stat_partial != nullptr ? 1 : 0;
+  pq.num_m_tiles = q.num_m_tiles; pq.num_n_tiles = q.num_n_tiles;
+  pq.num_taps = q.num_taps;
+  pq.num_kblocks = q.num_taps * q.kblocks_per_tap + q.k2_blocks;
+  pq.grid = grid;
+  pq.max_clusters = grid / 2;
+  if (conv_pair_decide(pq)) {
+    pq.max_clusters = max_pair_clusters<BN, BMN, EPI, OPT>();
+    if (conv_pair_decide(pq)) {
+      q.paired = 1;
+      q.pair_stages = std::min(6, L::kPipeBytes / (L::kABytes + L::kBBytes / 2));
+    }
+  }
   return q;
 }
 
 template <int BN, int BMN, int EPI, int OPT>
 static void launch_conv_t(const ConvGemmParams& q, cudaStream_t stream) {
   using L = ConvGemmSmem<BN, EPI, conv_staging_buffers<BN, OPT, EPI>()>;
-  static bool configured = false;
-  if (!configured) {
-    ARGUS_CUDA(cudaFuncSetAttribute(conv_gemm_kernel<BN, BMN, EPI, OPT>, cudaFuncAttributeMaxDynamicSharedMemorySize, L::kTotal));
-    configured = true;
-  }
   const int grid = std::min(q.num_m_tiles * q.num_n_tiles, num_sms());
+  if constexpr (has_pair_twin<BN, BMN>()) {
+    if (q.paired) {
+      configure_conv_t<BN, BMN, EPI, OPT, true>();
+      launch_kernel_cluster(conv_gemm_kernel<BN, BMN, EPI, OPT, true>, grid, 64 + 128 * EPI, L::kTotal, stream, 2, q);
+      ARGUS_CUDA(cudaGetLastError());
+      return;
+    }
+  }
+  ARGUS_CHECK(!q.paired, "this instance has no CTA-pair twin");
+  configure_conv_t<BN, BMN, EPI, OPT, false>();
   launch_kernel(conv_gemm_kernel<BN, BMN, EPI, OPT>, grid, 64 + 128 * EPI, L::kTotal, stream, q);
   ARGUS_CUDA(cudaGetLastError());
 }
@@ -585,10 +674,11 @@
   int block_n, b_mn, opt;
   ConvGemmParams (*finish)(const ConvGemmParams&);
   void (*launch)(const ConvGemmParams&, cudaStream_t);
+  int (*pair_clusters)();
 };
 template <int BN, int BMN, int OPT>
 constexpr ConvInstanceEntry conv_entry() {
-  return {BN, BMN, OPT, &finish_params<BN, BMN, 2, OPT>, &launch_conv_t<BN, BMN, 2, OPT>};
+  return {BN, BMN, OPT, &finish_params<BN, BMN, 2, OPT>, &launch_conv_t<BN, BMN, 2, OPT>, &max_pair_clusters<BN, BMN, 2, OPT>};
 }
 constexpr int kTail = kOptAffine | kOptRes | kOptRelu;
 const ConvInstanceEntry kConvInstances[] = {
@@ -684,6 +774,9 @@
   info.num_n_tiles = q.num_n_tiles;
   info.grid = std::min(q.num_m_tiles * q.num_n_tiles, num_sms());
   info.stat_slots = stat_slots(l);
+  info.paired = q.paired;
+  info.pair_stages = q.pair_stages;
+  info.max_pair_clusters = find_instance(info.inst).pair_clusters();
   return info;
 }
 
diff --git a/argus_b200/csrc/conv_ops.h b/argus_b200/csrc/conv_ops.h
--- a/argus_b200/csrc/conv_ops.h
+++ b/argus_b200/csrc/conv_ops.h
@@ -89,12 +89,23 @@
   ConvInstance inst;
   int halo = 0, b_resident = 0, halo_stages = 0;
   int num_m_tiles = 0, num_n_tiles = 0, grid = 0, stat_slots = 0;
+  int paired = 0, pair_stages = 0, max_pair_clusters = 0;
 };
 ConvLaunchInfo conv_launch_info(const ConvLaunch& l, const Epilogue& e);
 void conv_instances_record(bool on);
 std::vector<std::array<int, 5>> conv_instances_recorded();
 std::vector<std::array<int, 3>> conv_instances_all();
 int choose_epilogue_groups(const ConvGemmParams& p, int block_n);
+
+void conv_set_pair_mode(int mode);
+int conv_pair_mode();
+struct ConvPairQuery {
+  int mode = 0;
+  int block_n = 0, b_mn = 0, halo = 0, b_resident = 0, k2_blocks = 0, has_stats = 0;
+  int num_m_tiles = 0, num_n_tiles = 0, num_taps = 0, num_kblocks = 0, grid = 0;
+  int max_clusters = 0;
+};
+bool conv_pair_decide(const ConvPairQuery& q);
 int stat_slots(const ConvLaunch& l);
 int64_t wgrad_scratch_elems(const WgradLaunch& l);
 void launch_wgrad(const WgradLaunch& l, float* scratch, cudaStream_t stream);
diff --git a/argus_b200/csrc/ptx.cuh b/argus_b200/csrc/ptx.cuh
--- a/argus_b200/csrc/ptx.cuh
+++ b/argus_b200/csrc/ptx.cuh
@@ -57,6 +57,27 @@
       : "r"(bar), "r"(parity)
       : "memory");
   return done;
+}
+__device__ __forceinline__ uint32_t cluster_ctarank() {
+  uint32_t r;
+  asm volatile("mov.u32 %0, %%cluster_ctarank;" : "=r"(r));
+  return r;
+}
+__device__ __forceinline__ uint32_t cluster_id_x() {
+  uint32_t r;
+  asm volatile("mov.u32 %0, %%clusterid.x;" : "=r"(r));
+  return r;
+}
+__device__ __forceinline__ uint32_t mapa_shared(uint32_t addr, uint32_t rank) {
+  uint32_t r;
+  asm volatile("mapa.shared::cluster.u32 %0, %1, %2;" : "=r"(r) : "r"(addr), "r"(rank));
+  return r;
+}
+__device__ __forceinline__ void mbar_arrive_cluster(uint32_t bar) {
+  asm volatile("mbarrier.arrive.release.cluster.shared::cluster.b64 _, [%0];" ::"r"(bar) : "memory");
+}
+__device__ __forceinline__ void cluster_sync() {
+  asm volatile("barrier.cluster.arrive.release.aligned;\n\tbarrier.cluster.wait.acquire.aligned;" ::: "memory");
 }
 __device__ __forceinline__ unsigned long long globaltimer_ns() {
   unsigned long long t;
@@ -111,6 +132,20 @@
                "l"(reinterpret_cast<uint64_t>(src)), "r"(bytes), "r"(bar)
                : "memory");
 }
+__device__ __forceinline__ void tma_load_2d_pair(const void* desc, uint32_t bar, uint32_t dst, int c0, int c1) {
+  asm volatile(
+      "cp.async.bulk.tensor.2d.cta_group::2.shared::cluster.global.mbarrier::complete_tx::bytes [%0], [%1, {%3, %4}], [%2];"
+      ::"r"(dst), "l"(reinterpret_cast<uint64_t>(desc)), "r"(bar), "r"(c0), "r"(c1)
+      : "memory");
+}
+__device__ __forceinline__ void tma_load_4d_pair(const void* desc, uint32_t bar, uint32_t dst, int c0, int c1, int c2,
+                                                 int c3) {
+  asm volatile(
+      "cp.async.bulk.tensor.4d.cta_group::2.shared::cluster.global.mbarrier::complete_tx::bytes [%0], [%1, {%3, %4, %5, "
+      "%6}], [%2];" ::"r"(dst),
+      "l"(reinterpret_cast<uint64_t>(desc)), "r"(bar), "r"(c0), "r"(c1), "r"(c2), "r"(c3)
+      : "memory");
+}
 __device__ __forceinline__ void tma_store_4d(const void* desc, uint32_t src, int c0, int c1, int c2, int c3) {
   asm volatile("cp.async.bulk.tensor.4d.global.shared::cta.bulk_group [%0, {%2, %3, %4, %5}], [%1];" ::"l"(
                    reinterpret_cast<uint64_t>(desc)),
@@ -136,6 +171,16 @@
 }
 __device__ __forceinline__ void tmem_dealloc(uint32_t addr, uint32_t ncols) {
   asm volatile("tcgen05.dealloc.cta_group::1.sync.aligned.b32 %0, %1;" ::"r"(addr), "r"(ncols) : "memory");
+}
+__device__ __forceinline__ void tmem_alloc_pair(uint32_t dst_smem, uint32_t ncols) {
+  asm volatile("tcgen05.alloc.cta_group::2.sync.aligned.shared::cta.b32 [%0], %1;" ::"r"(dst_smem), "r"(ncols)
+               : "memory");
+}
+__device__ __forceinline__ void tmem_relinquish_pair() {
+  asm volatile("tcgen05.relinquish_alloc_permit.cta_group::2.sync.aligned;" ::: "memory");
+}
+__device__ __forceinline__ void tmem_dealloc_pair(uint32_t addr, uint32_t ncols) {
+  asm volatile("tcgen05.dealloc.cta_group::2.sync.aligned.b32 %0, %1;" ::"r"(addr), "r"(ncols) : "memory");
 }
 
 __device__ __forceinline__ void umma_bf16(uint32_t tmem_d, uint64_t desc_a, uint64_t desc_b, uint32_t idesc,
@@ -151,6 +196,23 @@
 }
 __device__ __forceinline__ void umma_commit(uint32_t bar) {
   asm volatile("tcgen05.commit.cta_group::1.mbarrier::arrive::one.shared::cluster.b64 [%0];" ::"r"(bar) : "memory");
+}
+__device__ __forceinline__ void umma_bf16_pair(uint32_t tmem_d, uint64_t desc_a, uint64_t desc_b, uint32_t idesc,
+                                               uint32_t accumulate) {
+  asm volatile(
+      "{\n\t"
+      ".reg .pred p;\n\t"
+      "setp.ne.b32 p, %4, 0;\n\t"
+      "tcgen05.mma.cta_group::2.kind::f16 [%0], %1, %2, %3, p;\n\t"
+      "}\n" ::"r"(tmem_d),
+      "l"(desc_a), "l"(desc_b), "r"(idesc), "r"(accumulate)
+      : "memory");
+}
+__device__ __forceinline__ void umma_commit_pair(uint32_t bar) {
+  asm volatile(
+      "tcgen05.commit.cta_group::2.mbarrier::arrive::one.shared::cluster.multicast::cluster.b64 [%0], %1;" ::"r"(bar),
+      "h"(static_cast<uint16_t>(3))
+      : "memory");
 }
 
 __device__ __forceinline__ void tmem_ld_32x32(uint32_t taddr, uint32_t (&v)[32]) {
diff --git a/argus_b200/csrc/runtime.h b/argus_b200/csrc/runtime.h
--- a/argus_b200/csrc/runtime.h
+++ b/argus_b200/csrc/runtime.h
@@ -70,20 +70,36 @@
 void pdl_mark_kernel(cudaStream_t stream);
 #ifdef __CUDACC__
 template <typename... KArgs, typename... Args>
-inline void launch_kernel(void (*kernel)(KArgs...), dim3 grid, dim3 block, size_t smem, cudaStream_t stream,
-                          Args&&... args) {
+inline void launch_kernel_cluster(void (*kernel)(KArgs...), dim3 grid, dim3 block, size_t smem, cudaStream_t stream,
+                                  int cluster, Args&&... args) {
   cudaLaunchConfig_t cfg = {};
   cfg.gridDim = grid;
   cfg.blockDim = block;
   cfg.dynamicSmemBytes = smem;
   cfg.stream = stream;
-  cudaLaunchAttribute attr[1];
-  attr[0].id = cudaLaunchAttributeProgrammaticStreamSerialization;
-  attr[0].val.programmaticStreamSerializationAllowed = 1;
+  cudaLaunchAttribute attr[2];
+  int n = 0;
+  if (pdl_enabled() && pdl_chain_ok(stream)) {
+    attr[n].id = cudaLaunchAttributeProgrammaticStreamSerialization;
+    attr[n].val.programmaticStreamSerializationAllowed = 1;
+    ++n;
+  }
+  if (cluster > 1) {
+    attr[n].id = cudaLaunchAttributeClusterDimension;
+    attr[n].val.clusterDim.x = static_cast<unsigned>(cluster);
+    attr[n].val.clusterDim.y = 1;
+    attr[n].val.clusterDim.z = 1;
+    ++n;
+  }
   cfg.attrs = attr;
-  cfg.numAttrs = (pdl_enabled() && pdl_chain_ok(stream)) ? 1 : 0;
+  cfg.numAttrs = n;
   ARGUS_CUDA(cudaLaunchKernelEx(&cfg, kernel, static_cast<KArgs>(args)...));
   pdl_mark_kernel(stream);
+}
+template <typename... KArgs, typename... Args>
+inline void launch_kernel(void (*kernel)(KArgs...), dim3 grid, dim3 block, size_t smem, cudaStream_t stream,
+                          Args&&... args) {
+  launch_kernel_cluster(kernel, grid, block, smem, stream, 1, static_cast<Args&&>(args)...);
 }
 #endif
 
diff --git a/include/argus_b200.h b/include/argus_b200.h
--- a/include/argus_b200.h
+++ b/include/argus_b200.h
@@ -47,6 +47,14 @@
 #define ARGUS_LAUNCH_INFO_INTS 10
 int argus_conv2d_launch_info(int launch, int N, int H, int W, int Cin, int Cout, int k, int stride, int kind,
                              int concat_channels, int flags, int* out, int cap, int* n_launches);
+int argus_conv_set_pairing(int mode);
+#define ARGUS_PAIR_INFO_INTS 4
+int argus_conv2d_pair_info(int launch, int N, int H, int W, int Cin, int Cout, int k, int stride, int kind,
+                           int concat_channels, int flags, int* out, int cap, int* n_launches, int* lid_map,
+                           int map_cap);
+int argus_conv_pair_plan(int mode, int block_n, int b_mn, int halo, int b_resident, int k2_blocks, int has_stats,
+                         int num_m_tiles, int num_n_tiles, int num_taps, int num_kblocks, int grid, int max_clusters,
+                         int* paired, int* lid_map, int map_cap);
 int argus_conv_instances_record(int on);
 int argus_conv_instances_get(int* keys, int cap, int* n);
 int argus_conv_instances_all(int* keys, int cap, int* n);
diff --git a/profiles/pair_ab.py b/profiles/pair_ab.py
--- /dev/null
+++ b/profiles/pair_ab.py
@@ -0,0 +1,93 @@
+import ctypes
+import json
+import os
+import sys
+
+os.environ["ARGUS_PROFILE_DETAIL"] = "1"
+sys.path.insert(0, ".")
+import torch
+
+from argus_b200 import _lib
+from argus_b200.engine import TrainEngine
+from argus_b200.models import NCameraCNN
+from bench import synthetic_batch
+
+rounds = int(sys.argv[1]) if len(sys.argv) > 1 else 3
+MA, MB = (int(sys.argv[2]), int(sys.argv[3])) if len(sys.argv) > 3 else (0, 1)
+dev = torch.device("cuda", 0)
+imgs, tgt = synthetic_batch(256, 2, 256, 256, 0)
+imgs, tgt = imgs.to(dev), tgt.to(dev)
+lib = _lib.load()
+
+
+def fresh():
+    torch.manual_seed(42)
+    model = NCameraCNN().to(dev)
+    return model, TrainEngine(model, distributed=False)
+
+
+finals = {}
+for mode in (MA, MB):
+    _lib.call("argus_conv_set_pairing", mode)
+    model, eng = fresh()
+    for _ in range(3):
+        eng.step(imgs, tgt)
+    torch.cuda.synchronize()
+    finals[mode] = [p.detach().clone() for p in model.parameters()]
+    del model, eng
+same = all(torch.equal(a, b) for a, b in zip(finals[MA], finals[MB]))
+print(json.dumps({"weights_bitwise_equal_after_3_steps": same}), flush=True)
+
+model, eng = fresh()
+for mode in (MA, MB):
+    _lib.call("argus_conv_set_pairing", mode)
+    for _ in range(2):
+        eng.step(imgs, tgt)
+torch.cuda.synchronize()
+
+
+def step_ms(n=10):
+    a, b = torch.cuda.Event(enable_timing=True), torch.cuda.Event(enable_timing=True)
+    a.record()
+    for _ in range(n):
+        eng.step(imgs, tgt)
+    b.record()
+    torch.cuda.synchronize()
+    return a.elapsed_time(b) / n
+
+
+def families():
+    _lib.call("argus_model_set_wgrad_overlap", model._handle.ptr, 0)
+    lib.argus_profile_enable(1)
+    for _ in range(2):
+        eng.step(imgs, tgt)
+    torch.cuda.synchronize()
+    buf = ctypes.create_string_buffer(1 << 18)
+    _lib.check(lib.argus_profile_report(buf, ctypes.c_int(1 << 18)))
+    lib.argus_profile_enable(0)
+    _lib.call("argus_model_set_wgrad_overlap", model._handle.ptr, 1)
+    fam = json.loads(buf.value.decode())
+    return {k: (v["launches"] / 2, v["ms"] / 2) for k, v in fam.items() if k.startswith("conv_fwd") or k.startswith("conv_dgrad")}
+
+
+res = {MA: {"step": [], "fam": []}, MB: {"step": [], "fam": []}}
+for r in range(rounds):
+    for mode in (MA, MB):
+        _lib.call("argus_conv_set_pairing", mode)
+        eng.step(imgs, tgt)
+        res[mode]["step"].append(step_ms())
+        res[mode]["fam"].append(families())
+        print(json.dumps({"round": r, "mode": mode, "step_ms": round(res[mode]["step"][-1], 3)}), flush=True)
+
+print(f"step ms  mode {MA}:", [round(x, 3) for x in res[MA]["step"]], f" mode {MB}:", [round(x, 3) for x in res[MB]["step"]])
+keys = sorted(res[MA]["fam"][0], key=lambda k: -res[MA]["fam"][0][k][1])
+print(f"{'family':48s} {'n':>4s}  {f'mode {MA} ms (min..max)':>22s}  {f'mode {MB} ms (min..max)':>22s}  {'gain us':>8s}")
+for k in keys:
+    a = [f[k][1] for f in res[MA]["fam"]]
+    b = [f[k][1] for f in res[MB]["fam"] if k in f]
+    if not b:
+        continue
+    n = res[MA]["fam"][0][k][0]
+    print(f"{k:48s} {n:4.0f}  {min(a):9.4f}..{max(a):9.4f}  {min(b):9.4f}..{max(b):9.4f}  {1e3 * (min(a) - min(b)):8.1f}")
+props = torch.cuda.get_device_properties(0)
+print("device:", props.name, flush=True)
```
